# PaddlePaddle/Paddle3D

Measured on NVIDIA H100. Metric: CenterPoint frames/sec @300k pts, 0.075m voxel (0.1m voxel: geometry_01m), 1440x1440x40 grid, higher is better.
Workload: dtype f16x3 (fp16 hi/lo' pairs, f32 accumulation)

## Files before the change

### include/p3d_b200.h

```cpp
#ifndef P3D_B200_H_
#define P3D_B200_H_

#include <stddef.h>
#include <stdint.h>

#ifdef __cplusplus
extern "C" {
#endif

typedef void *p3d_stream_t;

enum p3d_status {
  P3D_OK = 0,
  P3D_ERR_INVALID_ARG = -1,
  P3D_ERR_WORKSPACE = -2,
  P3D_ERR_CUDA = -3,
  P3D_ERR_UNSUPPORTED = -4
};

const char *p3d_status_string(int status);
int p3d_last_cuda_error(void);
int p3d_abi_version(void);

size_t p3d_hard_voxelize_workspace_bytes(int64_t num_points, int max_points, int max_voxels);
int p3d_hard_voxelize(const float *points, int64_t num_points, int num_point_dim, const float *voxel_size_host,
                      const float *point_cloud_range_host, int max_points, int max_voxels, float *voxels,
                      int32_t *coords, int32_t *num_points_per_voxel, int32_t *num_voxels, void *workspace,
                      size_t workspace_bytes, p3d_stream_t stream);

int p3d_voxelize_mean(const float *points, int64_t num_points, int num_point_dim, const float *voxel_size_host,
                      const float *point_cloud_range_host, int max_points, int max_voxels, int batch_id,
                      float *mean, int32_t *coors4, int32_t *num_points_per_voxel, int32_t *num_voxels,
                      void *workspace, size_t workspace_bytes, p3d_stream_t stream);

int p3d_voxel_mean(const float *voxels, const int32_t *num_points_per_voxel, const int32_t *num_voxels_dev,
                   int num_voxels_cap, int max_points, int num_point_dim, float *mean, p3d_stream_t stream);

size_t p3d_scatter_dense_workspace_bytes(int batch, int D, int ny, int nx);
int p3d_scatter_dense(const float *feats, const int32_t *coords, const int32_t *n_dev, int n_cap, int C,
                      int batch, int D, int ny, int nx, int use_z, float *out, void *workspace,
                      size_t workspace_bytes, p3d_stream_t stream);

int p3d_bev_pool_v2(const float *depth, const float *feat, const int32_t *ranks_depth, const int32_t *ranks_feat,
                    const int32_t *ranks_bev, const int32_t *interval_lengths, const int32_t *interval_starts,
                    int n_intervals, int c, float *out, int64_t out_numel, p3d_stream_t stream);
int p3d_bev_pool_v2_bkwd(const float *out_grad, const float *depth, const float *feat, const int32_t *ranks_depth,
                         const int32_t *ranks_feat, const int32_t *ranks_bev, const int32_t *interval_lengths,
                         const int32_t *interval_starts, int n_intervals, int c, float *depth_grad,
                         int64_t depth_numel, float *feat_grad, int64_t feat_numel, p3d_stream_t stream);

int p3d_boxes_overlap_bev(const float *boxes_a, int num_a, const float *boxes_b, int num_b, float *overlap,
                          p3d_stream_t stream);
int p3d_boxes_iou_bev(const float *boxes_a, int num_a, const float *boxes_b, int num_b, float *iou,
                      p3d_stream_t stream);
size_t p3d_nms_workspace_bytes(int n);
int p3d_nms(const float *boxes, int n, float nms_overlap_thresh, int normal, int32_t *keep, int32_t *num_keep,
            void *workspace, size_t workspace_bytes, p3d_stream_t stream);

size_t p3d_centerpoint_postprocess_workspace_bytes(int num_tasks, int feat_h, int feat_w, int nms_pre_max_size,
                                                    int nms_post_max_size);
int p3d_centerpoint_postprocess(int num_tasks, const float *const *hm, const int32_t *hm_channels_host,
                                const float *const *reg, const float *const *height, const float *const *dim,
                                const float *const *vel, const float *const *rot, int feat_h, int feat_w,
                                const float *voxel_size_host, const float *point_cloud_range_host,
                                const float *post_center_range_host, const int32_t *num_classes_host,
                                int down_ratio, float score_threshold, float nms_iou_threshold,
                                int nms_pre_max_size, int nms_post_max_size, int with_velocity, float *bboxes,
                                float *scores, int64_t *labels, int32_t *counts, void *workspace,
                                size_t workspace_bytes, p3d_stream_t stream);

#define P3D_BEVDET_NMS_ROTATE 0
#define P3D_BEVDET_NMS_CIRCLE 1
size_t p3d_bevdet_postprocess_workspace_bytes(int num_tasks, const int32_t *hm_channels_host, int feat_h, int feat_w,
                                              int max_num);
int p3d_bevdet_postprocess(int num_tasks, const float *const *hm, const int32_t *hm_channels_host,
                           const float *const *reg, const float *const *height, const float *const *dim,
                           const float *const *vel, const float *const *rot, int feat_h, int feat_w,
                           const float *voxel_size_host, const float *point_cloud_range_host,
                           const float *post_center_range_host, int out_size_factor, float score_threshold,
                           int max_num, int pre_max_size, int post_max_size, const int32_t *nms_type_host,
                           const float *nms_thr_host, const float *min_radius_host, const float *rescale_host,
                           const int32_t *label_offset_host, float *bboxes, float *scores, int64_t *labels,
                           int32_t *counts, void *workspace, size_t workspace_bytes, p3d_stream_t stream);

size_t p3d_sparse_rulebook_workspace_bytes(int64_t n_in_cap, int64_t n_out_cap);
int p3d_sparse_rulebook_subm(const int32_t *coords, const int32_t *n_in_dev, int64_t n_in_cap, int batch,
                             const int *spatial_host, const int *ksize_host, int32_t *nbr, void *workspace,
                             size_t workspace_bytes, p3d_stream_t stream);
int p3d_sparse_rulebook_conv(const int32_t *coords, const int32_t *n_in_dev, int64_t n_in_cap, int batch,
                             const int *spatial_host, const int *ksize_host, const int *stride_host,
                             const int *pad_host, int32_t *out_coords, int32_t *n_out_dev, int64_t out_cap,
                             int32_t *nbr, void *workspace, size_t workspace_bytes, p3d_stream_t stream);

size_t p3d_sparse_table_bytes(int64_t rows_cap);
int p3d_sparse_table_build(const int32_t *coords, const int32_t *n_dev, int64_t n_cap, int batch,
                           const int *spatial_host, void *table, size_t table_bytes, p3d_stream_t stream);
int p3d_sparse_rulebook_subm_t(const int32_t *coords, const int32_t *n_dev, int64_t n_cap, int batch,
                               const int *spatial_host, const int *ksize_host, const void *table, size_t table_bytes,
                               int32_t *nbr, p3d_stream_t stream);

int p3d_sparse_rulebook_level_t(const int32_t *coords, const int32_t *n_in_dev, int64_t n_in_cap, int batch,
                                const int *spatial_host, const int *ksize_host, const int *stride_host,
                                const int *pad_host, const void *table_in, size_t table_in_bytes, int32_t *out_coords,
                                int32_t *n_out_dev, int64_t out_cap, void *table_out, size_t table_out_bytes,
                                int32_t *nbr, const int *subm_ksize_host, int32_t *nbr_subm, p3d_stream_t stream);

int p3d_sparse_affine_act(const float *x, const int32_t *n_dev, int64_t n_cap, int C, const float *scale,
                          const float *shift, const float *residual, int relu, float *out, p3d_stream_t stream);

enum p3d_conv_precision { P3D_CONV_FP32 = 0, P3D_CONV_TF32X3 = 1 };
size_t p3d_sparse_conv_packed_weight_bytes(int K, int Cin, int Cout);
int p3d_sparse_conv_pack_weights(const float *weight, int K, int Cin, int Cout, float *packed, p3d_stream_t stream);
int p3d_sparse_conv_gather_gemm(const float *in, const int32_t *nbr, const int32_t *n_out_dev, int64_t n_out_cap,
                                int K, int Cin, int Cout, const float *weight, const float *scale,
                                const float *shift, const float *residual, int relu, int precision, float *out,
                                p3d_stream_t stream);

size_t p3d_sparse_conv_splitk_workspace_bytes(int64_t n_out_cap, int Cin, int Cout);
int p3d_sparse_conv_gather_gemm_tf32x3_ws(const float *in, const int32_t *nbr, const int32_t *n_out_dev,
                                          int64_t n_out_cap, int K, int Cin, int Cout, const float *packed_weight,
                                          const float *scale, const float *shift, const float *residual, int relu,
                                          float *out, void *workspace, size_t workspace_bytes, p3d_stream_t stream);

int p3d_rows_convert_layout(const float *src, int src_layout, const int32_t *n_dev, int64_t n_cap, int C, float *dst,
                            p3d_stream_t stream);
int p3d_sparse_conv_gather_gemm_split(const float *in_split, const int32_t *nbr, const int32_t *n_out_dev,
                                      int64_t n_out_cap, int K, int Cin, int Cout, const float *packed_weight,
                                      const float *scale, const float *shift, const float *residual_split, int relu,
                                      float *out_f32, float *out_split, p3d_stream_t stream);
int p3d_sparse_conv_gather_gemm_split_ws(const float *in_split, const int32_t *nbr, const int32_t *n_out_dev,
                                         int64_t n_out_cap, int K, int Cin, int Cout, const float *packed_weight,
                                         const float *scale, const float *shift, const float *residual_split, int relu,
                                         float *out_f32, float *out_split, void *workspace, size_t workspace_bytes,
                                         p3d_stream_t stream);

int p3d_sparse_conv_small_cin_h16(const float *in, const int32_t *nbr, const int32_t *n_out_dev, int64_t n_out_cap, int K,
                                  int Cin, int Cout, const float *weight, const float *scale, const float *shift, int relu,
                                  float *out_f32, void *out_h16, int32_t *status_dev, p3d_stream_t stream);
int p3d_sparse_rows_to_pixel_h16(const void *rows_h16, const int32_t *coords, const int32_t *n_dev, int n_cap, int C,
                                 int batch, int D, int ny, int nx, void *out_pixel_h16, p3d_stream_t stream);
size_t p3d_sparse_conv_f16_packed_weight_bytes(int K, int Cin, int Cout);
int p3d_sparse_conv_f16_pack_weights(const float *weight, int K, int Cin, int Cout, void *packed, int32_t *status_dev,
                                     p3d_stream_t stream);
int p3d_rows_convert_h16(const void *src, int to_h16, const int32_t *n_dev, int64_t n_cap, int C, void *dst,
                         int32_t *status_dev, p3d_stream_t stream);
size_t p3d_sparse_conv_f16_workspace_bytes(int64_t n_out_cap, int Cout, int max_splits);
int p3d_sparse_conv_f16(const void *in_h16, const int32_t *nbr, const int32_t *n_out_dev, int64_t n_out_cap, int K,
                        int Cin, int Cout, const void *packed_weight, const float *scale, const float *shift,
                        const void *residual_h16, int relu, float *out_f32, void *out_h16, void *workspace,
                        size_t workspace_bytes, int max_splits, int32_t *status_dev, p3d_stream_t stream);

size_t p3d_sparse_conv_wm_packed_weight_bytes(int K, int Cin, int Cout);
int p3d_sparse_conv_wm_pack_weights(const float *weight, int K, int Cin, int Cout, void *packed, int32_t *status_dev,
                                    p3d_stream_t stream);
size_t p3d_sparse_conv_wm_workspace_bytes(int64_t n_out_cap, int Cout);
int p3d_sparse_conv_wm(const void *in_h16, const int32_t *nbr, const int32_t *n_out_dev, int64_t n_out_cap, int K, int Cin,
                       int Cout, const void *packed_weight, const float *scale, const float *shift,
                       const void *residual_h16, int relu, float *out_f32, void *out_h16, void *workspace,
                       size_t workspace_bytes, int32_t *status_dev, p3d_stream_t stream);

int p3d_nchw_to_pixel_split(const float *in, int B, int C, int H, int W, float *out_split, p3d_stream_t stream);
size_t p3d_dense_conv2d_packed_weight_bytes(int taps, int Cin, int Cout, int n_tile);
int p3d_dense_conv2d_split(const float *in_split, int B, int H, int W, int Cin, const float *packed_weight, int Cout,
                           int n_tile, int kh, int kw, int stride, int pad, int up, const float *scale,
                           const float *shift, int relu, float *out_split, int out_C, int out_c0, float *out_nchw,
                           p3d_stream_t stream);

int p3d_head_final_conv(const float *in_split, int B, int H, int W, int in_C, int Cin, int groups, const float *weight,
                        const float *bias, const int32_t *plane0_host, const int32_t *cnt_host, int planes,
                        float *out_nchw, p3d_stream_t stream);

int p3d_nchw_to_pixel_h16(const float *in, int B, int C, int H, int W, void *out_h16, int32_t *status_dev,
                          p3d_stream_t stream);
int p3d_pixel_h16_to_nchw(const void *in_h16, int B, int C, int H, int W, float *out, p3d_stream_t stream);
size_t p3d_dense_conv2d_f16_packed_weight_bytes(int taps, int Cin, int Cout, int n_tile);
int p3d_dense_conv2d_f16_pack_weights(const float *weight_tci, int taps, int Cin, int n_tile, void *packed,
                                      int32_t *status_dev, p3d_stream_t stream);
size_t p3d_bev_pool_prepare_workspace_bytes(int64_t num_points);
int p3d_bev_pool_prepare(const float *coor, int B, int N, int D, int H, int W, const float *grid_lower_bound_host,
                         const float *grid_interval_host, const int32_t *grid_size_host, int32_t *ranks_bev,
                         int32_t *ranks_depth, int32_t *ranks_feat, int32_t *interval_starts, int32_t *interval_lengths,
                         int32_t *counts_dev, void *workspace, size_t workspace_bytes, p3d_stream_t stream);

typedef struct p3d_lss_camera {
  float inv_post_rot[9];
  float post_trans[3];
  float combine[9];
  float trans[3];
} p3d_lss_camera;

int p3d_lss_prepare(const p3d_lss_camera *cams, const float *bda, const float *axis_depth, const float *axis_x,
                    const float *axis_y, int B, int N, int D, int H, int W, const float *grid_lower_bound_host,
                    const float *grid_interval_host, const int32_t *grid_size_host, float *coor, int32_t *ranks_bev,
                    int32_t *ranks_depth, int32_t *ranks_feat, int32_t *interval_starts, int32_t *interval_lengths,
                    int32_t *counts_dev, void *workspace, size_t workspace_bytes, p3d_stream_t stream);
int p3d_lss_depth_feat(const float *logits, const float *tran_feat, int BN, int D, int H, int W, int C, float *depth,
                       float *feat, p3d_stream_t stream);
int p3d_lss_depth_feat_h16(const void *rows_h16, int BN, int H, int W, int in_C, int D, int C, float *depth, float *feat,
                           p3d_stream_t stream);
int p3d_bev_pool_v2_dev(const float *depth, const float *feat, const int32_t *ranks_depth, const int32_t *ranks_feat,
                        const int32_t *ranks_bev, const int32_t *interval_lengths, const int32_t *interval_starts,
                        const int32_t *counts_dev, int64_t capacity, int c, int B, int Z, int Y, int X, int planar,
                        float *out, p3d_stream_t stream);

int p3d_head_out_conv_f16(const void *in_h16, int B, int H, int W, int in_C, int Cin, int groups, const void *packed_weight,
                          const float *bias, const int32_t *cin0_dev, const int32_t *plane0_dev, const int32_t *cnt_dev,
                          int planes, float *out_nchw, p3d_stream_t stream);
int p3d_head_conv_p_f16(const void *in_h16, int B, int H, int W, int Cin, const void *packed_weight, int Cout,
                        const float *scale, const float *shift, const void *packed_w2, float *p_out, int32_t *status_dev,
                        p3d_stream_t stream);
int p3d_head_tap_sum(const float *p_in, int B, int H, int W, int groups, const float *bias, const int32_t *plane0_dev,
                     const int32_t *cnt_dev, int planes, float *out_nchw, p3d_stream_t stream);
int p3d_dense_conv2d_f16(const void *in_h16, int B, int H, int W, int Cin, const void *packed_weight, int Cout, int n_tile,
                         int kh, int kw, int stride, int pad, int up, const float *scale, const float *shift, int relu,
                         void *out_h16, int out_C, int out_c0, float *out_nchw, int mode, int m_tiles,
                         int32_t *status_dev, p3d_stream_t stream);
int p3d_dense_conv2d_f16_residual(const void *in_h16, int B, int H, int W, int Cin, const void *packed_weight, int Cout,
                                  int n_tile, int kh, int kw, int stride, int pad, int up, const float *scale,
                                  const float *shift, int relu, void *out_h16, int out_C, int out_c0, float *out_nchw,
                                  const void *res_h16, int res_C, int mode, int m_tiles, int32_t *status_dev,
                                  p3d_stream_t stream);
int p3d_upsample_bilinear_h16(const void *in_h16, int B, int h, int w, int C, int scale, void *out_h16, int out_C, int out_c0,
                              int32_t *status_dev, p3d_stream_t stream);
int p3d_upsample_nearest_h16(const void *in_h16, int B, int h, int w, int C, int scale, void *out_h16, int out_C, int out_c0,
                             p3d_stream_t stream);
size_t p3d_resnet_stem_packed_weight_bytes(void);
int p3d_resnet_stem_pack_weights(const float *weight, void *packed, int32_t *status_dev, p3d_stream_t stream);
int p3d_resnet_stem_h16(const float *in, int B, int H, int W, const void *packed_weight, const float *scale, const float *shift,
                        void *out_h16, int32_t *status_dev, p3d_stream_t stream);
int p3d_image_prep_u8(const uint8_t *frames, int N, int band_rows, int H0, int W0, const int32_t *kh, const int32_t *xbounds,
                      int kh_size, int rW, const int32_t *kv, const int32_t *ybounds, int kv_size, int rH, int crop_x,
                      int crop_y, int fH, int fW, const float *mean_host, const double *std_inv_host, int swap_rb,
                      float *out, p3d_stream_t stream);
int p3d_bev_pool_v2_dev_h16(const float *depth, const float *feat, const int32_t *ranks_depth, const int32_t *ranks_feat,
                            const int32_t *ranks_bev, const int32_t *interval_lengths, const int32_t *interval_starts,
                            const int32_t *counts_dev, int64_t capacity, int c, int B, int Z, int Y, int X, void *out_h16,
                            int out_C, int32_t *status_dev, p3d_stream_t stream);
int p3d_bev_shift_h16(const void *in_h16, int B, int h, int w, int in_C, int C, const float *tf_dev, void *out_h16, int out_C,
                      int out_c0, int32_t *status_dev, p3d_stream_t stream);

int p3d_pillar_feature_net(const float *voxels, const int32_t *num_points_per_voxel, const int32_t *coors,
                           const int32_t *num_voxels_dev, int64_t n_cap, int max_points, int num_point_dim,
                           int out_channels, const float *weight, const float *bn_scale, const float *bn_shift,
                           const float *voxel_size_host, const float *point_cloud_range_host, float *out,
                           p3d_stream_t stream);
int p3d_pillar_feature_net2(const float *voxels, const int32_t *num_points_per_voxel, const int32_t *coors,
                            const int32_t *num_voxels_dev, int64_t n_cap, int max_points, int num_point_dim,
                            int mid_channels, const float *weight1, const float *bn_scale1, const float *bn_shift1,
                            int out_channels, const float *weight2, const float *bn_scale2, const float *bn_shift2,
                            const float *voxel_size_host, const float *point_cloud_range_host, float *out,
                            p3d_stream_t stream);

size_t p3d_anchor_head_postprocess_workspace_bytes(int num_anchors, int grid_nx, int grid_ny, int nms_pre_max_size);
int p3d_anchor_head_postprocess(const float *head, int feat_h, int feat_w, int anchors_per_loc, int num_classes,
                                const float *anchors, const int32_t *anchor_corners, const int32_t *coords,
                                const int32_t *num_coords_dev, int coords_cap, int grid_nx, int grid_ny,
                                int anchor_area_threshold, float score_threshold,
                                float nms_iou_threshold, int nms_pre_max_size, int nms_post_max_size,
                                const float *post_center_range_host, float *boxes, float *scores, int64_t *labels,
                                int32_t *counts, uint8_t *anchor_mask, float *sorted_boxes, float *sorted_scores,
                                void *workspace, size_t workspace_bytes, p3d_stream_t stream);

typedef struct p3d_sweep_desc {
  int32_t slot;
  int32_t rows;
  int32_t has_transform;
  float time_lag;
  double ref_from_curr[12];
} p3d_sweep_desc;

size_t p3d_merge_sweeps_workspace_bytes(int num_entries, int64_t slot_cap);
int p3d_merge_sweeps(const float *raw, int num_slots, int64_t slot_cap, int raw_dim, const p3d_sweep_desc *desc,
                     int num_entries, const int32_t *use_dim_host, int n_use_dim, int use_time_lag,
                     float sweep_remove_radius, float *out, int64_t cap, int32_t *n_out_dev, int32_t *status_dev,
                     void *workspace, size_t workspace_bytes, p3d_stream_t stream);

#ifdef __cplusplus
}
#endif
#endif
```

### paddle3d_b200/_lib.py

```python
import ctypes as C
import os

_HERE = os.path.dirname(os.path.abspath(__file__))
LIB_PATH = os.path.join(_HERE, "libp3d_b200.so")
_lib = None

c_f32p = C.c_void_p
_i64 = C.c_int64
_int = C.c_int
_f = C.c_float
_sz = C.c_size_t
_vp = C.c_void_p

SIGNATURES = {
    "p3d_status_string": (C.c_char_p, [_int]),
    "p3d_last_cuda_error": (_int, []),
    "p3d_abi_version": (_int, []),
    "p3d_hard_voxelize_workspace_bytes": (_sz, [_i64, _int, _int]),
    "p3d_hard_voxelize": (_int, [_vp, _i64, _int, _vp, _vp, _int, _int, _vp, _vp, _vp, _vp, _vp, _sz, _vp]),
    "p3d_voxelize_mean": (_int, [_vp, _i64, _int, _vp, _vp, _int, _int, _int, _vp, _vp, _vp, _vp, _vp, _sz, _vp]),
    "p3d_voxel_mean": (_int, [_vp, _vp, _vp, _int, _int, _int, _vp, _vp]),
    "p3d_scatter_dense_workspace_bytes": (_sz, [_int, _int, _int, _int]),
    "p3d_scatter_dense": (_int, [_vp, _vp, _vp, _int, _int, _int, _int, _int, _int, _int, _vp, _vp, _sz, _vp]),
    "p3d_bev_pool_v2": (_int, [_vp, _vp, _vp, _vp, _vp, _vp, _vp, _int, _int, _vp, _i64, _vp]),
    "p3d_bev_pool_v2_bkwd": (_int, [_vp, _vp, _vp, _vp, _vp, _vp, _vp, _vp, _int, _int, _vp, _i64, _vp, _i64, _vp]),
    "p3d_boxes_overlap_bev": (_int, [_vp, _int, _vp, _int, _vp, _vp]),
    "p3d_boxes_iou_bev": (_int, [_vp, _int, _vp, _int, _vp, _vp]),
    "p3d_nms_workspace_bytes": (_sz, [_int]),
    "p3d_nms": (_int, [_vp, _int, _f, _int, _vp, _vp, _vp, _sz, _vp]),
    "p3d_centerpoint_postprocess_workspace_bytes": (_sz, [_int, _int, _int, _int, _int]),
    "p3d_centerpoint_postprocess": (_int, [_int, _vp, _vp, _vp, _vp, _vp, _vp, _vp, _int, _int, _vp, _vp, _vp, _vp,
                                           _int, _f, _f, _int, _int, _int, _vp, _vp, _vp, _vp, _vp, _sz, _vp]),
    "p3d_bevdet_postprocess_workspace_bytes": (_sz, [_int, _vp, _int, _int, _int]),
    "p3d_bevdet_postprocess": (_int, [_int, _vp, _vp, _vp, _vp, _vp, _vp, _vp, _int, _int, _vp, _vp, _vp, _int, _f, _int,
                                      _int, _int, _vp, _vp, _vp, _vp, _vp, _vp, _vp, _vp, _vp, _vp, _sz, _vp]),
    "p3d_sparse_rulebook_workspace_bytes": (_sz, [_i64, _i64]),
    "p3d_sparse_rulebook_subm": (_int, [_vp, _vp, _i64, _int, _vp, _vp, _vp, _vp, _sz, _vp]),
    "p3d_sparse_rulebook_conv": (_int, [_vp, _vp, _i64, _int, _vp, _vp, _vp, _vp, _vp, _vp, _i64, _vp, _vp, _sz,
                                        _vp]),
    "p3d_sparse_table_bytes": (_sz, [_i64]),
    "p3d_sparse_table_build": (_int, [_vp, _vp, _i64, _int, _vp, _vp, _sz, _vp]),
    "p3d_sparse_rulebook_subm_t": (_int, [_vp, _vp, _i64, _int, _vp, _vp, _vp, _sz, _vp, _vp]),
    "p3d_sparse_rulebook_level_t": (_int, [_vp, _vp, _i64, _int, _vp, _vp, _vp, _vp, _vp, _sz, _vp, _vp, _i64, _vp, _sz,
                                           _vp, _vp, _vp, _vp]),
    "p3d_sparse_affine_act": (_int, [_vp, _vp, _i64, _int, _vp, _vp, _vp, _int, _vp, _vp]),
    "p3d_sparse_conv_packed_weight_bytes": (_sz, [_int, _int, _int]),
    "p3d_sparse_conv_pack_weights": (_int, [_vp, _int, _int, _int, _vp, _vp]),
    "p3d_rows_convert_layout": (_int, [_vp, _int, _vp, _i64, _int, _vp, _vp]),
    "p3d_sparse_conv_gather_gemm_split": (_int, [_vp, _vp, _vp, _i64, _int, _int, _int, _vp, _vp, _vp, _vp, _int, _vp,
                                                 _vp, _vp]),
    "p3d_sparse_conv_gather_gemm_split_ws": (_int, [_vp, _vp, _vp, _i64, _int, _int, _int, _vp, _vp, _vp, _vp, _int, _vp,
                                                    _vp, _vp, _sz, _vp]),
    "p3d_sparse_conv_splitk_workspace_bytes": (_sz, [_i64, _int, _int]),
    "p3d_sparse_conv_small_cin_h16": (_int, [_vp, _vp, _vp, _i64, _int, _int, _int, _vp, _vp, _vp, _int, _vp, _vp, _vp, _vp]),
    "p3d_sparse_rows_to_pixel_h16": (_int, [_vp, _vp, _vp, _int, _int, _int, _int, _int, _int, _vp, _vp]),
    "p3d_sparse_conv_f16_packed_weight_bytes": (_sz, [_int, _int, _int]),
    "p3d_sparse_conv_f16_pack_weights": (_int, [_vp, _int, _int, _int, _vp, _vp, _vp]),
    "p3d_rows_convert_h16": (_int, [_vp, _int, _vp, _i64, _int, _vp, _vp, _vp]),
    "p3d_sparse_conv_f16_workspace_bytes": (_sz, [_i64, _int, _int]),
    "p3d_sparse_conv_f16": (_int, [_vp, _vp, _vp, _i64, _int, _int, _int, _vp, _vp, _vp, _vp, _int, _vp, _vp, _vp, _sz,
                                   _int, _vp, _vp]),
    "p3d_sparse_conv_wm_packed_weight_bytes": (_sz, [_int, _int, _int]),
    "p3d_sparse_conv_wm_pack_weights": (_int, [_vp, _int, _int, _int, _vp, _vp, _vp]),
    "p3d_sparse_conv_wm_workspace_bytes": (_sz, [_i64, _int]),
    "p3d_sparse_conv_wm": (_int, [_vp, _vp, _vp, _i64, _int, _int, _int, _vp, _vp, _vp, _vp, _int, _vp, _vp, _vp, _sz,
                                  _vp, _vp]),
    "p3d_nchw_to_pixel_split": (_int, [_vp, _int, _int, _int, _int, _vp, _vp]),
    "p3d_dense_conv2d_packed_weight_bytes": (_sz, [_int, _int, _int, _int]),
    "p3d_pillar_feature_net": (_int, [_vp, _vp, _vp, _vp, _i64, _int, _int, _int, _vp, _vp, _vp, _vp, _vp, _vp, _vp]),
    "p3d_pillar_feature_net2": (_int, [_vp, _vp, _vp, _vp, _i64, _int, _int, _int, _vp, _vp, _vp, _int, _vp, _vp, _vp, _vp,
                                       _vp, _vp, _vp]),
    "p3d_head_final_conv": (_int, [_vp, _int, _int, _int, _int, _int, _int, _vp, _vp, _vp, _vp, _int, _vp, _vp]),
    "p3d_nchw_to_pixel_h16": (_int, [_vp, _int, _int, _int, _int, _vp, _vp, _vp]),
    "p3d_pixel_h16_to_nchw": (_int, [_vp, _int, _int, _int, _int, _vp, _vp]),
    "p3d_dense_conv2d_f16_packed_weight_bytes": (_sz, [_int, _int, _int, _int]),
    "p3d_dense_conv2d_f16_pack_weights": (_int, [_vp, _int, _int, _int, _vp, _vp, _vp]),
    "p3d_bev_pool_prepare_workspace_bytes": (_sz, [_i64]),
    "p3d_bev_pool_prepare": (_int, [_vp, _int, _int, _int, _int, _int, _vp, _vp, _vp, _vp, _vp, _vp, _vp, _vp, _vp, _vp, _sz,
                                    _vp]),
    "p3d_lss_prepare": (_int, [_vp, _vp, _vp, _vp, _vp, _int, _int, _int, _int, _int, _vp, _vp, _vp, _vp, _vp, _vp, _vp, _vp,
                               _vp, _vp, _vp, _sz, _vp]),
    "p3d_lss_depth_feat": (_int, [_vp, _vp, _int, _int, _int, _int, _int, _vp, _vp, _vp]),
    "p3d_bev_pool_v2_dev": (_int, [_vp, _vp, _vp, _vp, _vp, _vp, _vp, _vp, _i64, _int, _int, _int, _int, _int, _int, _vp, _vp]),
    "p3d_head_out_conv_f16": (_int, [_vp, _int, _int, _int, _int, _int, _int, _vp, _vp, _vp, _vp, _vp, _int, _vp, _vp]),
    "p3d_head_conv_p_f16": (_int, [_vp, _int, _int, _int, _int, _vp, _int, _vp, _vp, _vp, _vp, _vp, _vp]),
    "p3d_head_tap_sum": (_int, [_vp, _int, _int, _int, _int, _vp, _vp, _vp, _int, _vp, _vp]),
    "p3d_dense_conv2d_f16": (_int, [_vp, _int, _int, _int, _int, _vp, _int, _int, _int, _int, _int, _int, _int, _vp, _vp,
                                    _int, _vp, _int, _int, _vp, _int, _int, _vp, _vp]),
    "p3d_dense_conv2d_f16_residual": (_int, [_vp, _int, _int, _int, _int, _vp, _int, _int, _int, _int, _int, _int, _int, _vp,
                                             _vp, _int, _vp, _int, _int, _vp, _vp, _int, _int, _int, _vp, _vp]),
    "p3d_upsample_bilinear_h16": (_int, [_vp, _int, _int, _int, _int, _int, _vp, _int, _int, _vp, _vp]),
    "p3d_upsample_nearest_h16": (_int, [_vp, _int, _int, _int, _int, _int, _vp, _int, _int, _vp]),
    "p3d_resnet_stem_packed_weight_bytes": (_sz, []),
    "p3d_resnet_stem_pack_weights": (_int, [_vp, _vp, _vp, _vp]),
    "p3d_resnet_stem_h16": (_int, [_vp, _int, _int, _int, _vp, _vp, _vp, _vp, _vp, _vp]),
    "p3d_lss_depth_feat_h16": (_int, [_vp, _int, _int, _int, _int, _int, _int, _vp, _vp, _vp]),
    "p3d_image_prep_u8": (_int, [_vp, _int, _int, _int, _int, _vp, _vp, _int, _int, _vp, _vp, _int, _int, _int, _int, _int,
                                 _int, _vp, _vp, _int, _vp, _vp]),
    "p3d_bev_pool_v2_dev_h16": (_int, [_vp, _vp, _vp, _vp, _vp, _vp, _vp, _vp, _i64, _int, _int, _int, _int, _int, _vp, _int,
                                       _vp, _vp]),
    "p3d_bev_shift_h16": (_int, [_vp, _int, _int, _int, _int, _int, _vp, _vp, _int, _int, _vp, _vp]),
    "p3d_dense_conv2d_split": (_int, [_vp, _int, _int, _int, _int, _vp, _int, _int, _int, _int, _int, _int, _int, _vp, _vp,
                                      _int, _vp, _int, _int, _vp, _vp]),
    "p3d_sparse_conv_gather_gemm_tf32x3_ws": (_int, [_vp, _vp, _vp, _i64, _int, _int, _int, _vp, _vp, _vp, _vp, _int, _vp,
                                                     _vp, _sz, _vp]),
    "p3d_sparse_conv_gather_gemm": (_int, [_vp, _vp, _vp, _i64, _int, _int, _int, _vp, _vp, _vp, _vp, _int, _int,
                                           _vp, _vp]),
    "p3d_anchor_head_postprocess_workspace_bytes": (_sz, [_int, _int, _int, _int]),
    "p3d_anchor_head_postprocess": (_int, [_vp, _int, _int, _int, _int, _vp, _vp, _vp, _vp, _int, _int, _int, _int, _f,
                                           _f, _int, _int, _vp, _vp, _vp, _vp, _vp, _vp, _vp, _vp, _vp, _sz, _vp]),
    "p3d_merge_sweeps_workspace_bytes": (_sz, [_int, _i64]),
    "p3d_merge_sweeps": (_int, [_vp, _int, _i64, _int, _vp, _int, _vp, _int, _int, _f, _vp, _i64, _vp, _vp, _vp, _sz,
                                _vp]),
}


class P3DError(RuntimeError):
    pass


def lib():
    global _lib
    if _lib is None:
        if not os.path.exists(LIB_PATH):
            raise P3DError("libp3d_b200.so is not built: run `python -c 'import __graft_entry__ as g; g.build()'` "
                           "(paddle3d_b200 has no CPU or library fallback)")
        _lib = C.CDLL(LIB_PATH)
        for name, (res, args) in SIGNATURES.items():
            fn = getattr(_lib, name)
            fn.restype = res
            fn.argtypes = args
    return _lib


_DEBUG_SYNC = bool(os.environ.get("P3D_DEBUG_SYNC"))


def check(rc, what):
    if _DEBUG_SYNC and rc == 0:
        import torch
        try:
            torch.cuda.synchronize()
        except Exception as e:
            raise P3DError("%s: kernel fault (%s)" % (what, e))
    if rc != 0:
        l = lib()
        msg = l.p3d_status_string(rc).decode()
        extra = " (cudaError %d)" % l.p3d_last_cuda_error() if rc == -3 else ""
        raise P3DError("%s failed: %s%s" % (what, msg, extra))


def fptr(arr):
    return C.cast(arr, C.c_void_p)


def host_floats(vals):
    return (C.c_float * len(vals))(*[float(v) for v in vals])


def host_ints(vals):
    return (C.c_int * len(vals))(*[int(v) for v in vals])
```

### paddle3d_b200/centerpoint_pillars.py

```python
import numpy as np
import torch

from . import synth
from .dense_head import DenseRPNHead, SecondTrunk
from .frame import CapturedFrame, ResultSlot
from .ops import centerpoint_postprocess as cpp
from .ops import pillar_encoder as pe
from .ops import sparse_nn as sp
from .ops import voxelize as vox
from .pointpillars import grid_size

CONFIG = dict(
    pfn=dict(feat_channels=(64, 64), bn_eps=1e-3),
    backbone=dict(out_channels=(64, 128, 256), layer_nums=(3, 5, 5), downsample_strides=(2, 2, 2)),
    fpn=dict(out_channels=(128, 128, 128), upsample_strides=(0.5, 1, 2), use_conv_for_no_stride=True),
    head=dict(tasks=tuple(synth.CENTERPOINT_TASKS), share_conv_channel=64),
    test=synth.CENTERPOINT_PILLARS_TEST_CFG,
)


class CenterPointPillars:

    def __init__(self, cfg=None, model_cfg=None):
        self.cfg = dict(cfg or synth.CP_PILLARS)
        self.mc = model_cfg or CONFIG
        mc = self.mc
        self.grid = grid_size(self.cfg)
        self.F = self.cfg["point_dim"]
        c1, c2 = mc["pfn"]["feat_channels"]
        self.pfn_channels = (c1 // 2, c2)
        self.C = c2
        b, f, h = mc["backbone"], mc["fpn"], mc["head"]
        self.head = DenseRPNHead(in_channels=self.C, out_channels=b["out_channels"], layer_nums=b["layer_nums"],
                                 downsample_strides=b["downsample_strides"], fpn_out_channels=f["out_channels"],
                                 upsample_strides=f["upsample_strides"], tasks=h["tasks"],
                                 share_conv_channel=h["share_conv_channel"], bev_depth=1)
        self.test_cfg = dict(mc["test"])
        self.label_off = synth.label_offsets(list(h["tasks"]))
        self.feat_hw, self.cat_hw = self._feature_sizes()
        self.device = None

    def _feature_sizes(self):
        h, w = self.grid[1], self.grid[0]
        sizes = []
        for blk in self.head.blocks:
            for c in blk:
                h, w = (h + 2 * c.padding - c.k) // c.stride + 1, (w + 2 * c.padding - c.k) // c.stride + 1
            sizes.append((h, w))
        cat = {SecondTrunk.deblock_out_hw(de, hh, ww) for (hh, ww), de in zip(sizes, self.head.deblocks)}
        if len(cat) != 1:
            raise ValueError("model config: the FPN deblocks give different sizes %s" % sorted(cat))
        return sizes, cat.pop()

    def init_weight(self, seed=0, device="cuda", bn_gain=1.0):
        rng = np.random.default_rng(seed)
        eps = self.mc["pfn"]["bn_eps"]
        self.pfn = []
        for fan_in, c in ((self.F + 5, self.pfn_channels[0]), (2 * self.pfn_channels[0], self.pfn_channels[1])):
            self.pfn.append(dict(weight=synth.kaiming_uniform(rng, (fan_in, c), fan_in),
                                 gamma=np.full(c, bn_gain, np.float32), beta=np.zeros(c, np.float32),
                                 mean=np.zeros(c, np.float32), var=np.ones(c, np.float32), eps=eps))
        self.head.init_weight(seed=seed + 1, device=device, bn_gain=bn_gain)
        self.device = None if device is None else torch.device(device)
        if device is not None:
            self.pfn_dev = [dict(l, weight=torch.from_numpy(l["weight"]).to(device)) for l in self.pfn]
            self.pfn_folded = [pe.fold_bn(l["gamma"], l["beta"], l["mean"], l["var"], l["eps"], device) for l in self.pfn]
        return self

    def export_numpy(self):
        return dict(self.head.export_numpy(), pfn=self.pfn)

    def encode(self, points):
        cfg = self.cfg
        voxels, co, npv, nv = vox.hard_voxelize(points, cfg["voxel_size"], cfg["point_cloud_range"], cfg["max_points"],
                                                cfg["max_voxels"])
        coors = torch.nn.functional.pad(co, (1, 0))
        feats = pe.pillar_feature_net2(voxels, npv, coors, self.pfn_dev, cfg["voxel_size"], cfg["point_cloud_range"],
                                       num_voxels=nv, folded=self.pfn_folded)
        nx, ny = self.grid
        image, shape = sp.sparse_coo_tensor(coors, feats, [1, 1, ny, nx, self.C], num=nv).to_pixel_h16()
        return image, shape, coors, nv

    def dense(self, image, shape):
        return self.head.forward_h16(image, shape)

    def postprocess(self, h):
        return cpp.centerpoint_postprocess_heads(h, self.cfg["voxel_size"][:2], self.cfg["point_cloud_range"],
                                                 self.test_cfg, self.label_off)

    def calibrate_heatmap_bias(self, points, target_frac=0.014):
        image, shape, _, _ = self.encode(points)
        self.head.calibrate_heatmap_bias(image, self.test_cfg["score_threshold"], target_frac, shape=shape)
        return self

    def head_planes(self):
        return self.head.head_planes()

    def flops(self):
        out = dict(backbone=0.0, fpn=0.0)
        h, w = self.grid[1], self.grid[0]
        for blk in self.head.blocks:
            for c in blk:
                h, w = (h + 2 * c.padding - c.k) // c.stride + 1, (w + 2 * c.padding - c.k) // c.stride + 1
                out["backbone"] += 2.0 * h * w * c.cin * c.cout * c.k * c.k
        for (h, w), de in zip(self.feat_hw, self.head.deblocks):
            oh, ow = SecondTrunk.deblock_out_hw(de, h, w)
            out["fpn"] += 2.0 * oh * ow * de.cin * de.cout * (1 if de.up > 1 else de.k * de.k)
        out.update(self.head.head_flops(*self.cat_hw))
        return out


class CenterPointPillarsHotPath(CapturedFrame):

    def __init__(self, cfg=None, device="cuda:0", seed=0, num_points=None, bn_gain=1.0, model_cfg=None,
                 sweep_input=None, sweep_ring=None):
        super().__init__(cfg or synth.CP_PILLARS, device, num_points, sweep_input, sweep_ring)
        m = self.model = CenterPointPillars(self.cfg, model_cfg).init_weight(seed=seed, device=self.device,
                                                                             bn_gain=bn_gain)
        self.slot = ResultSlot(len(m.label_off) * m.test_cfg["nms_post_max_size"], 9, len(m.label_off) + 1,
                               1 if self.sweep_input is None else 2)

    def forward_device(self):
        m = self.model
        if self.sweep_input is not None:
            self._merge_sweeps()
        image, shape, coors, nv = m.encode(self.points)
        h = m.dense(image, shape)
        boxes, scores, labels, counts = m.postprocess(h)
        status = torch.stack([sp.status_tensor(self.device)[0]] +
                             ([self._merge_status[0]] if self.sweep_input is not None else []))
        return dict(boxes=boxes, scores=scores, labels=labels, counts=counts, num_voxels=nv, coors=coors, head=h,
                    status=status)

    def _calibrate(self):
        self.model.calibrate_heatmap_bias(self.points)

    def check_status(self, status_host):
        st = [int(v) for v in status_host]
        if len(st) > 1:
            self._check_merge_status(st[1])
        if st[0]:
            raise RuntimeError("CenterPoint-pillars: an activation left fp16's range (|x| >= 65504) on the fp16-pair path")
```

### paddle3d_b200/csrc/dense_conv_f16.cu

```cuda
#include <cuda.h>
#include <cuda_fp16.h>

#include <type_traits>

#include "h16.cuh"
#include "p3d_b200.h"
#include "tc_common.cuh"

namespace p3d {
namespace dcf {

using namespace tc;

constexpr int kTW = 8, kTH = 16;
constexpr int kPitch = kTW + 2;
constexpr int kMaxA = 6, kMaxB = 12;
constexpr int kSmemBudget = (227 - 6) * 1024;
constexpr int kDenseThreads = 384;
constexpr uint32_t kConsumerWarps = 8;
constexpr uint32_t kEpiThreads = 96;

struct Params {
  int B, H, W, Cin;
  int taps, kw, stride, pad;
  int up;
  int oH, oW;
  int tiles_x, tiles_y, n_ntiles;
  int cout;
  int out_H, out_W;
  int out_C, out_c0;
  int relu;
  const uint8_t *packed_w;
  const float *scale, *shift;
  uint8_t *out_h16;
  float *out_nchw;
  int32_t *status;
};
struct ParamsP : Params {
  const uint8_t *packed_w2;
};
struct ParamsR : Params {
  const uint8_t *res_h16;
  int res_C;
};
template <bool FUSE_P, bool RES = false>
using KParams = std::conditional_t<FUSE_P, ParamsP, std::conditional_t<RES, ParamsR, Params>>;

constexpr int kP2Blk = 64 * 32, kP2Bytes = 4 * kP2Blk, kPPitch = 28;

template <int N, int MT, bool HALO>
struct Cfg {
  static constexpr int A_ROWS = HALO ? kPitch * (kTH * MT + 2) : kM * MT;
  static constexpr int A_BYTES = ((A_ROWS * 128 + 1023) / 1024) * 1024;
  static constexpr int B_BYTES = 128 * N;
  static constexpr int B_BLK = 64 * N;
  static constexpr int SP = N + 8;
  static constexpr int STG_WG = MT * 64 * SP;
  static constexpr int STG_BYTES = 2 * STG_WG * 4;
  static constexpr int PAIR_BLK = 64 * 128, PAIR_BYTES = MT * (N / 32) * PAIR_BLK;
  static_assert(PAIR_BYTES + 2 * 2 * N * 4 <= STG_WG * 4 && STG_WG * 4 % 1024 == 0, "pair tile inside the staging tile");
  static constexpr int AVAIL = kSmemBudget - STG_BYTES;
  static constexpr int NA_TAP_RAW = AVAIL / (A_BYTES + B_BYTES);
  static constexpr int NA = HALO ? 2 : (NA_TAP_RAW > kMaxA ? kMaxA : NA_TAP_RAW);
  static constexpr int BUDGET = AVAIL - NA * A_BYTES;
  static constexpr int NB_RAW = BUDGET / B_BYTES;
  static constexpr int NB = NB_RAW > kMaxB ? kMaxB : NB_RAW;
  static constexpr int ACC = MT * N;
  static constexpr int SPU = HALO ? 9 : 1;
  static constexpr int P_REGS = 88, C_REGS = 208;
  static_assert(128 * P_REGS + 256 * C_REGS <= kDenseThreads * 168, "register split");
  static_assert(N == 64 || N == 128, "N tile: 64 or 128");
  static_assert(MT == 1 || MT == 2, "one or two M tiles");
  static_assert(MT * N <= 128, "accumulators: at most 128 registers per thread");
  static_assert(NB >= 3, "weight ring too shallow");
  static_assert(NA >= 2 && NA <= kMaxA, "activation ring depth");
};

__device__ __forceinline__ void tma_tile4d(uint32_t dst, const CUtensorMap *map, int c, int x, int y, int b, uint32_t bar) {
  asm volatile(
      "cp.async.bulk.tensor.4d.shared::cluster.global.tile.mbarrier::complete_tx::bytes [%0], [%1, {%2, %3, %4, %5}], [%6];" ::
          "r"(dst),
      "l"(reinterpret_cast<uint64_t>(map)), "r"(c), "r"(x), "r"(y), "r"(b), "r"(bar)
      : "memory");
}
__device__ __forceinline__ void tma_store4d(const CUtensorMap *map, uint32_t src, int c, int x, int y, int b) {
  asm volatile("cp.async.bulk.tensor.4d.global.shared::cta.bulk_group [%0, {%2, %3, %4, %5}], [%1];" ::"l"(
                   reinterpret_cast<uint64_t>(map)),
               "r"(src), "r"(c), "r"(x), "r"(y), "r"(b)
               : "memory");
}
__device__ __forceinline__ void tma_store5d(const CUtensorMap *map, uint32_t src, int c, int d1, int d2, int d3, int d4) {
  asm volatile("cp.async.bulk.tensor.5d.global.shared::cta.bulk_group [%0, {%2, %3, %4, %5, %6}], [%1];" ::"l"(
                   reinterpret_cast<uint64_t>(map)),
               "r"(src), "r"(c), "r"(d1), "r"(d2), "r"(d3), "r"(d4)
               : "memory");
}
__device__ __forceinline__ void st_shared_u32(uint32_t addr, uint32_t v) {
  asm volatile("st.shared.b32 [%0], %1;" ::"r"(addr), "r"(v));
}
__device__ __forceinline__ float2 ld_shared_f2(uint32_t addr) {
  float2 v;
  asm("ld.shared.v2.f32 {%0, %1}, [%2];" : "=f"(v.x), "=f"(v.y) : "r"(addr));
  return v;
}
__device__ __forceinline__ void bulk_commit() { asm volatile("cp.async.bulk.commit_group;" ::: "memory"); }
__device__ __forceinline__ void bulk_wait_read() { asm volatile("cp.async.bulk.wait_group.read 0;" ::: "memory"); }
__device__ __forceinline__ void bulk_wait_all() { asm volatile("cp.async.bulk.wait_group 0;" ::: "memory"); }
struct Item {
  int nt, tap0, tx0, ty0, b;
};

enum TraceField {
  kTrItems, kTrCycles,
  kTrAFull, kTrBFull = kTrAFull + 2,
  kTrMma = kTrBFull + 2,
  kTrEpi = kTrMma + 2,
  kTrStageFree = kTrEpi + 2,
  kTrAEmpty = kTrStageFree + 2, kTrBEmpty,
  kTrEwWait, kTrEwBusy,
  kTrFields
};
#ifdef P3D_DENSE_TRACE
constexpr int kTrMaxCtas = 1024;
__device__ unsigned long long g_dense_trace[kTrMaxCtas][kTrFields];
struct Trace {
  unsigned long long sum[kTrFields] = {};
  __device__ __forceinline__ long long now() const { return clock64(); }
  __device__ __forceinline__ void add(int f, long long t0) { sum[f] += static_cast<unsigned long long>(clock64() - t0); }
  __device__ __forceinline__ void count(int f, unsigned long long v) { sum[f] += v; }
  __device__ void flush(int cw) const {
#pragma unroll
    for (int f = 0; f < kTrFields; ++f) {
      const int dst = f >= kTrAFull && f < kTrAEmpty ? f + cw : f;
      if (sum[f]) atomicAdd(&g_dense_trace[blockIdx.x % kTrMaxCtas][dst], sum[f]);
    }
  }
};
#else
struct Trace {
  __device__ __forceinline__ long long now() const { return 0; }
  __device__ __forceinline__ void add(int, long long) {}
  __device__ __forceinline__ void count(int, unsigned long long) {}
  __device__ __forceinline__ void flush(int) const {}
};
#endif
__device__ __forceinline__ Item decode(long long idx, const Params &p, int th) {
  Item it;
  long long q = blockIdx.x + idx * gridDim.x;
  it.nt = static_cast<int>(q % p.n_ntiles);
  q /= p.n_ntiles;
  it.tap0 = 0;
  if (p.up > 1) {
    const int up2 = p.up * p.up;
    it.tap0 = static_cast<int>(q % up2);
    q /= up2;
  }
  it.tx0 = static_cast<int>(q % p.tiles_x) * kTW;
  q /= p.tiles_x;
  it.ty0 = static_cast<int>(q % p.tiles_y) * th;
  it.b = static_cast<int>(q / p.tiles_y);
  return it;
}

template <int N, int MT>
__device__ __forceinline__ void epilogue_warps(const Params &p, const float *stg, unsigned long long *staged,
                                               unsigned long long *freed, long long n_items, int th, int et) {
  constexpr int SP = N + 8, ROWS = MT * 64;
  const int ew = et >> 5, lane = et & 31;
  bool ovf = false;
  Trace tr;
  for (long long idx = 0; idx < n_items; ++idx) {
    const Item im = decode(idx, p, th);
    const int dy = p.up > 1 ? im.tap0 / p.up : 0, dx = p.up > 1 ? im.tap0 % p.up : 0;
    for (int c = 0; c < 2; ++c) {
      long long t0 = tr.now();
      mbar_wait(smem_u32(staged + c), static_cast<uint32_t>(idx & 1));
      tr.add(kTrEwWait, t0);
      t0 = tr.now();
      const float *st = stg + c * ROWS * SP;
      auto pixel = [&](int r, int &Y, int &X) {
        const int m = c * 64 + (r & 63), iy = im.ty0 + (r >> 6) * kTH + m / kTW, ix = im.tx0 + m % kTW;
        Y = iy * p.up + dy;
        X = ix * p.up + dx;
        return iy < p.oH && ix < p.oW;
      };
      if (p.out_h16) {
        const int r4 = lane >> 3, c4 = (lane & 7) * 4;
        for (int q = 0; q < N / 32; ++q) {
          const int col = q * 32 + c4, ch = im.nt * N + col, oc = p.out_c0 + ch;
          if (ch >= p.cout) continue;
          float sc[4], sh[4];
#pragma unroll
          for (int e = 0; e < 4; ++e) {
            sc[e] = p.scale ? __ldg(p.scale + ch + e) : 1.0f;
            sh[e] = p.shift ? __ldg(p.shift + ch + e) : 0.0f;
          }
#pragma unroll 2
          for (int rq = ew; rq < ROWS / 4; rq += 3) {
            const int r = rq * 4 + r4;
            int Y, X;
            if (!pixel(r, Y, X)) continue;
            const float4 o4 = *reinterpret_cast<const float4 *>(st + r * SP + col);
            float v[4] = {o4.x, o4.y, o4.z, o4.w};
#pragma unroll
            for (int e = 0; e < 4; ++e) {
              v[e] = fmaf(v[e], sc[e], sh[e]);
              if (p.relu) v[e] = fmaxf(v[e], 0.f);
            }
            __half2 h01, l01, h23, l23;
            split_h16x2(v[0], v[1], h01, l01, ovf);
            split_h16x2(v[2], v[3], h23, l23, ovf);
            uint8_t *op = p.out_h16 + ((static_cast<size_t>(im.b) * p.out_H + Y) * p.out_W + X) * (4 * static_cast<size_t>(p.out_C)) +
                          (oc / 32) * 128 + (oc % 32) * 2;
            *reinterpret_cast<uint2 *>(op) = make_uint2(*reinterpret_cast<const uint32_t *>(&h01), *reinterpret_cast<const uint32_t *>(&h23));
            *reinterpret_cast<uint2 *>(op + 64) = make_uint2(*reinterpret_cast<const uint32_t *>(&l01), *reinterpret_cast<const uint32_t *>(&l23));
          }
        }
      }
      if (p.out_nchw) {
        const int px = lane & 7, cc = lane >> 3;
        for (int u = ew; u < (ROWS / 8) * (N / 4); u += 3) {
          const int r = (u % (ROWS / 8)) * 8 + px, col = (u / (ROWS / 8)) * 4 + cc, ch = im.nt * N + col;
          int Y, X;
          if (ch >= p.cout || !pixel(r, Y, X)) continue;
          const float sc = p.scale ? __ldg(p.scale + ch) : 1.0f, sh = p.shift ? __ldg(p.shift + ch) : 0.0f;
          float v = fmaf(st[r * SP + col], sc, sh);
          if (p.relu) v = fmaxf(v, 0.f);
          p.out_nchw[((static_cast<size_t>(im.b) * p.cout + ch) * p.out_H + Y) * p.out_W + X] = v;
        }
      }
      mbar_arrive(smem_u32(freed + c));
      tr.add(kTrEwBusy, t0);
    }
  }
  if (ovf && p.status) atomicOr(p.status, 1);
  if (et == 0) tr.flush(0);
}

template <int N, int MT, bool FUSE_P>
__device__ __forceinline__ void epilogue_pairs(const Params &p, const CUtensorMap *out_map, const uint8_t *tiles, int tile_bytes,
                                               unsigned long long *staged, unsigned long long *freed, long long n_items,
                                               int th, int et) {
  constexpr int NQ = N / 32, BLK = 64 * 128;
  const bool lead = et == 0;
  const bool whole = p.out_c0 % 32 == 0;
  Trace tr;
  for (long long idx = 0; idx < n_items; ++idx) {
    const Item im = decode(idx, p, th);
    const int dy = p.up > 1 ? im.tap0 / p.up : 0, dx = p.up > 1 ? im.tap0 % p.up : 0;
    for (int c = 0; c < 2; ++c) {
      long long t0 = tr.now();
      mbar_wait(smem_u32(staged + c), static_cast<uint32_t>(idx & 1));
      tr.add(kTrEwWait, t0);
      t0 = tr.now();
      if constexpr (FUSE_P) {
        if (lead) tma_store4d(out_map, smem_u32(tiles + c * tile_bytes), 0, im.tx0, im.ty0 + c * 8, (im.b * p.n_ntiles + im.nt) * 2);
      } else {
        for (int blk = 0; blk < MT * NQ; ++blk) {
          const int ch0 = im.nt * N + (blk % NQ) * 32, iy0 = im.ty0 + (blk / NQ) * kTH + c * 8;
          if (ch0 >= p.cout) continue;
          const uint8_t *src = tiles + c * tile_bytes + blk * BLK;
          if (whole && ch0 + 32 <= p.cout) {
            if (!lead) continue;
            const int hc = 2 * (p.out_c0 + ch0);
            if (p.up == 1) {
              tma_store4d(out_map, smem_u32(src), hc, im.tx0, iy0, im.b);
            } else {
              for (int y = 0; y < 8 && iy0 + y < p.oH; ++y)
                tma_store5d(out_map, smem_u32(src + y * 1024), hc, dx, im.tx0, dy, im.b * p.oH + iy0 + y);
            }
            continue;
          }
          for (int u = et; u < 128; u += kEpiThreads) {
            const int r = u >> 1, h = u & 1, iy = iy0 + (r >> 3), ix = im.tx0 + (r & 7);
            if (ch0 + 16 * h >= p.cout || iy >= p.oH || ix >= p.oW) continue;
            const int oc = p.out_c0 + ch0 + 16 * h, Y = iy * p.up + dy, X = ix * p.up + dx;
            uint8_t *op = p.out_h16 + ((static_cast<size_t>(im.b) * p.out_H + Y) * p.out_W + X) * (4 * static_cast<size_t>(p.out_C)) +
                          (oc / 32) * 128 + (oc % 32) * 2;
            const uint8_t *row = src + r * 128;
  #pragma unroll
            for (int k = 0; k < 2; ++k) {
              *reinterpret_cast<uint4 *>(op + 16 * k) = *reinterpret_cast<const uint4 *>(row + (((2 * h + k) ^ (r & 7)) << 4));
              *reinterpret_cast<uint4 *>(op + 64 + 16 * k) = *reinterpret_cast<const uint4 *>(row + (((4 + 2 * h + k) ^ (r & 7)) << 4));
            }
          }
        }
      }
      if (lead) {
        bulk_commit();
        bulk_wait_read();
      }
      mbar_arrive(smem_u32(freed + c));
      tr.add(kTrEwBusy, t0);
    }
  }
  if (lead) {
    bulk_wait_all();
    tr.flush(0);
  }
}

template <int N, int MT, bool HALO, bool FUSE_P = false, bool RES = false>
__global__ void __launch_bounds__(kDenseThreads, 1)
    dense_conv_f16_kernel(const __grid_constant__ CUtensorMap in_map, const __grid_constant__ CUtensorMap out_map,
                          const KParams<FUSE_P, RES> p) {
  using C = Cfg<N, MT, HALO>;
  static_assert(!(FUSE_P && RES), "a residual launch writes the pixel H16 image");
  static_assert(!FUSE_P || (N == 128 && MT == 1 && HALO && 2 * kP2Bytes == C::B_BYTES &&
                            2 * 64 * kPPitch * 4 <= C::PAIR_BYTES),
                "fused P: two 64-channel heads' W2 images fill one weight slot; P fits over the pair blocks");
  constexpr int TH = kTH * MT;
  constexpr int H = N / 2;
  asm volatile("griddepcontrol.launch_dependents;" ::: "memory");
  asm volatile("griddepcontrol.wait;" ::: "memory");
  const int up2 = p.up * p.up;
  const long long n_total = static_cast<long long>(p.B) * p.tiles_y * p.tiles_x * p.n_ntiles * (p.up > 1 ? up2 : 1);
  if (static_cast<long long>(blockIdx.x) >= n_total) return;
  const long long n_items = (n_total - blockIdx.x + gridDim.x - 1) / gridDim.x;

  extern __shared__ __align__(1024) uint8_t smem_raw[];
  uint8_t *smem = reinterpret_cast<uint8_t *>((reinterpret_cast<uintptr_t>(smem_raw) + 1023) & ~uintptr_t(1023));
  __shared__ __align__(8) unsigned long long s_bar[2 * kMaxA + 2 * kMaxB + 4];
  constexpr int kAF = 0, kAE = kMaxA, kBF = 2 * kMaxA, kBE = 2 * kMaxA + kMaxB, kSS = 2 * kMaxA + 2 * kMaxB, kSF = kSS + 2;

  const int tid = threadIdx.x, wg = tid >> 7, wtid = tid & 127;
  if (tid == 0) {
    for (int s = 0; s < C::NA; ++s) {
      mbar_init(smem_u32(&s_bar[kAF + s]), 1);
      mbar_init(smem_u32(&s_bar[kAE + s]), kConsumerWarps);
    }
    for (int s = 0; s < C::NB; ++s) {
      mbar_init(smem_u32(&s_bar[kBF + s]), 1);
      mbar_init(smem_u32(&s_bar[kBE + s]), kConsumerWarps);
    }
    for (int c = 0; c < 2; ++c) {
      mbar_init(smem_u32(&s_bar[kSS + c]), 128);
      mbar_init(smem_u32(&s_bar[kSF + c]), kEpiThreads);
    }
    fence_mbar_init();
  }
  __syncthreads();
  const uint32_t a_ring = smem_u32(smem);
  const uint32_t b_ring = a_ring + C::NA * C::A_BYTES;
  float *const stg = reinterpret_cast<float *>(smem + C::NA * C::A_BYTES + C::NB * C::B_BYTES);
  const bool pairs = p.out_nchw == nullptr;
  const int G = p.Cin / 32;
  const int taps_item = p.up > 1 ? 1 : p.taps;
  const int units_item = HALO ? G : taps_item * G;

  if (wg == 0) {
    asm volatile("setmaxnreg.dec.sync.aligned.u32 %0;" ::"n"(C::P_REGS));
    if (tid >= 32) {
      if (pairs)
        epilogue_pairs<N, MT, FUSE_P>(p, &out_map, reinterpret_cast<const uint8_t *>(stg), C::STG_WG * 4, s_bar + kSS, s_bar + kSF,
                              n_items, TH, tid - 32);
      else
        epilogue_warps<N, MT>(p, stg, s_bar + kSS, s_bar + kSF, n_items, TH, tid - 32);
      return;
    }
    if (tid != 0) return;
    uint32_t a_slot = 0, a_ph = 0, b_slot = 0, b_ph = 0;
    Trace tr;
    for (long long idx = 0; idx < n_items; ++idx) {
      const Item im = decode(idx, p, TH);
      const uint8_t *w_tile = p.packed_w + static_cast<size_t>(im.nt) * p.taps * (p.Cin / 16) * C::B_BLK;
      int dy = 0, dx = 0;
      for (int tu = 0; tu < (HALO ? 1 : taps_item); ++tu) {
        const int tap = p.up > 1 ? im.tap0 : tu;
        for (int g = 0; g < G; ++g) {
          const uint32_t abar = smem_u32(&s_bar[kAF + a_slot]), a_dst = a_ring + a_slot * C::A_BYTES;
          const long long t0 = tr.now();
          mbar_wait(smem_u32(&s_bar[kAE + a_slot]), a_ph ^ 1u);
          tr.add(kTrAEmpty, t0);
          mbar_arrive_expect_tx(abar, static_cast<uint32_t>(C::A_ROWS * 128));
          if (HALO) {
            tma_tile4d(a_dst, &in_map, g * 64, im.tx0 - 1, im.ty0 - 1, im.b, abar);
          } else {
            const int x = im.tx0 * p.stride - p.pad + dx, y = im.ty0 * p.stride - p.pad + dy;
            tma_tile4d(a_dst, &in_map, g * 64, x, y, im.b, abar);
          }
          if (++a_slot == C::NA) a_slot = 0, a_ph ^= 1u;
          for (int t = 0; t < C::SPU; ++t) {
            const uint32_t bbar = smem_u32(&s_bar[kBF + b_slot]);
            const long long t1 = tr.now();
            mbar_wait(smem_u32(&s_bar[kBE + b_slot]), b_ph ^ 1u);
            tr.add(kTrBEmpty, t1);
            mbar_arrive_expect_tx(bbar, static_cast<uint32_t>(C::B_BYTES));
            bulk_g2s(b_ring + b_slot * C::B_BYTES, w_tile + (static_cast<size_t>(HALO ? t : tap) * (p.Cin / 16) + 2 * g) * C::B_BLK,
                     static_cast<uint32_t>(C::B_BYTES), bbar);
            if (++b_slot == C::NB) b_slot = 0, b_ph ^= 1u;
          }
        }
        if (++dx == p.kw) dx = 0, ++dy;
      }
      if constexpr (FUSE_P) {
        const uint32_t bbar = smem_u32(&s_bar[kBF + b_slot]);
        const long long t1 = tr.now();
        mbar_wait(smem_u32(&s_bar[kBE + b_slot]), b_ph ^ 1u);
        tr.add(kTrBEmpty, t1);
        mbar_arrive_expect_tx(bbar, static_cast<uint32_t>(C::B_BYTES));
        bulk_g2s(b_ring + b_slot * C::B_BYTES, p.packed_w2 + static_cast<size_t>(im.nt) * C::B_BYTES,
                 static_cast<uint32_t>(C::B_BYTES), bbar);
        if (++b_slot == C::NB) b_slot = 0, b_ph ^= 1u;
      }
    }
    tr.flush(0);
    return;
  }

  asm volatile("setmaxnreg.inc.sync.aligned.u32 %0;" ::"n"(C::C_REGS));
  const int cw = wg - 1;
  const bool warp_leader = (tid & 31) == 0;
  auto release = [&](int base, uint32_t slot) {
    if (warp_leader) mbar_arrive(smem_u32(&s_bar[base + slot]));
  };
  uint32_t a_slot = 0, a_ph = 0, b_slot = 0, b_ph = 0;
  float acc[C::ACC];
  bool ovf = false;
  Trace tr;
  const long long t_start = tr.now();
  for (long long idx = 0; idx < n_items; ++idx) {
#pragma unroll
    for (int i = 0; i < C::ACC; ++i) acc[i] = 0.f;
    const Item im = decode(idx, p, TH);
    const uint32_t ss = smem_u32(stg) + cw * C::STG_WG * 4 + C::PAIR_BYTES + static_cast<uint32_t>(idx & 1) * 2 * N * 4;
    if (pairs) {
      for (int c = wtid; c < 2 * N; c += 128) {
        const int ch = im.nt * N + c % N;
        const float *src = c < N ? p.scale : p.shift;
        st_shared_u32(ss + c * 4, __float_as_uint(ch < p.cout && src ? __ldg(src + ch) : (c < N ? 1.0f : 0.0f)));
      }
    }
    uint32_t prev_b = 0;
    int prev_a = -1;
    bool pending = false;
    for (int ua = 0; ua < units_item; ++ua) {
      long long t0 = tr.now();
      mbar_wait(smem_u32(&s_bar[kAF + a_slot]), a_ph);
      tr.add(kTrAFull, t0);
      const uint32_t a_base = a_ring + a_slot * C::A_BYTES;
      for (int t = 0; t < C::SPU; ++t) {
        t0 = tr.now();
        mbar_wait(smem_u32(&s_bar[kBF + b_slot]), b_ph);
        tr.add(kTrBFull, t0);
        const uint32_t b_base = b_ring + b_slot * C::B_BYTES;
        wg_fence();
#pragma unroll
        for (int kb = 0; kb < 2; ++kb) {
          const uint32_t bk = b_base + static_cast<uint32_t>(kb * C::B_BLK);
          const uint64_t dbh = smem_desc(bk, 2 * N * 16, 128), dbl = smem_desc(bk + N * 16, 2 * N * 16, 128);
#pragma unroll
          for (int mt = 0; mt < MT; ++mt) {
            uint32_t a0, sbo;
            if (HALO) {
              a0 = a_base + static_cast<uint32_t>(((mt * kTH + cw * 8 + t / 3) * kPitch + t % 3) * 128);
              sbo = kPitch * 128;
            } else {
              a0 = a_base + static_cast<uint32_t>((mt * kM + cw * 64) * 128);
              sbo = 1024;
            }
            const uint64_t dah = desc_sw128(a0 + kb * 32, sbo), dal = desc_sw128(a0 + (2 + kb) * 32, sbo);
            float *d = acc + mt * N;
            wg::mma_f16<N>(d, dah, dbh, 1u);
            wg::mma_f16<N>(d + H, dah, dbl, 1u);
            wg::mma_f16<N>(d + H, dal, dbh, 1u);
          }
        }
        wg_commit();
        t0 = tr.now();
        wg_wait<1>();
        tr.add(kTrMma, t0);
        if (pending) {
          release(kBE, prev_b);
          if (prev_a >= 0) release(kAE, static_cast<uint32_t>(prev_a));
        }
        pending = true;
        prev_b = b_slot;
        prev_a = t == C::SPU - 1 ? static_cast<int>(a_slot) : -1;
        if (++b_slot == C::NB) b_slot = 0, b_ph ^= 1u;
      }
      if (++a_slot == C::NA) a_slot = 0, a_ph ^= 1u;
    }
    long long t0 = tr.now();
    wg_wait<0>();
    tr.add(kTrMma, t0);
    t0 = tr.now();
    release(kBE, prev_b);
    release(kAE, static_cast<uint32_t>(prev_a));
    wg_fence_acc<C::ACC>(acc);
    tr.add(kTrEpi, t0);
    t0 = tr.now();
    if (idx > 0) mbar_wait(smem_u32(&s_bar[kSF + cw]), static_cast<uint32_t>((idx - 1) & 1));
    tr.add(kTrStageFree, t0);
    t0 = tr.now();
    if (pairs) {
      const int lane = wtid & 31, key = lane >> 2;
      const uint32_t row = smem_u32(stg) + cw * C::STG_WG * 4 + ((wtid >> 5) * 16 + key) * 128 + (lane & 3) * 4;
      uint32_t a_hi[4], a_lo[4];
#pragma unroll
      for (int jj = 0; jj < 4; ++jj) a_hi[jj] = row + ((jj ^ key) << 4), a_lo[jj] = row + (((4 + jj) ^ key) << 4);
      uint32_t after_bar;
      asm volatile("bar.sync %1, 128;\n\tmov.u32 %0, 0;" : "=r"(after_bar) : "r"(1 + cw) : "memory");
      const uint32_t sc_col = ss + after_bar + (lane & 3) * 8;
      int r_off[MT][2], r_rem = 0;
      if constexpr (RES) {
        const int r_iy = im.ty0 + cw * 8 + (wtid >> 5) * 2, r_ix = im.tx0 + key;
#pragma unroll
        for (int mt = 0; mt < MT; ++mt)
#pragma unroll
          for (int h = 0; h < 2; ++h) {
            const int Y = r_iy + mt * kTH + h;
            r_off[mt][h] = r_ix < p.oW && Y < p.oH
                               ? ((im.b * p.out_H + Y) * p.out_W + r_ix) * 4 * p.res_C + (im.nt * N / 32) * 128 + (lane & 3) * 4
                               : -1;
          }
        r_rem = p.cout - im.nt * N;
      }
      bool o[MT][2] = {};
#pragma unroll
      for (int j = 0; j < N / 8; ++j) {
        const float2 sc = ld_shared_f2(sc_col + j * 32), sh = ld_shared_f2(sc_col + (N + j * 8) * 4);
        const float sc0 = sc.x, sc1 = sc.y, sh0 = sh.x, sh1 = sh.y;
#pragma unroll
        for (int mt = 0; mt < MT; ++mt) {
#pragma unroll
          for (int h = 0; h < 2; ++h) {
            const int i = j * 4 + h * 2;
            float v0 = fmaf(acc[mt * N + H + i], kLoInv, acc[mt * N + i]);
            float v1 = fmaf(acc[mt * N + H + i + 1], kLoInv, acc[mt * N + i + 1]);
            v0 = fmaf(v0, sc0, sh0);
            v1 = fmaf(v1, sc1, sh1);
            if constexpr (RES) {
              if (r_off[mt][h] >= 0 && j * 8 < r_rem) {
                const uint8_t *rp = p.res_h16 + r_off[mt][h] + (j / 4) * 128 + (j & 3) * 16;
                const uint32_t rh = __ldg(reinterpret_cast<const unsigned int *>(rp));
                const uint32_t rl = __ldg(reinterpret_cast<const unsigned int *>(rp + 64));
                const float2 fh = __half22float2(*reinterpret_cast<const __half2 *>(&rh));
                const float2 fl = __half22float2(*reinterpret_cast<const __half2 *>(&rl));
                v0 += fmaf(fl.x, kLoInv, fh.x);
                v1 += fmaf(fl.y, kLoInv, fh.y);
              }
            }
            if (p.relu) v0 = fmaxf(v0, 0.f), v1 = fmaxf(v1, 0.f);
            __half2 hi, lo;
            split_h16x2(v0, v1, hi, lo, o[mt][h]);
            const uint32_t off = (mt * (N / 32) + j / 4) * C::PAIR_BLK + h * 8 * 128;
            st_shared_u32(a_hi[j & 3] + off, *reinterpret_cast<const uint32_t *>(&hi));
            st_shared_u32(a_lo[j & 3] + off, *reinterpret_cast<const uint32_t *>(&lo));
          }
        }
      }
      const int iy = im.ty0 + cw * 8 + (wtid >> 5) * 2, ix = im.tx0 + key;
#pragma unroll
      for (int mt = 0; mt < MT; ++mt)
        ovf |= ix < p.oW && ((o[mt][0] && iy + mt * kTH < p.oH) || (o[mt][1] && iy + mt * kTH + 1 < p.oH));
      fence_proxy_async();
      if constexpr (FUSE_P) {
        asm volatile("bar.sync %0, 128;" ::"r"(1 + cw) : "memory");
        const long long t1 = tr.now();
        mbar_wait(smem_u32(&s_bar[kBF + b_slot]), b_ph);
        tr.add(kTrBFull, t1);
        const uint32_t w2 = b_ring + b_slot * C::B_BYTES, tile = smem_u32(stg) + cw * C::STG_WG * 4;
        float pacc[64];
#pragma unroll
        for (int i = 0; i < 64; ++i) pacc[i] = 0.f;
        wg_fence();
#pragma unroll
        for (int j = 0; j < 2; ++j) {
#pragma unroll
          for (int k = 0; k < 2; ++k) {
#pragma unroll
            for (int kb = 0; kb < 2; ++kb) {
              const uint32_t bk = w2 + static_cast<uint32_t>(j * kP2Bytes + (k * 2 + kb) * kP2Blk);
              const uint64_t dbh = smem_desc(bk, 2 * 32 * 16, 128), dbl = smem_desc(bk + 32 * 16, 2 * 32 * 16, 128);
              const uint32_t a0 = tile + static_cast<uint32_t>((2 * j + k) * C::PAIR_BLK);
              const uint64_t dah = desc_sw128(a0 + kb * 32), dal = desc_sw128(a0 + (2 + kb) * 32);
              wg::mma_f16<32>(pacc + 32 * j, dah, dbh, 1u);
              wg::mma_f16<32>(pacc + 32 * j + 16, dah, dbl, 1u);
              wg::mma_f16<32>(pacc + 32 * j + 16, dal, dbh, 1u);
            }
          }
        }
        wg_commit();
        wg_wait<0>();
        release(kBE, b_slot);
        if (++b_slot == C::NB) b_slot = 0, b_ph ^= 1u;
        wg_fence_acc<64>(pacc);
        asm volatile("bar.sync %0, 128;" ::"r"(1 + cw) : "memory");
        float *const pt = stg + cw * C::STG_WG;
#pragma unroll
        for (int j = 0; j < 2; ++j) {
#pragma unroll
          for (int i = 0; i < 16; i += 2) {
            const int r = frag_row(i, wtid), c = frag_col(i, wtid);
            if (c < kPPitch)
              *reinterpret_cast<float2 *>(pt + (j * 64 + r) * kPPitch + c) =
                  make_float2(fmaf(pacc[32 * j + 16 + i], kLoInv, pacc[32 * j + i]),
                              fmaf(pacc[32 * j + 17 + i], kLoInv, pacc[32 * j + 1 + i]));
          }
        }
        fence_proxy_async();
      }
    } else {
      float *const st = stg + cw * C::STG_WG;
#pragma unroll
      for (int mt = 0; mt < MT; ++mt) {
#pragma unroll
        for (int i = 0; i < H; i += 2) {
          const int r = mt * 64 + frag_row(i, wtid), c = frag_col(i, wtid);
          *reinterpret_cast<float2 *>(st + r * C::SP + c) =
              make_float2(fmaf(acc[mt * N + H + i], kLoInv, acc[mt * N + i]), fmaf(acc[mt * N + H + i + 1], kLoInv, acc[mt * N + i + 1]));
        }
      }
    }
    mbar_arrive(smem_u32(&s_bar[kSS + cw]));
    tr.add(kTrEpi, t0);
  }
  if (ovf && p.status) atomicOr(p.status, 1);
  if (cw == 0) {
    tr.count(kTrItems, static_cast<unsigned long long>(n_items));
    tr.add(kTrCycles, t_start);
  }
  if (wtid == 0) tr.flush(cw);
}

__global__ void __launch_bounds__(256) nchw_to_pixel_h16_kernel(const float *__restrict__ in, int C, long long HW,
                                                                __half *__restrict__ out, int32_t *status) {
  __shared__ float s_t[32][33];
  const int b = blockIdx.z;
  const long long p0 = static_cast<long long>(blockIdx.x) * 32;
  const int c0 = blockIdx.y * 32;
  const int tx = threadIdx.x & 31, ty = threadIdx.x >> 5;
  for (int k = ty; k < 32; k += 8) {
    const int c = c0 + k;
    const long long px = p0 + tx;
    s_t[k][tx] = (c < C && px < HW) ? in[(static_cast<size_t>(b) * C + c) * HW + px] : 0.f;
  }
  __syncthreads();
  bool ovf = false;
  for (int k = ty; k < 32; k += 8) {
    const long long px = p0 + k;
    if (px < HW) {
      __half h, l;
      split_h16(s_t[tx][k], h, l, ovf);
      __half *grp = out + (static_cast<size_t>(b) * HW + px) * (2 * static_cast<size_t>(C)) + static_cast<size_t>(c0) * 2;
      grp[tx] = h;
      grp[32 + tx] = l;
    }
  }
  if (ovf && status) atomicOr(status, 1);
}

__global__ void __launch_bounds__(256) pixel_h16_to_nchw_kernel(const __half *__restrict__ in, int C, long long HW,
                                                                float *__restrict__ out, long long total) {
  const long long q = static_cast<long long>(blockIdx.x) * blockDim.x + threadIdx.x;
  if (q >= total) return;
  const long long px = q % HW;
  const int c = static_cast<int>((q / HW) % C);
  const long long b = q / (HW * C);
  const __half *grp = in + (b * HW + px) * (2 * static_cast<long long>(C)) + (c / 32) * 64;
  out[q] = merge_h16(grp[c % 32], grp[32 + c % 32]);
}

using Encode = CUresult (*)(CUtensorMap *, CUtensorMapDataType, cuuint32_t, void *, const cuuint64_t *, const cuuint64_t *,
                            const cuuint32_t *, const cuuint32_t *, CUtensorMapInterleave, CUtensorMapSwizzle,
                            CUtensorMapL2promotion, CUtensorMapFloatOOBfill);
inline Encode tensor_map_encoder() {
  static Encode encode = nullptr;
  if (!encode) {
    void *fn = nullptr;
    cudaDriverEntryPointQueryResult qr;
    if (cudaGetDriverEntryPoint("cuTensorMapEncodeTiled", &fn, cudaEnableDefault, &qr) != cudaSuccess || !fn) return nullptr;
    encode = reinterpret_cast<Encode>(fn);
  }
  return encode;
}

inline int make_image_map(const void *img, int B, int H, int W, int Cin, int stride, int box_x, int box_y, CUtensorMap *map) {
  const Encode encode = tensor_map_encoder();
  if (!encode) return P3D_ERR_UNSUPPORTED;
  const cuuint64_t row = static_cast<cuuint64_t>(4) * Cin;
  const cuuint64_t gdim[4] = {static_cast<cuuint64_t>(2 * Cin), static_cast<cuuint64_t>(W), static_cast<cuuint64_t>(H),
                              static_cast<cuuint64_t>(B)};
  const cuuint64_t gstride[3] = {row, row * W, row * W * H};
  const cuuint32_t box[4] = {64u, static_cast<cuuint32_t>(box_x * stride), static_cast<cuuint32_t>(box_y * stride), 1u};
  const cuuint32_t estride[4] = {1u, static_cast<cuuint32_t>(stride), static_cast<cuuint32_t>(stride), 1u};
  const CUresult r = encode(map, CU_TENSOR_MAP_DATA_TYPE_FLOAT16, 4, const_cast<void *>(img), gdim, gstride, box, estride,
                            CU_TENSOR_MAP_INTERLEAVE_NONE, CU_TENSOR_MAP_SWIZZLE_128B, CU_TENSOR_MAP_L2_PROMOTION_NONE,
                            CU_TENSOR_MAP_FLOAT_OOB_FILL_NONE);
  return r == CUDA_SUCCESS ? P3D_OK : P3D_ERR_INVALID_ARG;
}

inline int make_out_map(void *img, int B, int H, int W, int out_C, int up, CUtensorMap *map) {
  const Encode encode = tensor_map_encoder();
  if (!encode) return P3D_ERR_UNSUPPORTED;
  const cuuint64_t row = static_cast<cuuint64_t>(4) * out_C;
  CUresult r;
  if (up == 1) {
    const cuuint64_t gdim[4] = {static_cast<cuuint64_t>(2 * out_C), static_cast<cuuint64_t>(W), static_cast<cuuint64_t>(H),
                                static_cast<cuuint64_t>(B)};
    const cuuint64_t gstride[3] = {row, row * W, row * W * H};
    const cuuint32_t box[4] = {64u, static_cast<cuuint32_t>(kTW), 8u, 1u}, estride[4] = {1u, 1u, 1u, 1u};
    r = encode(map, CU_TENSOR_MAP_DATA_TYPE_FLOAT16, 4, img, gdim, gstride, box, estride, CU_TENSOR_MAP_INTERLEAVE_NONE,
               CU_TENSOR_MAP_SWIZZLE_128B, CU_TENSOR_MAP_L2_PROMOTION_NONE, CU_TENSOR_MAP_FLOAT_OOB_FILL_NONE);
  } else {
    const cuuint64_t u = static_cast<cuuint64_t>(up), ow = u * W;
    const cuuint64_t gdim[5] = {static_cast<cuuint64_t>(2 * out_C), u, static_cast<cuuint64_t>(W), u,
                                static_cast<cuuint64_t>(B) * H};
    const cuuint64_t gstride[4] = {row, row * u, row * ow, row * ow * u};
    const cuuint32_t box[5] = {64u, 1u, static_cast<cuuint32_t>(kTW), 1u, 1u}, estride[5] = {1u, 1u, 1u, 1u, 1u};
    r = encode(map, CU_TENSOR_MAP_DATA_TYPE_FLOAT16, 5, img, gdim, gstride, box, estride, CU_TENSOR_MAP_INTERLEAVE_NONE,
               CU_TENSOR_MAP_SWIZZLE_128B, CU_TENSOR_MAP_L2_PROMOTION_NONE, CU_TENSOR_MAP_FLOAT_OOB_FILL_NONE);
  }
  return r == CUDA_SUCCESS ? P3D_OK : P3D_ERR_INVALID_ARG;
}

inline int make_p_map(float *pbuf, int B, int H, int W, int p_groups, CUtensorMap *map) {
  const Encode encode = tensor_map_encoder();
  if (!encode) return P3D_ERR_UNSUPPORTED;
  const cuuint64_t px = static_cast<cuuint64_t>(4) * kPPitch;
  const cuuint64_t gdim[4] = {static_cast<cuuint64_t>(kPPitch), static_cast<cuuint64_t>(W), static_cast<cuuint64_t>(H),
                              static_cast<cuuint64_t>(B) * p_groups};
  const cuuint64_t gstride[3] = {px, px * W, px * W * H};
  const cuuint32_t box[4] = {static_cast<cuuint32_t>(kPPitch), static_cast<cuuint32_t>(kTW), 8u, 2u}, estride[4] = {1u, 1u, 1u, 1u};
  const CUresult r = encode(map, CU_TENSOR_MAP_DATA_TYPE_FLOAT32, 4, pbuf, gdim, gstride, box, estride, CU_TENSOR_MAP_INTERLEAVE_NONE,
                            CU_TENSOR_MAP_SWIZZLE_NONE, CU_TENSOR_MAP_L2_PROMOTION_NONE, CU_TENSOR_MAP_FLOAT_OOB_FILL_NONE);
  return r == CUDA_SUCCESS ? P3D_OK : P3D_ERR_INVALID_ARG;
}

template <int N, int MT, bool HALO, bool FUSE_P = false, bool RES = false>
int launch(const CUtensorMap &map, const CUtensorMap &out_map, const KParams<FUSE_P, RES> &p, cudaStream_t st) {
  using C = Cfg<N, MT, HALO>;
  const size_t smem = static_cast<size_t>(C::NA) * C::A_BYTES + static_cast<size_t>(C::NB) * C::B_BYTES + C::STG_BYTES + 1024;
  if (smem > static_cast<size_t>(kSmemBudget)) return P3D_ERR_UNSUPPORTED;
  auto kern = dense_conv_f16_kernel<N, MT, HALO, FUSE_P, RES>;
  P3D_CUDA_CHECK(cudaFuncSetAttribute(kern, cudaFuncAttributeMaxDynamicSharedMemorySize, static_cast<int>(smem)));
  const long long work = static_cast<long long>(p.B) * p.tiles_y * p.tiles_x * p.n_ntiles * (p.up > 1 ? p.up * p.up : 1);
  cudaLaunchConfig_t cfg = {};
  const long long sms = num_sms();
  cfg.gridDim = dim3(static_cast<unsigned int>(work < sms ? work : sms));
  cfg.blockDim = dim3(kDenseThreads);
  cfg.dynamicSmemBytes = smem;
  cfg.stream = st;
  cudaLaunchAttribute attr[1];
  attr[0].id = cudaLaunchAttributeProgrammaticStreamSerialization;
  attr[0].val.programmaticStreamSerializationAllowed = 1;
  cfg.attrs = attr;
  cfg.numAttrs = 1;
  P3D_CUDA_CHECK(cudaLaunchKernelEx(&cfg, kern, map, out_map, p));
  P3D_LAUNCH_CHECK();
  return P3D_OK;
}

namespace out9 {
constexpr int kHT = 16, kOT = 14;
constexpr int kRows = kHT * kHT;
constexpr int kABytes = kRows * 128;
constexpr int kN = 32, kStride = 29;
constexpr int kWBlk = 64 * kN;
constexpr int kPBytes = kRows * kStride * 4;
constexpr int kMaxNA = 5, kNW = 3;
constexpr int kAcc = 2 * kN;

struct Params {
  int B, H, W, G;
  int tiles_x, tiles_y, groups, planes, NA;
  const uint8_t *packed_w;
  const float *bias;
  const int32_t *cin0;
  const int32_t *plane0, *cnt;
  float *out;
};

__global__ void __launch_bounds__(kThreads, 1) head_out9_kernel(const __grid_constant__ CUtensorMap in_map, const Params p) {
  asm volatile("griddepcontrol.launch_dependents;" ::: "memory");
  asm volatile("griddepcontrol.wait;" ::: "memory");
  const long long n_work = static_cast<long long>(p.B) * p.tiles_y * p.tiles_x * p.groups;
  if (static_cast<long long>(blockIdx.x) >= n_work) return;
  extern __shared__ __align__(1024) uint8_t smem_raw[];
  uint8_t *smem = reinterpret_cast<uint8_t *>((reinterpret_cast<uintptr_t>(smem_raw) + 1023) & ~uintptr_t(1023));
  __shared__ __align__(8) unsigned long long s_bar[kMaxNA + kNW];
  constexpr int kAF = 0, kWF = kMaxNA;
  const int tid = threadIdx.x, wg = tid >> 7, wtid = tid & 127;
  const int NA = p.NA, G = p.G;
  const uint32_t w_slot = static_cast<uint32_t>(2 * G * kWBlk);
  if (tid == 0) {
    for (int s = 0; s < NA; ++s) mbar_init(smem_u32(&s_bar[kAF + s]), 1);
    for (int s = 0; s < kNW; ++s) mbar_init(smem_u32(&s_bar[kWF + s]), 1);
    fence_mbar_init();
  }
  const uint32_t a_ring = smem_u32(smem);
  const uint32_t w_ring = a_ring + static_cast<uint32_t>(NA * kABytes);
  float *s_p = reinterpret_cast<float *>(smem + static_cast<size_t>(NA) * kABytes + static_cast<size_t>(kNW) * w_slot);

  auto decode = [&](long long w, int &g, int &tx0, int &ty0, int &b) {
    g = static_cast<int>(w % p.groups);
    long long q = w / p.groups;
    tx0 = static_cast<int>(q % p.tiles_x) * kOT;
    q /= p.tiles_x;
    ty0 = static_cast<int>(q % p.tiles_y) * kOT;
    b = static_cast<int>(q / p.tiles_y);
  };
  const long long n_items = (n_work - blockIdx.x + gridDim.x - 1) / gridDim.x;
  const long long n_steps = n_items * G;
  auto issue_a = [&](long long q) {
    int g, tx0, ty0, b;
    decode(blockIdx.x + (q / G) * gridDim.x, g, tx0, ty0, b);
    const int cg0 = (p.cin0 ? __ldg(p.cin0 + g) : g * G * 32) / 32;
    const uint32_t slot = static_cast<uint32_t>(q % NA), bar = smem_u32(&s_bar[kAF + slot]);
    mbar_arrive_expect_tx(bar, static_cast<uint32_t>(kABytes));
    tma_tile4d(a_ring + slot * kABytes, &in_map, (cg0 + static_cast<int>(q % G)) * 64, tx0 - 1, ty0 - 1, b, bar);
  };
  auto issue_w = [&](long long i) {
    const int g = static_cast<int>((blockIdx.x + i * gridDim.x) % p.groups);
    const uint32_t slot = static_cast<uint32_t>(i % kNW), bar = smem_u32(&s_bar[kWF + slot]);
    mbar_arrive_expect_tx(bar, w_slot);
    bulk_g2s(w_ring + slot * w_slot, p.packed_w + static_cast<size_t>(g) * w_slot, w_slot, bar);
  };

  long long next_a = 0, next_w = 0, q = 0;
  float acc[kAcc];
  for (long long idx = 0; idx < n_items; ++idx) {
    int g, tx0, ty0, b;
    decode(blockIdx.x + idx * gridDim.x, g, tx0, ty0, b);
    const int cnt = __ldg(p.cnt + g), p0 = __ldg(p.plane0 + g);
    const float4 bias = __ldg(reinterpret_cast<const float4 *>(p.bias) + g);
#pragma unroll
    for (int i = 0; i < kAcc; ++i) acc[i] = 0.f;
    const uint32_t ws = static_cast<uint32_t>(idx % kNW);
    for (int k = 0; k < G; ++k, ++q) {
      __syncthreads();
      if (tid == 0) {
        for (; next_a < n_steps && next_a <= q + NA - 1; ++next_a) issue_a(next_a);
        for (; next_w < n_items && (next_w - kNW + 1) * G <= q; ++next_w) issue_w(next_w);
      }
      if (k == 0) mbar_wait(smem_u32(&s_bar[kWF + ws]), static_cast<uint32_t>((idx / kNW) & 1));
      const uint32_t sa = static_cast<uint32_t>(q % NA);
      mbar_wait(smem_u32(&s_bar[kAF + sa]), static_cast<uint32_t>((q / NA) & 1));
      const uint32_t a_base = a_ring + sa * kABytes;
      const uint32_t w_base = w_ring + ws * w_slot;
      wg_fence();
#pragma unroll
      for (int kb = 0; kb < 2; ++kb) {
        const uint32_t bk = w_base + static_cast<uint32_t>((k * 2 + kb) * kWBlk);
        const uint64_t dbh = smem_desc(bk, 2 * kN * 16, 128), dbl = smem_desc(bk + kN * 16, 2 * kN * 16, 128);
#pragma unroll
        for (int mt = 0; mt < 2; ++mt) {
          const uint32_t a0 = a_base + static_cast<uint32_t>((mt * kM + wg * 64) * 128);
          const uint64_t dah = desc_sw128(a0 + kb * 32), dal = desc_sw128(a0 + (2 + kb) * 32);
          float *d = acc + mt * kN;
          wg::mma_f16<kN>(d, dah, dbh, 1u);
          wg::mma_f16<kN>(d + kN / 2, dah, dbl, 1u);
          wg::mma_f16<kN>(d + kN / 2, dal, dbh, 1u);
        }
      }
      wg_commit();
      wg_wait<0>();
    }
    wg_fence_acc<kAcc>(acc);
#pragma unroll
    for (int mt = 0; mt < 2; ++mt) {
#pragma unroll
      for (int i = 0; i < kN / 2; ++i) {
        const int r = mt * kM + wg * 64 + frag_row(i, wtid), c = frag_col(i, wtid);
        if (c < 27) s_p[r * kStride + c] = fmaf(acc[mt * kN + kN / 2 + i], kLoInv, acc[mt * kN + i]);
      }
    }
    __syncthreads();
    for (int o = tid; o < kOT * kOT; o += kThreads) {
      const int oy = o / kOT, ox = o - oy * kOT;
      const int Y = ty0 + oy, X = tx0 + ox;
      if (Y < p.H && X < p.W) {
        float s0 = bias.x, s1 = bias.y, s2 = bias.z;
#pragma unroll
        for (int t = 0; t < 9; ++t) {
          const float *e = s_p + ((oy + t / 3) * kHT + ox + t % 3) * kStride + t * 3;
          s0 += e[0];
          s1 += e[1];
          s2 += e[2];
        }
        float *op = p.out + ((static_cast<size_t>(b) * p.planes + p0) * p.H + Y) * p.W + X;
        const size_t plane = static_cast<size_t>(p.H) * p.W;
        op[0] = s0;
        if (cnt > 1) op[plane] = s1;
        if (cnt > 2) op[2 * plane] = s2;
      }
    }
  }
}
}

namespace tapsum {
constexpr int kTX = 32, kTY = 8, kThreads = kTX * kTY, kSX = kTX + 2, kSY = kTY + 2, kSP = 27;

struct Params {
  int B, H, W, groups, planes, tiles_x, tiles_y;
  const float *p;
  const float *bias;
  const int32_t *plane0, *cnt;
  float *out;
};

__global__ void __launch_bounds__(kThreads) head_tap_sum_kernel(const Params p) {
  asm volatile("griddepcontrol.launch_dependents;" ::: "memory");
  asm volatile("griddepcontrol.wait;" ::: "memory");
  __shared__ float s_p[kSY * kSX * kSP];
  long long q = blockIdx.x;
  const int tx0 = static_cast<int>(q % p.tiles_x) * kTX;
  q /= p.tiles_x;
  const int ty0 = static_cast<int>(q % p.tiles_y) * kTY;
  q /= p.tiles_y;
  const int g = static_cast<int>(q % p.groups), b = static_cast<int>(q / p.groups);
  const float *src = p.p + static_cast<size_t>(b * p.groups + g) * p.H * p.W * kPPitch;
  constexpr int V = kPPitch / 4;
  for (int u = threadIdx.x; u < kSY * kSX * V; u += kThreads) {
    const int pix = u / V, v = u - pix * V, sy = pix / kSX, sx = pix - sy * kSX, Y = ty0 - 1 + sy, X = tx0 - 1 + sx;
    float4 f = make_float4(0.f, 0.f, 0.f, 0.f);
    if (Y >= 0 && Y < p.H && X >= 0 && X < p.W)
      f = __ldg(reinterpret_cast<const float4 *>(src + (static_cast<size_t>(Y) * p.W + X) * kPPitch) + v);
    float *d = s_p + pix * kSP + v * 4;
    d[0] = f.x;
    d[1] = f.y;
    d[2] = f.z;
    if (v < V - 1) d[3] = f.w;
  }
  __syncthreads();
  const int lx = threadIdx.x % kTX, ly = threadIdx.x / kTX, X = tx0 + lx, Y = ty0 + ly;
  if (X >= p.W || Y >= p.H) return;
  const int cnt = __ldg(p.cnt + g), p0 = __ldg(p.plane0 + g);
  const size_t plane = static_cast<size_t>(p.H) * p.W;
  float *op = p.out + (static_cast<size_t>(b) * p.planes + p0) * plane + static_cast<size_t>(Y) * p.W + X;
  for (int co = 0; co < cnt; ++co) {
    float s = __ldg(p.bias + g * 4 + co);
#pragma unroll
    for (int t = 0; t < 9; ++t) s += s_p[((ly + t / 3) * kSX + lx + t % 3) * kSP + t * 3 + co];
    op[co * plane] = s;
  }
}
}

}
}

using namespace p3d;

extern "C" int p3d_nchw_to_pixel_h16(const float *in, int B, int C, int H, int W, void *out_h16, int32_t *status_dev,
                                     p3d_stream_t stream) {
  if (!in || !out_h16 || B < 1 || C < 32 || C % 32 || H < 1 || W < 1) return P3D_ERR_INVALID_ARG;
  const long long hw = static_cast<long long>(H) * W;
  dim3 grid(static_cast<unsigned int>((hw + 31) / 32), static_cast<unsigned int>(C / 32), B);
  dcf::nchw_to_pixel_h16_kernel<<<grid, 256, 0, static_cast<cudaStream_t>(stream)>>>(in, C, hw, static_cast<__half *>(out_h16),
                                                                                      status_dev);
  P3D_LAUNCH_CHECK();
  return P3D_OK;
}

extern "C" int p3d_pixel_h16_to_nchw(const void *in_h16, int B, int C, int H, int W, float *out, p3d_stream_t stream) {
  if (!in_h16 || !out || B < 1 || C < 32 || C % 32 || H < 1 || W < 1) return P3D_ERR_INVALID_ARG;
  const long long hw = static_cast<long long>(H) * W, total = hw * C * B;
  dcf::pixel_h16_to_nchw_kernel<<<div_up(total, 256), 256, 0, static_cast<cudaStream_t>(stream)>>>(
      static_cast<const __half *>(in_h16), C, hw, out, total);
  P3D_LAUNCH_CHECK();
  return P3D_OK;
}

#ifdef P3D_DENSE_TRACE
extern "C" int p3d_dense_trace_read(unsigned long long *host, int max_ctas, int reset) {
  const size_t n = static_cast<size_t>(max_ctas < dcf::kTrMaxCtas ? max_ctas : dcf::kTrMaxCtas) * dcf::kTrFields;
  P3D_CUDA_CHECK(cudaDeviceSynchronize());
  if (host) P3D_CUDA_CHECK(cudaMemcpyFromSymbol(host, dcf::g_dense_trace, n * sizeof(unsigned long long)));
  if (reset) {
    void *dev = nullptr;
    P3D_CUDA_CHECK(cudaGetSymbolAddress(&dev, dcf::g_dense_trace));
    P3D_CUDA_CHECK(cudaMemset(dev, 0, sizeof(dcf::g_dense_trace)));
    P3D_CUDA_CHECK(cudaDeviceSynchronize());
  }
  return dcf::kTrFields;
}
#endif

extern "C" size_t p3d_dense_conv2d_f16_packed_weight_bytes(int taps, int Cin, int Cout, int n_tile) {
  if (taps < 1 || Cin < 32 || Cin % 32 || Cout < 1 || (n_tile != 16 && n_tile != 32 && n_tile != 64 && n_tile != 128)) return 0;
  const size_t tiles = static_cast<size_t>((Cout + n_tile - 1) / n_tile);
  return align_up(tiles * taps * Cin * static_cast<size_t>(n_tile) * 4);
}

namespace {
template <bool RES>
int dense_conv2d_f16(const void *in_h16, int B, int H, int W, int Cin, const void *packed_weight, int Cout, int n_tile, int kh,
                     int kw, int stride, int pad, int up, const float *scale, const float *shift, int relu, void *out_h16,
                     int out_C, int out_c0, float *out_nchw, const void *res_h16, int res_C, int mode, int m_tiles,
                     int32_t *status_dev, p3d_stream_t stream) {
  if (!in_h16 || !packed_weight || (!out_h16 && !out_nchw) || B < 1 || H < 1 || W < 1 || Cout < 1 || (mode != 0 && mode != 1))
    return P3D_ERR_INVALID_ARG;
  if (Cin < 32 || Cin % 32 || (n_tile != 64 && n_tile != 128)) return P3D_ERR_UNSUPPORTED;
  if (up < 1 || (up > 1 && (kh != up || kw != up || stride != up || pad != 0))) return P3D_ERR_UNSUPPORTED;
  if (up == 1 && (kh < 1 || kw < 1 || kh * kw > 32 || stride < 1 || stride > 2 || pad < 0)) return P3D_ERR_UNSUPPORTED;
  if (out_h16 && (Cout % 16 || out_C % 32 || out_c0 % 16 || out_c0 + Cout > out_C)) return P3D_ERR_INVALID_ARG;
  if ((reinterpret_cast<uintptr_t>(in_h16) & 15) || (reinterpret_cast<uintptr_t>(packed_weight) & 15) ||
      (reinterpret_cast<uintptr_t>(out_h16) & 15))
    return P3D_ERR_INVALID_ARG;
  dcf::KParams<false, RES> p;
  if constexpr (RES) {
    p.res_h16 = static_cast<const uint8_t *>(res_h16);
    p.res_C = res_C;
  }
  p.B = B;
  p.H = H;
  p.W = W;
  p.Cin = Cin;
  p.taps = kh * kw;
  p.kw = kw;
  p.up = up;
  p.stride = up > 1 ? 1 : stride;
  p.pad = up > 1 ? 0 : pad;
  p.oH = up > 1 ? H : (H + 2 * pad - kh) / stride + 1;
  p.oW = up > 1 ? W : (W + 2 * pad - kw) / stride + 1;
  if (p.oH < 1 || p.oW < 1) return P3D_ERR_INVALID_ARG;
  p.out_H = up > 1 ? H * up : p.oH;
  p.out_W = up > 1 ? W * up : p.oW;
  p.n_ntiles = (Cout + n_tile - 1) / n_tile;
  p.cout = Cout;
  p.out_C = out_C;
  p.out_c0 = out_c0;
  p.relu = relu;
  p.packed_w = static_cast<const uint8_t *>(packed_weight);
  p.scale = scale;
  p.shift = shift;
  p.out_h16 = static_cast<uint8_t *>(out_h16);
  p.out_nchw = out_nchw;
  p.status = status_dev;
  const bool halo = mode == 0 && up == 1 && kh == 3 && kw == 3 && stride == 1 && pad == 1;
  int mt = m_tiles;
  if (mt != 1 && mt != 2) {
    const long long tx = (p.oW + dcf::kTW - 1) / dcf::kTW, sms = num_sms();
    const long long per_row = static_cast<long long>(B) * tx * p.n_ntiles * (up > 1 ? up * up : 1);
    const long long items1 = per_row * ((p.oH + dcf::kTH - 1) / dcf::kTH), items2 = per_row * ((p.oH + 2 * dcf::kTH - 1) / (2 * dcf::kTH));
    mt = (n_tile <= 64 && 2 * ((items2 + sms - 1) / sms) <= (items1 + sms - 1) / sms) ? 2 : 1;
  }
  if (n_tile > 64) mt = 1;
  p.tiles_x = (p.oW + dcf::kTW - 1) / dcf::kTW;
  p.tiles_y = (p.oH + dcf::kTH * mt - 1) / (dcf::kTH * mt);
  CUtensorMap map;
  const int bx = halo ? dcf::kPitch : dcf::kTW, by = halo ? dcf::kTH * mt + 2 : dcf::kTH * mt;
  int rc = dcf::make_image_map(in_h16, B, H, W, Cin, p.stride, bx, by, &map);
  if (rc != P3D_OK) return rc;
  CUtensorMap omap = {};
  if (!out_nchw && (rc = dcf::make_out_map(out_h16, B, p.oH, p.oW, out_C, up, &omap)) != P3D_OK) return rc;
  cudaStream_t st = static_cast<cudaStream_t>(stream);
  if (n_tile == 128)
    return halo ? dcf::launch<128, 1, true, false, RES>(map, omap, p, st) : dcf::launch<128, 1, false, false, RES>(map, omap, p, st);
  if (mt == 2)
    return halo ? dcf::launch<64, 2, true, false, RES>(map, omap, p, st) : dcf::launch<64, 2, false, false, RES>(map, omap, p, st);
  return halo ? dcf::launch<64, 1, true, false, RES>(map, omap, p, st) : dcf::launch<64, 1, false, false, RES>(map, omap, p, st);
}
}

extern "C" int p3d_dense_conv2d_f16(const void *in_h16, int B, int H, int W, int Cin, const void *packed_weight, int Cout,
                                    int n_tile, int kh, int kw, int stride, int pad, int up, const float *scale,
                                    const float *shift, int relu, void *out_h16, int out_C, int out_c0, float *out_nchw,
                                    int mode, int m_tiles, int32_t *status_dev, p3d_stream_t stream) {
  return dense_conv2d_f16<false>(in_h16, B, H, W, Cin, packed_weight, Cout, n_tile, kh, kw, stride, pad, up, scale, shift, relu,
                                 out_h16, out_C, out_c0, out_nchw, nullptr, 0, mode, m_tiles, status_dev, stream);
}

extern "C" int p3d_dense_conv2d_f16_residual(const void *in_h16, int B, int H, int W, int Cin, const void *packed_weight,
                                             int Cout, int n_tile, int kh, int kw, int stride, int pad, int up,
                                             const float *scale, const float *shift, int relu, void *out_h16, int out_C,
                                             int out_c0, float *out_nchw, const void *res_h16, int res_C, int mode,
                                             int m_tiles, int32_t *status_dev, p3d_stream_t stream) {
  if (!res_h16 || (reinterpret_cast<uintptr_t>(res_h16) & 15)) return P3D_ERR_INVALID_ARG;
  if (up != 1 || out_nchw || !out_h16 || out_c0 % 32 || res_C % 32) return P3D_ERR_UNSUPPORTED;
  if (res_C < Cout) return P3D_ERR_INVALID_ARG;
  const long long oh = (H + 2 * pad - kh) / (stride > 0 ? stride : 1) + 1, ow = (W + 2 * pad - kw) / (stride > 0 ? stride : 1) + 1;
  if (static_cast<long long>(B) * oh * ow * 4 * res_C > 0x7fffffffll) return P3D_ERR_UNSUPPORTED;
  return dense_conv2d_f16<true>(in_h16, B, H, W, Cin, packed_weight, Cout, n_tile, kh, kw, stride, pad, up, scale, shift, relu,
                                out_h16, out_C, out_c0, out_nchw, res_h16, res_C, mode, m_tiles, status_dev, stream);
}

extern "C" int p3d_head_out_conv_f16(const void *in_h16, int B, int H, int W, int in_C, int Cin, int groups,
                                     const void *packed_weight, const float *bias, const int32_t *cin0_dev,
                                     const int32_t *plane0_dev, const int32_t *cnt_dev, int planes, float *out_nchw,
                                     p3d_stream_t stream) {
  if (!in_h16 || !packed_weight || !bias || !plane0_dev || !cnt_dev || !out_nchw || B < 1 || H < 1 || W < 1 || groups < 1 ||
      planes < 1 || in_C % 32 || Cin > in_C)
    return P3D_ERR_INVALID_ARG;
  if (Cin < 32 || Cin % 32) return P3D_ERR_UNSUPPORTED;
  if ((reinterpret_cast<uintptr_t>(in_h16) & 15) || (reinterpret_cast<uintptr_t>(packed_weight) & 15) ||
      (reinterpret_cast<uintptr_t>(bias) & 15))
    return P3D_ERR_INVALID_ARG;
  namespace o9 = dcf::out9;
  const long long w_ring = static_cast<long long>(o9::kNW) * 2 * (Cin / 32) * o9::kWBlk;
  const long long na = (dcf::kSmemBudget - 1024 - o9::kPBytes - w_ring) / o9::kABytes;
  if (na < 2) return P3D_ERR_UNSUPPORTED;
  o9::Params p;
  p.B = B;
  p.H = H;
  p.W = W;
  p.G = Cin / 32;
  p.tiles_x = (W + o9::kOT - 1) / o9::kOT;
  p.tiles_y = (H + o9::kOT - 1) / o9::kOT;
  p.groups = groups;
  p.planes = planes;
  p.NA = static_cast<int>(na < o9::kMaxNA ? na : o9::kMaxNA);
  p.packed_w = static_cast<const uint8_t *>(packed_weight);
  p.bias = bias;
  p.cin0 = cin0_dev;
  p.plane0 = plane0_dev;
  p.cnt = cnt_dev;
  p.out = out_nchw;
  CUtensorMap map;
  const int rc = dcf::make_image_map(in_h16, B, H, W, in_C, 1, o9::kHT, o9::kHT, &map);
  if (rc != P3D_OK) return rc;
  const size_t smem = static_cast<size_t>(p.NA) * o9::kABytes + static_cast<size_t>(w_ring) + o9::kPBytes + 1024;
  auto kern = o9::head_out9_kernel;
  P3D_CUDA_CHECK(cudaFuncSetAttribute(kern, cudaFuncAttributeMaxDynamicSharedMemorySize, static_cast<int>(smem)));
  const long long work = static_cast<long long>(B) * p.tiles_y * p.tiles_x * groups;
  cudaLaunchConfig_t cfg = {};
  const long long sms = num_sms();
  cfg.gridDim = dim3(static_cast<unsigned int>(work < sms ? work : sms));
  cfg.blockDim = dim3(tc::kThreads);
  cfg.dynamicSmemBytes = smem;
  cfg.stream = static_cast<cudaStream_t>(stream);
  cudaLaunchAttribute attr[1];
  attr[0].id = cudaLaunchAttributeProgrammaticStreamSerialization;
  attr[0].val.programmaticStreamSerializationAllowed = 1;
  cfg.attrs = attr;
  cfg.numAttrs = 1;
  P3D_CUDA_CHECK(cudaLaunchKernelEx(&cfg, kern, map, p));
  P3D_LAUNCH_CHECK();
  return P3D_OK;
}

extern "C" int p3d_head_conv_p_f16(const void *in_h16, int B, int H, int W, int Cin, const void *packed_weight, int Cout,
                                   const float *scale, const float *shift, const void *packed_w2, float *p_out,
                                   int32_t *status_dev, p3d_stream_t stream) {
  if (!in_h16 || !packed_weight || !packed_w2 || !p_out || B < 1 || H < 1 || W < 1 || Cout < 1) return P3D_ERR_INVALID_ARG;
  if (Cin < 32 || Cin % 32 || Cout % 128) return P3D_ERR_UNSUPPORTED;
  if ((reinterpret_cast<uintptr_t>(in_h16) & 15) || (reinterpret_cast<uintptr_t>(packed_weight) & 15) ||
      (reinterpret_cast<uintptr_t>(packed_w2) & 15) || (reinterpret_cast<uintptr_t>(p_out) & 15))
    return P3D_ERR_INVALID_ARG;
  dcf::ParamsP p = {};
  p.B = B;
  p.H = p.oH = p.out_H = H;
  p.W = p.oW = p.out_W = W;
  p.Cin = Cin;
  p.taps = 9;
  p.kw = 3;
  p.stride = p.pad = p.up = 1;
  p.n_ntiles = Cout / 128;
  p.cout = Cout;
  p.relu = 1;
  p.packed_w = static_cast<const uint8_t *>(packed_weight);
  p.scale = scale;
  p.shift = shift;
  p.status = status_dev;
  p.packed_w2 = static_cast<const uint8_t *>(packed_w2);
  p.tiles_x = (W + dcf::kTW - 1) / dcf::kTW;
  p.tiles_y = (H + dcf::kTH - 1) / dcf::kTH;
  CUtensorMap map, pmap;
  int rc = dcf::make_image_map(in_h16, B, H, W, Cin, 1, dcf::kPitch, dcf::kTH + 2, &map);
  if (rc != P3D_OK || (rc = dcf::make_p_map(p_out, B, H, W, Cout / 64, &pmap)) != P3D_OK) return rc;
  return dcf::launch<128, 1, true, true>(map, pmap, p, static_cast<cudaStream_t>(stream));
}

extern "C" int p3d_head_tap_sum(const float *p_in, int B, int H, int W, int groups, const float *bias, const int32_t *plane0_dev,
                                const int32_t *cnt_dev, int planes, float *out_nchw, p3d_stream_t stream) {
  if (!p_in || !bias || !plane0_dev || !cnt_dev || !out_nchw || B < 1 || H < 1 || W < 1 || groups < 1 || planes < 1 ||
      (reinterpret_cast<uintptr_t>(p_in) & 15))
    return P3D_ERR_INVALID_ARG;
  namespace ts = dcf::tapsum;
  ts::Params p;
  p.B = B;
  p.H = H;
  p.W = W;
  p.groups = groups;
  p.planes = planes;
  p.tiles_x = (W + ts::kTX - 1) / ts::kTX;
  p.tiles_y = (H + ts::kTY - 1) / ts::kTY;
  p.p = p_in;
  p.bias = bias;
  p.plane0 = plane0_dev;
  p.cnt = cnt_dev;
  p.out = out_nchw;
  cudaLaunchConfig_t cfg = {};
  cfg.gridDim = dim3(static_cast<unsigned int>(static_cast<long long>(B) * groups * p.tiles_y * p.tiles_x));
  cfg.blockDim = dim3(ts::kThreads);
  cfg.stream = static_cast<cudaStream_t>(stream);
  cudaLaunchAttribute attr[1];
  attr[0].id = cudaLaunchAttributeProgrammaticStreamSerialization;
  attr[0].val.programmaticStreamSerializationAllowed = 1;
  cfg.attrs = attr;
  cfg.numAttrs = 1;
  P3D_CUDA_CHECK(cudaLaunchKernelEx(&cfg, ts::head_tap_sum_kernel, p));
  P3D_LAUNCH_CHECK();
  return P3D_OK;
}
```

### paddle3d_b200/dense_head.py

```python
import numpy as np
import torch

from .ops import dense_conv as dc

COMMON_HEADS = (("reg", 2), ("height", 1), ("dim", 3), ("rot", 2), ("vel", 2))


class _Conv:

    def __init__(self, cin, cout, k, stride=1, padding=0, bias=False, bn_eps=None, relu=True, up=1, f16=True, transposed=False,
                 cin_pad=None, cout_pad=None):
        self.cin, self.cout, self.k, self.stride, self.padding, self.up = cin, cout, k, stride, padding, up
        self.cin_pad, self.cout_pad = cin_pad, cout_pad
        self.transposed = transposed or up > 1
        self.has_bias, self.bn_eps, self.relu = bias, bn_eps, relu
        self.f16 = f16 and cout >= 16
        self.n_tile = dc.n_tile_for_f16(cout) if self.f16 else dc.n_tile_for(cout)
        self.np = None
        self.dev = None

    def init(self, rng, device=None, randomize_bn=False, bias_value=None, bn_gain=1.0):
        cin, cout, k = self.cin, self.cout, self.k
        bound = 1.0 / np.sqrt(cin * k * k)
        shape = (cin, cout, k, k) if self.transposed else (cout, cin, k, k)
        w = rng.uniform(-bound, bound, size=shape).astype(np.float32)
        b = None
        if self.has_bias:
            b = (np.full(cout, bias_value, np.float32) if bias_value is not None
                 else rng.uniform(-bound, bound, size=cout).astype(np.float32))
        p = dict(weight=w, bias=b, stride=self.stride, padding=self.padding, up=self.up, relu=self.relu, bn=None,
                 transposed=self.transposed)
        if self.bn_eps is not None:
            if randomize_bn:
                g, bt = rng.uniform(0.5, 1.5, cout), rng.uniform(-0.2, 0.2, cout)
                m, v = rng.uniform(-0.1, 0.1, cout), rng.uniform(0.5, 1.5, cout)
            else:
                g, bt, m, v = np.ones(cout), np.zeros(cout), np.zeros(cout), np.ones(cout)
            g = g * bn_gain
            p["bn"] = dict(gamma=g.astype(np.float32), beta=bt.astype(np.float32), mean=m.astype(np.float32),
                           var=v.astype(np.float32), eps=self.bn_eps)
        self.np = p
        s = np.ones(cout)
        t = np.zeros(cout) if b is None else b.astype(np.float64)
        if p["bn"] is not None:
            bn = p["bn"]
            s = bn["gamma"].astype(np.float64) / np.sqrt(bn["var"].astype(np.float64) + bn["eps"])
            t = (t - bn["mean"]) * s + bn["beta"]
        if device is None:
            return self
        if self.f16:
            pack = dc.pack_deconv_weight_f16 if self.transposed else dc.pack_conv_weight_f16
        else:
            pack = dc.pack_deconv_weight if self.transposed else dc.pack_conv_weight
        wd = w
        if self.cin_pad and self.cin_pad > cin:
            ax = 0 if self.transposed else 1
            wd = np.zeros(shape[:ax] + (self.cin_pad,) + shape[ax + 1:], np.float32)
            wd[(slice(None),) * ax + (slice(0, cin),)] = w
        if self.cout_pad and self.cout_pad > cout:
            if self.transposed:
                raise ValueError("cout_pad: Conv2D weights only")
            wp = np.zeros((self.cout_pad,) + wd.shape[1:], np.float32)
            wp[:cout] = wd
            wd = wp
            s, t = np.concatenate([s, np.ones(self.cout_pad - cout)]), np.concatenate([t, np.zeros(self.cout_pad - cout)])
        self.dev = dict(
            packed=pack(torch.from_numpy(wd).to(device), self.n_tile),
            scale=torch.from_numpy(s.astype(np.float32)).to(device) if p["bn"] is not None else None,
            shift=torch.from_numpy(t.astype(np.float32)).to(device) if (p["bn"] is not None or b is not None) else None)
        return self

    def __call__(self, x_split, shape, **kw):
        d = self.dev
        if self.f16:
            if "out_split" in kw:
                kw["out_h16"] = kw.pop("out_split")
            return dc.dense_conv2d_f16(x_split, shape, d["packed"], self.cout_pad or self.cout, self.n_tile, self.k, self.stride,
                                       self.padding, self.up, d["scale"], d["shift"], self.relu, **kw)
        return dc.dense_conv2d(x_split, shape, d["packed"], self.cout, self.n_tile, self.k, self.stride, self.padding, self.up,
                               d["scale"], d["shift"], self.relu, **kw)


class SecondTrunk:

    def __init__(self, in_channels, out_channels, layer_nums, downsample_strides, fpn_out_channels, upsample_strides,
                 use_conv_for_no_stride=True, f16=True):
        self.f16 = f16

        def conv(*a, **k):
            return _Conv(*a, f16=f16, **k)
        bn3 = 1e-3
        self.blocks = []
        cin = in_channels
        for cout, n, s in zip(out_channels, layer_nums, downsample_strides):
            blk = [conv(cin, cout, 3, s, 1, bn_eps=bn3)] + [conv(cout, cout, 3, 1, 1, bn_eps=bn3) for _ in range(n)]
            self.blocks.append(blk)
            cin = cout
        self.deblocks = []
        for ci, co, u in zip(out_channels, fpn_out_channels, upsample_strides):
            if u > 1:
                self.deblocks.append(conv(ci, co, u, u, 0, bn_eps=bn3, up=u))
            elif u < 1:
                k = int(round(1 / u))
                self.deblocks.append(conv(ci, co, k, k, 0, bn_eps=bn3))
            else:
                self.deblocks.append(conv(ci, co, 1, 1, 0, bn_eps=bn3, transposed=not use_conv_for_no_stride))
        self.fpn_channels = int(sum(fpn_out_channels))

    def convs(self):
        return [c for blk in self.blocks for c in blk] + list(self.deblocks)

    def export_numpy(self):
        return dict(blocks=[[c.np for c in blk] for blk in self.blocks], deblocks=[c.np for c in self.deblocks])

    def __call__(self, x, shape, first=None):
        b = shape[0]
        feats = []
        for bi, blk in enumerate(self.blocks):
            for ci, conv in enumerate(blk):
                if bi == 0 and ci == 0 and first is not None:
                    conv = first
                x, _, (b_, oh, ow) = conv(x, shape)
                shape = (b_, oh, ow, conv.cout)
            feats.append((x, shape))
        out_hws = {self.deblock_out_hw(de, fshape[1], fshape[2]) for (_, fshape), de in zip(feats, self.deblocks)}
        if len(out_hws) != 1:
            raise ValueError("the FPN deblocks give feature maps of different sizes %s; the concat needs one size"
                             % sorted(out_hws))
        out_hw = out_hws.pop()
        cat = torch.empty((b * out_hw[0] * out_hw[1], 2 * self.fpn_channels),
                          dtype=torch.float16 if self.f16 else torch.float32, device=x.device)
        c0 = 0
        for (f, fshape), de in zip(feats, self.deblocks):
            de(f, fshape, out_split=cat, out_channels=self.fpn_channels, out_c0=c0)
            c0 += de.cout
        return cat, (b, out_hw[0], out_hw[1], self.fpn_channels)

    @staticmethod
    def deblock_out_hw(de, h, w):
        if de.up > 1:
            return h * de.up, w * de.up
        return (h + 2 * de.padding - de.k) // de.stride + 1, (w + 2 * de.padding - de.k) // de.stride + 1


class DenseRPNHead:
    def __init__(self, in_channels=256, out_channels=(128, 256), layer_nums=(5, 5), downsample_strides=(1, 2),
                 fpn_out_channels=(256, 256), upsample_strides=(1, 2), tasks=(1, 2, 2, 1, 2, 2), share_conv_channel=64,
                 f16=True, with_velocity=True, bev_depth=2, trunk=None):
        if trunk is not None and (not f16 or bev_depth > 1):
            raise ValueError("a custom trunk runs on the fp16-pair path with bev_depth 1")
        self.tasks = list(tasks)
        self.in_channels, self.bev_depth = in_channels, bev_depth
        self.num_classes = list(tasks)
        self.with_velocity = with_velocity
        self.f16 = f16
        if f16 and (share_conv_channel % 32 or not 32 <= share_conv_channel <= 320):
            raise ValueError("the fp16-pair head output convs need share_conv_channel a multiple of 32 and at most 320 "
                             "(got %d); use f16=False" % share_conv_channel)

        def conv(*a, **k):
            return _Conv(*a, f16=f16, **k)
        bn5 = 1e-5
        if trunk is None:
            trunk = SecondTrunk(in_channels, out_channels, layer_nums, downsample_strides, fpn_out_channels,
                                upsample_strides, use_conv_for_no_stride=True, f16=f16)
            self.blocks, self.deblocks = trunk.blocks, trunk.deblocks
        else:
            self.blocks = self.deblocks = None
        self.trunk, self.fpn_channels = trunk, trunk.fpn_channels
        self.shared = conv(self.fpn_channels, share_conv_channel, 3, 1, 1, bias=True, bn_eps=bn5)
        self.heads = []
        for ncls in self.tasks:
            hs = []
            for name, c in list(COMMON_HEADS) + [("hm", ncls)]:
                hs.append((name, conv(share_conv_channel, share_conv_channel, 3, 1, 1, bias=True, bn_eps=bn5),
                           conv(share_conv_channel, c, 3, 1, 1, bias=True, relu=False)))
            self.heads.append(hs)
        self._batched = None

    def all_convs(self):
        out = self.trunk.convs() + [self.shared]
        for hs in self.heads:
            for _, a, b in hs:
                out += [a, b]
        return out

    def head_planes(self):
        return sum(sum(c for _, c in COMMON_HEADS) + n for n in self.tasks)

    def head_flops(self, h, w):
        px = h * w
        sh = self.shared
        out = dict(head_shared=2.0 * px * sh.cin * sh.cout * sh.k * sh.k, head_convmodules=0.0, head_output=0.0)
        for hs in self.heads:
            for _, a, f in hs:
                out["head_convmodules"] += 2.0 * px * a.cin * a.cout * a.k * a.k
                out["head_output"] += 2.0 * px * f.cin * f.cout * f.k * f.k
        out["head"] = out["head_shared"] + out["head_convmodules"] + out["head_output"]
        return out

    def init_weight(self, seed=0, device="cuda", randomize_bn=False, bn_gain=1.0):
        rng = np.random.default_rng(seed)
        hm_finals = {id(b) for hs in self.heads for name, _, b in hs if name == "hm"}
        finals = {id(b) for hs in self.heads for _, _, b in hs}
        for c in self.all_convs():
            dev = None if (self.f16 and id(c) in finals) else device
            c.init(rng, dev, randomize_bn, bias_value=-2.19 if id(c) in hm_finals else None, bn_gain=bn_gain)
        self._batched = None
        self._first_zc = None
        if self.f16 and device is not None and self.bev_depth > 1 and self.in_channels % self.bev_depth == 0:
            c0 = self.blocks[0][0]
            D, C = self.bev_depth, self.in_channels // self.bev_depth
            perm = np.asarray([c * D + z for z in range(D) for c in range(C)])
            zc = _Conv(c0.cin, c0.cout, c0.k, c0.stride, c0.padding, bias=c0.has_bias, bn_eps=c0.bn_eps, relu=c0.relu, f16=True)
            zc.np = dict(c0.np, weight=np.ascontiguousarray(c0.np["weight"][:, perm]))
            zc.dev = dict(c0.dev, packed=dc.pack_conv_weight_f16(torch.from_numpy(zc.np["weight"]).to(device), zc.n_tile))
            self._first_zc = zc
        return self

    def export_numpy(self):
        return dict(self.trunk.export_numpy(), shared=self.shared.np,
                    heads=[[(n, a.np, b.np) for n, a, b in hs] for hs in self.heads])

    def _trunk(self, bev, shape=None):
        first = None
        if shape is None:
            b, c, h, w = bev.shape
            x = dc.nchw_to_pixel_h16(bev) if self.f16 else dc.nchw_to_pixel_split(bev)
            shape = (b, h, w, c)
        else:
            if not self.f16 or (self.bev_depth > 1 and self._first_zc is None):
                raise ValueError("pixel fp16-pair input needs the f16 head")
            x = bev
            first = self._first_zc
        cat, (b, H, W, _) = self.trunk(x, shape, first=first)
        s, _, _ = self.shared(cat, (b, H, W, self.fpn_channels))
        return s, (b, H, W, self.shared.cout)

    def _final_convs(self, mid, shape, in_C, groups_params, planes_total, device):
        from ._lib import check, lib
        from ._mem import ptr, stream
        b, H, W, cin = shape
        gp = groups_params
        planes = torch.empty((b, planes_total, H, W), dtype=torch.float32, device=device)
        if self.f16:
            check(lib().p3d_head_out_conv_f16(ptr(mid), b, H, W, in_C, cin, int(gp["cnt9"].numel()), ptr(gp["packed9"]),
                                              ptr(gp["bias9"]), ptr(gp["cin0_9"]), ptr(gp["plane0_9"]), ptr(gp["cnt9"]),
                                              planes_total, ptr(planes), stream(device)), "head_out_conv_f16")
        else:
            check(lib().p3d_head_final_conv(ptr(mid), b, H, W, in_C, cin, len(gp["cnt"]), ptr(gp["fw"]), ptr(gp["fb"]),
                                            gp["plane0"].ctypes.data, gp["cnt"].ctypes.data, planes_total, ptr(planes),
                                            stream(device)), "head_final_conv")
        return planes

    def _group_params(self, finals, cin, device):
        groups = len(finals)
        wts, plane0, cnt, p0 = [], [], [], 0
        for _, f in finals:
            wts.append(f.np["weight"].transpose(2, 3, 1, 0).reshape(9, cin, f.cout))
            plane0.append(p0)
            cnt.append(f.cout)
            p0 += f.cout
        out = dict(plane0=np.asarray(plane0, np.int32), cnt=np.asarray(cnt, np.int32), planes=p0)
        if not self.f16:
            fw = np.zeros((groups, 9, cin, 4), np.float32)
            fb = np.zeros((groups, 4), np.float32)
            for g, (_, f) in enumerate(finals):
                fw[g, :, :, :f.cout] = wts[g]
                fb[g, :f.cout] = f.np["bias"]
            out.update(fw=torch.from_numpy(fw).to(device), fb=torch.from_numpy(fb).to(device))
            return out
        from ._lib import check, lib
        from ._mem import ptr, stream
        L = lib()
        w9, b9, cin0, pl0, cn = [], [], [], [], []
        for g, (_, f) in enumerate(finals):
            for j0 in range(0, f.cout, 3):
                k = min(3, f.cout - j0)
                w27 = np.zeros((cin, 9, 3), np.float32)
                w27[:, :, :k] = wts[g][:, :, j0:j0 + k].transpose(1, 0, 2)
                w2 = np.zeros((cin, 32), np.float32)
                w2[:, :27] = w27.reshape(cin, 27)
                bb = np.zeros((4,), np.float32)
                bb[:k] = f.np["bias"][j0:j0 + k]
                w9.append(w2)
                b9.append(bb)
                cin0.append(g * cin)
                pl0.append(int(plane0[g]) + j0)
                cn.append(k)
        blk9 = cin * 32 * 4
        packed9 = torch.zeros((len(w9) * blk9,), dtype=torch.uint8, device=device)
        for v, w2 in enumerate(w9):
            wt = torch.from_numpy(w2).to(device)
            check(L.p3d_dense_conv2d_f16_pack_weights(ptr(wt), 1, cin, 32, ptr(packed9[v * blk9:(v + 1) * blk9]),
                                                      ptr(dc._status(device)), stream(device)), "pack_weights")
        i32 = lambda a: torch.from_numpy(np.asarray(a, np.int32)).to(device)
        out.update(packed9=packed9, bias9=torch.from_numpy(np.stack(b9)).to(device), cin0_9=i32(cin0), plane0_9=i32(pl0),
                   cnt9=i32(cn))
        return out

    def _batched_params(self, device):
        if self._batched is not None:
            return self._batched
        firsts = [a for hs in self.heads for _, a, _ in hs]
        finals = [(n, f) for hs in self.heads for n, _, f in hs]
        cin = firsts[0].cin
        big = _Conv(cin, sum(a.cout for a in firsts), 3, 1, 1, bias=True, bn_eps=firsts[0].bn_eps, f16=self.f16)
        w = np.concatenate([a.np["weight"] for a in firsts], 0)
        scale, shift = [], []
        for a in firsts:
            bn = a.np["bn"]
            s_ = bn["gamma"].astype(np.float64) / np.sqrt(bn["var"].astype(np.float64) + bn["eps"])
            scale.append(s_)
            shift.append((a.np["bias"].astype(np.float64) - bn["mean"]) * s_ + bn["beta"])
        pack = dc.pack_conv_weight_f16 if self.f16 else dc.pack_conv_weight
        big.dev = dict(packed=pack(torch.from_numpy(w).to(device), big.n_tile),
                       scale=torch.from_numpy(np.concatenate(scale).astype(np.float32)).to(device),
                       shift=torch.from_numpy(np.concatenate(shift).astype(np.float32)).to(device))
        self._batched = dict(big=big, names=[n for n, _ in finals])
        self._batched.update(self._group_params(finals, cin, device))
        return self._batched

    def calibrate_heatmap_bias(self, bev, score_threshold=0.1, target_frac=0.014, shape=None):
        out = self.forward(bev, shape)
        logit_thr = float(np.log(score_threshold / (1.0 - score_threshold)))
        for t, hs in enumerate(self.heads):
            hm = out["hm"][t].float().amax(dim=1).flatten()
            k = max(1, int(round(hm.numel() * (1.0 - target_frac))))
            q = float(torch.kthvalue(hm, k).values.item())
            fin = [f for name, _, f in hs if name == "hm"][0]
            fin.np["bias"] = (fin.np["bias"] + np.float32(logit_thr - q)).astype(np.float32)
        self._batched = None
        return self

    def forward_h16(self, rows, shape):
        return self.forward(rows, shape)

    def fused_heads(self, bp):
        big = bp["big"]
        return (self.f16 and self.shared.cout == 64 and big.n_tile == 128 and big.cout % 128 == 0
                and all(int(k) <= 3 for k in bp["cnt"]))

    def _heads_conv_p(self, s, shape, bp, device):
        from ._lib import check, lib
        from ._mem import ptr, stream
        b, H, W, cin = shape
        big = bp["big"]
        d = big.dev
        p = torch.empty((b, big.cout // 64, H, W, 28), dtype=torch.float32, device=device)
        check(lib().p3d_head_conv_p_f16(ptr(s), b, H, W, cin, ptr(d["packed"]), big.cout, ptr(d["scale"]), ptr(d["shift"]),
                                        ptr(bp["packed9"]), ptr(p), ptr(dc._status(device)), stream(device)), "head_conv_p_f16")
        return p

    def _tap_sum(self, p, bp, device):
        from ._lib import check, lib
        from ._mem import ptr, stream
        b, groups, H, W, _ = p.shape
        planes = torch.empty((b, bp["planes"], H, W), dtype=torch.float32, device=device)
        check(lib().p3d_head_tap_sum(ptr(p), b, H, W, groups, ptr(bp["bias9"]), ptr(bp["plane0_9"]), ptr(bp["cnt9"]),
                                     bp["planes"], ptr(planes), stream(device)), "head_tap_sum")
        return planes

    def forward(self, bev, shape=None):
        s, shape = self._trunk(bev, shape)
        bp = self._batched_params(bev.device)
        big = bp["big"]
        if self.fused_heads(bp):
            planes = self._tap_sum(self._heads_conv_p(s, shape, bp, bev.device), bp, bev.device)
        else:
            mid, _, _ = big(s, shape)
            planes = self._final_convs(mid, shape, big.cout, bp, bp["planes"], bev.device)
        out = {}
        for name, p0, k in zip(bp["names"], bp["plane0"], bp["cnt"]):
            out.setdefault(name, []).append(planes[:, int(p0):int(p0) + int(k)])
        return out

    __call__ = forward
    forward_batched = forward

    def forward_per_head(self, bev):
        s, shape = self._trunk(bev)
        out = {}
        for hs in self.heads:
            for name, a, fin in hs:
                t, _, _ = a(s, shape)
                k, cin = fin.cout, fin.cin
                if self.f16:
                    gp = self._group_params([(name, fin)], cin, bev.device)
                    planes = self._final_convs(t, shape, a.cout, gp, k, bev.device)
                else:
                    _, planes, _ = fin(t, shape, want_nchw=True)
                out.setdefault(name, []).append(planes)
        return out

    def predict_by_custom_op(self, example, preds_dicts, test_cfg, **kwargs):
        postprocess_fn = kwargs.get("postprocess_fn")
        if postprocess_fn is None:
            from .ops.centerpoint_postprocess import centerpoint_postprocess as postprocess_fn

        def get(obj, key):
            return obj[key] if isinstance(obj, dict) else getattr(obj, key)

        def has(obj, key):
            return key in obj if isinstance(obj, dict) else hasattr(obj, key)

        nms = get(test_cfg, "nms") if has(test_cfg, "nms") else test_cfg
        if isinstance(preds_dicts, dict):
            preds_dicts = [{k: v[t] for k, v in preds_dicts.items()} for t in range(len(self.tasks))]
        hm, reg, height, dim, vel, rot, num_classes, flag = [], [], [], [], [], [], [], 0
        for task_id, pd in enumerate(preds_dicts):
            for nc in self.num_classes:
                num_classes.append(flag)
                flag += nc
            hm.append(pd["hm"])
            reg.append(pd["reg"])
            height.append(pd["height"])
            dim.append(pd["dim"])
            vel.append(pd["vel"] if self.with_velocity else pd["reg"])
            rot.append(pd["rot"])
        bboxes, scores, labels = postprocess_fn(
            hm, reg, height, dim, vel, rot, get(test_cfg, "voxel_size"), get(test_cfg, "point_cloud_range"),
            get(test_cfg, "post_center_limit_range"), num_classes, get(test_cfg, "down_ratio"),
            get(test_cfg, "score_threshold"), get(nms, "nms_iou_threshold"), get(nms, "nms_pre_max_size"),
            get(nms, "nms_post_max_size"), self.with_velocity)
        meta = None if (not example or "meta" not in example or len(example["meta"]) == 0) else example["meta"][0]
        return [{"meta": meta, "box3d_lidar": bboxes, "label_preds": labels, "scores": scores}]
```

### paddle3d_b200/ops/dense_conv.py

```python
import torch

from .._lib import check, lib
from .._mem import ptr, require_cuda, stream


def n_tile_for(cout):
    return 128 if cout >= 128 else (64 if cout > 16 else 16)


def nchw_to_pixel_split(x):
    x = require_cuda(x, "x", torch.float32)
    b, c, h, w = x.shape
    out = torch.empty((b * h * w, 2 * c), dtype=torch.float32, device=x.device)
    check(lib().p3d_nchw_to_pixel_split(ptr(x), b, c, h, w, ptr(out), stream(x.device)), "nchw_to_pixel_split")
    return out


def _pack(w_tci, n_tile):
    L = lib()
    taps, cin, cout = w_tci.shape
    tiles = (cout + n_tile - 1) // n_tile
    total = L.p3d_dense_conv2d_packed_weight_bytes(taps, cin, cout, n_tile)
    if not total:
        raise ValueError("unsupported dense conv shape: taps %d Cin %d Cout %d" % (taps, cin, cout))
    packed = torch.zeros((total // 4,), dtype=torch.float32, device=w_tci.device)
    padded = torch.zeros((taps, cin, tiles * n_tile), dtype=torch.float32, device=w_tci.device)
    padded[:, :, :cout] = w_tci
    block = taps * cin * 2 * n_tile
    for t in range(tiles):
        wt = padded[:, :, t * n_tile:(t + 1) * n_tile].contiguous()
        dst = packed[t * block:(t + 1) * block]
        check(L.p3d_sparse_conv_pack_weights(ptr(wt), taps, cin, n_tile, ptr(dst), stream(wt.device)),
              "sparse_conv_pack_weights")
    return packed


def pack_conv_weight(weight, n_tile):
    weight = require_cuda(weight, "weight", torch.float32)
    cout, cin, kh, kw = weight.shape
    return _pack(weight.permute(2, 3, 1, 0).reshape(kh * kw, cin, cout).contiguous(), n_tile)


def pack_deconv_weight(weight, n_tile):
    weight = require_cuda(weight, "weight", torch.float32)
    cin, cout, k, k2 = weight.shape
    return _pack(weight.permute(2, 3, 0, 1).reshape(k * k2, cin, cout).contiguous(), n_tile)


def dense_conv2d(x_split, shape, packed, cout, n_tile, kernel, stride=1, padding=0, up=1, scale=None, shift=None,
                 relu=False, out_split=None, out_channels=None, out_c0=0, want_nchw=False):
    x_split = require_cuda(x_split, "x_split", torch.float32)
    b, h, w, cin = [int(v) for v in shape]
    if up > 1:
        oh, ow = h * up, w * up
        kh = kw = st = up
        pd = 0
    else:
        kh = kw = int(kernel)
        st, pd = int(stride), int(padding)
        oh, ow = (h + 2 * pd - kh) // st + 1, (w + 2 * pd - kw) // st + 1
    dev = x_split.device
    oc = int(out_channels or cout)
    if out_split is None and not want_nchw:
        out_split = torch.empty((b * oh * ow, 2 * oc), dtype=torch.float32, device=dev)
    out_nchw = torch.empty((b, cout, oh, ow), dtype=torch.float32, device=dev) if want_nchw else None
    check(lib().p3d_dense_conv2d_split(ptr(x_split), b, h, w, cin, ptr(packed), int(cout), int(n_tile), kh, kw, st, pd,
                                       int(up), ptr(scale), ptr(shift), int(relu), ptr(out_split), oc, int(out_c0),
                                       ptr(out_nchw), stream(dev)), "dense_conv2d_split")
    return out_split, out_nchw, (b, oh, ow)


def n_tile_for_f16(cout):
    import os
    forced = os.environ.get("P3D_DENSE_NTILE")
    if forced and cout >= 128:
        return int(forced)
    return 128 if cout >= 128 else 64


def _status(dev):
    from . import sparse_nn as sp
    return sp.status_tensor(dev)


def nchw_to_pixel_h16(x):
    x = require_cuda(x, "x", torch.float32)
    b, c, h, w = x.shape
    out = torch.empty((b * h * w, 2 * c), dtype=torch.float16, device=x.device)
    check(lib().p3d_nchw_to_pixel_h16(ptr(x), b, c, h, w, ptr(out), ptr(_status(x.device)), stream(x.device)),
          "nchw_to_pixel_h16")
    return out


def pixel_h16_to_nchw(x_h16, shape):
    b, h, w, c = [int(v) for v in shape]
    out = torch.empty((b, c, h, w), dtype=torch.float32, device=x_h16.device)
    check(lib().p3d_pixel_h16_to_nchw(ptr(x_h16), b, c, h, w, ptr(out), stream(x_h16.device)), "pixel_h16_to_nchw")
    return out


def _pack_f16(w_tci, n_tile):
    L = lib()
    taps, cin, cout = w_tci.shape
    tiles = (cout + n_tile - 1) // n_tile
    total = L.p3d_dense_conv2d_f16_packed_weight_bytes(taps, cin, cout, n_tile)
    if not total:
        raise ValueError("unsupported dense conv shape: taps %d Cin %d Cout %d" % (taps, cin, cout))
    packed = torch.zeros((total,), dtype=torch.uint8, device=w_tci.device)
    padded = torch.zeros((taps, cin, tiles * n_tile), dtype=torch.float32, device=w_tci.device)
    padded[:, :, :cout] = w_tci
    block = taps * cin * n_tile * 4
    for t in range(tiles):
        wt = padded[:, :, t * n_tile:(t + 1) * n_tile].contiguous()
        dst = packed[t * block:(t + 1) * block]
        check(L.p3d_dense_conv2d_f16_pack_weights(ptr(wt), taps, cin, n_tile, ptr(dst), ptr(_status(wt.device)),
                                                  stream(wt.device)), "dense_conv2d_f16_pack_weights")
    return packed


def pack_conv_weight_f16(weight, n_tile):
    weight = require_cuda(weight, "weight", torch.float32)
    cout, cin, kh, kw = weight.shape
    return _pack_f16(weight.permute(2, 3, 1, 0).reshape(kh * kw, cin, cout).contiguous(), n_tile)


def pack_deconv_weight_f16(weight, n_tile):
    weight = require_cuda(weight, "weight", torch.float32)
    cin, cout, k, k2 = weight.shape
    return _pack_f16(weight.permute(2, 3, 0, 1).reshape(k * k2, cin, cout).contiguous(), n_tile)


def dense_conv2d_f16(x_h16, shape, packed, cout, n_tile, kernel, stride=1, padding=0, up=1, scale=None, shift=None,
                     relu=False, out_h16=None, out_channels=None, out_c0=0, want_nchw=False, mode=0, m_tiles=0,
                     residual=None, res_channels=None):
    x_h16 = require_cuda(x_h16, "x_h16", torch.float16)
    b, h, w, cin = [int(v) for v in shape]
    if up > 1:
        oh, ow = h * up, w * up
        kh = kw = st = up
        pd = 0
    else:
        kh = kw = int(kernel)
        st, pd = int(stride), int(padding)
        oh, ow = (h + 2 * pd - kh) // st + 1, (w + 2 * pd - kw) // st + 1
    dev = x_h16.device
    oc = int(out_channels or cout)
    if out_h16 is None and not want_nchw:
        out_h16 = torch.empty((b * oh * ow, 2 * oc), dtype=torch.float16, device=dev)
    out_nchw = torch.empty((b, cout, oh, ow), dtype=torch.float32, device=dev) if want_nchw else None
    if residual is not None:
        residual = require_cuda(residual, "residual", torch.float16)
        rc = int(res_channels or cout)
        if tuple(residual.shape) != (b * oh * ow, 2 * rc):
            raise ValueError("residual rows %s, want (%d, %d)" % (tuple(residual.shape), b * oh * ow, 2 * rc))
        check(lib().p3d_dense_conv2d_f16_residual(
            ptr(x_h16), b, h, w, cin, ptr(packed), int(cout), int(n_tile), kh, kw, st, pd, int(up), ptr(scale), ptr(shift),
            int(relu), ptr(out_h16), oc, int(out_c0), ptr(out_nchw), ptr(residual), rc, int(mode), int(m_tiles),
            ptr(_status(dev)), stream(dev)), "dense_conv2d_f16_residual")
        return out_h16, out_nchw, (b, oh, ow)
    check(lib().p3d_dense_conv2d_f16(ptr(x_h16), b, h, w, cin, ptr(packed), int(cout), int(n_tile), kh, kw, st, pd, int(up),
                                     ptr(scale), ptr(shift), int(relu), ptr(out_h16), oc, int(out_c0), ptr(out_nchw),
                                     int(mode), int(m_tiles), ptr(_status(dev)), stream(dev)), "dense_conv2d_f16")
    return out_h16, out_nchw, (b, oh, ow)


def upsample_bilinear_h16(x_h16, shape, scale, out_h16=None, out_channels=None, out_c0=0):
    x_h16 = require_cuda(x_h16, "x_h16", torch.float16)
    b, h, w, c = [int(v) for v in shape]
    s = int(scale)
    oc = int(out_channels or c)
    dev = x_h16.device
    if out_h16 is None:
        out_h16 = torch.empty((b * h * s * w * s, 2 * oc), dtype=torch.float16, device=dev)
    check(lib().p3d_upsample_bilinear_h16(ptr(x_h16), b, h, w, c, s, ptr(out_h16), oc, int(out_c0), ptr(_status(dev)),
                                          stream(dev)), "upsample_bilinear_h16")
    return out_h16, (b, h * s, w * s)


def upsample_nearest_h16(x_h16, shape, scale, out_h16=None, out_channels=None, out_c0=0):
    x_h16 = require_cuda(x_h16, "x_h16", torch.float16)
    b, h, w, c = [int(v) for v in shape]
    s = int(scale)
    oc = int(out_channels or c)
    dev = x_h16.device
    if out_h16 is None:
        out_h16 = torch.empty((b * h * s * w * s, 2 * oc), dtype=torch.float16, device=dev)
    check(lib().p3d_upsample_nearest_h16(ptr(x_h16), b, h, w, c, s, ptr(out_h16), oc, int(out_c0), stream(dev)),
          "upsample_nearest_h16")
    return out_h16, (b, h * s, w * s)


def pack_stem_weight(weight):
    weight = require_cuda(weight, "weight", torch.float32).contiguous()
    if tuple(weight.shape) != (64, 3, 7, 7):
        raise ValueError("resnet stem weight %s, want (64, 3, 7, 7)" % (tuple(weight.shape),))
    L = lib()
    packed = torch.empty((L.p3d_resnet_stem_packed_weight_bytes(),), dtype=torch.uint8, device=weight.device)
    check(L.p3d_resnet_stem_pack_weights(ptr(weight), ptr(packed), ptr(_status(weight.device)), stream(weight.device)),
          "resnet_stem_pack_weights")
    return packed


def stem_shape(h, w):
    ch, cw = (h - 1) // 2 + 1, (w - 1) // 2 + 1
    return (ch - 1) // 2 + 1, (cw - 1) // 2 + 1


def resnet_stem_h16(x, packed, scale, shift, out_h16=None):
    x = require_cuda(x, "x", torch.float32)
    b, c, h, w = x.shape
    if c != 3:
        raise ValueError("resnet_stem_h16 takes 3-channel images, got %d" % c)
    ph, pw = stem_shape(h, w)
    if out_h16 is None:
        out_h16 = torch.empty((b * ph * pw, 128), dtype=torch.float16, device=x.device)
    check(lib().p3d_resnet_stem_h16(ptr(x), b, h, w, ptr(packed), ptr(scale), ptr(shift), ptr(out_h16),
                                    ptr(_status(x.device)), stream(x.device)), "resnet_stem_h16")
    return out_h16, (b, ph, pw, 64)
```

### paddle3d_b200/pipeline.py

```python
import torch

from . import synth
from .frame import SWEEP_INPUT, CapturedFrame, ResultSlot, infer_in_flight, in_flight, stream_frames
from .layers import SparseResNet3D
from .ops import centerpoint_postprocess as cpp
from .ops import sparse_nn as sp
from .ops import voxelize as vox


class CenterPointHotPath(CapturedFrame):
    def __init__(self, cfg=None, device="cuda:0", precision=sp.FP32, seed=0, num_points=None, level_caps=None,
                 head_seed=0, with_head=False, keep_bev=True, bn_gain=1.0, sweep_input=None, sweep_ring=None):
        super().__init__(cfg or synth.C3, device, num_points, sweep_input, sweep_ring)
        self.test_cfg = dict(synth.CENTERPOINT_TEST_CFG)
        self.label_off = synth.label_offsets()
        self.net = SparseResNet3D(self.F, self.cfg["voxel_size"], self.cfg["point_cloud_range"])
        self.net.init_weight(seed=seed, device=self.device, bn_gain=bn_gain).set_precision(precision)
        V = self.cfg["max_voxels"]
        self.net.set_level_caps(level_caps or [3 * V, 3 * V, 2 * V, V])
        h = synth.centerpoint_head_outputs(head_seed)
        self.head_host = h
        self.head = {k: [torch.from_numpy(x).to(self.device) for x in v] for k, v in h.items()}
        self.dense = None
        if with_head:
            from .dense_head import DenseRPNHead
            self.dense = DenseRPNHead(in_channels=128 * 2).init_weight(seed=seed + 1, device=self.device, bn_gain=bn_gain)
        self.keep_bev = keep_bev or self.dense is None or not self.dense.f16
        self.slot = ResultSlot(len(self.label_off) * self.test_cfg["nms_post_max_size"], 9, len(self.label_off) + 1,
                               5 if self.sweep_input is None else 6)

    def forward_device(self):
        cfg = self.cfg
        si = self.sweep_input
        if si is not None:
            self._merge_sweeps()
        mean, coors, npv, nv = vox.voxelize_mean(self.points, cfg["voxel_size"], cfg["point_cloud_range"],
                                                 cfg["max_points"], cfg["max_voxels"], 0)
        bev, bev_h16 = None, None
        if self.keep_bev:
            bev = self.net(mean, coors, 1, num=nv)
            h = self.dense(bev) if self.dense is not None else self.head
        else:
            bev_h16 = self.net(mean, coors, 1, num=nv, pixel_h16=True)
            h = self.dense.forward_h16(*bev_h16)
        status = torch.stack([sp.status_tensor(self.device)[0]] + [c[1] for c in self.net.level_counters] +
                             ([self._merge_status[0]] if si is not None else []))
        boxes, scores, labels, counts = cpp.centerpoint_postprocess_heads(h, cfg["voxel_size"][:2], cfg["point_cloud_range"],
                                                                          self.test_cfg, self.label_off)
        return dict(bev=bev, bev_h16=bev_h16, boxes=boxes, scores=scores, labels=labels, counts=counts, num_voxels=nv,
                    coors=coors, mean=mean, status=status)

    def bev_nchw(self):
        if self.out["bev"] is not None:
            self.stream.synchronize()
            return self.out["bev"]
        from .ops import dense_conv as dc
        rows, shape = self.out["bev_h16"]
        with torch.cuda.stream(self.stream):
            out = dc.pixel_h16_to_nchw(rows, shape)
            b, h, w, cd = shape
            D = self.dense.bev_depth
            out = out.view(b, D, cd // D, h, w).transpose(1, 2).reshape(b, cd, h, w).contiguous()
        self.stream.synchronize()
        return out

    def calibrate_head(self, points_dev):
        if self.dense is None:
            return self
        cfg = self.cfg
        with torch.cuda.stream(self.stream):
            self.points.copy_(points_dev)
            mean, coors, npv, nv = vox.voxelize_mean(self.points, cfg["voxel_size"], cfg["point_cloud_range"],
                                                     cfg["max_points"], cfg["max_voxels"], 0)
            bev = self.net(mean, coors, 1, num=nv)
            self.dense.calibrate_heatmap_bias(bev, self.test_cfg["score_threshold"])
        self.stream.synchronize()
        return self

    def check_status(self, status_host):
        st = [int(v) for v in status_host]
        n_levels = len(self.net.level_counters)
        if len(st) > 1 + n_levels:
            self._check_merge_status(st[1 + n_levels])
        if st[0]:
            raise RuntimeError("sparse backbone: an activation left fp16's range (|x| >= 65504) on the fp16-pair path; "
                               "run this model with precision TF32X3_SPLIT")
        for lvl, v in enumerate(st[1:1 + n_levels]):
            if v:
                raise RuntimeError("sparse backbone: strided level %d overflowed its row capacity (set_level_caps); "
                                   "output sites were dropped" % (lvl + 1))

    def share_model(self, other):
        self.net, self.dense = other.net, other.dense

    def export_weights_numpy(self):
        def conv(l):
            return dict(weight=l.weight.cpu().numpy(), bias=None if l.bias is None else l.bias.cpu().numpy(),
                        stride=l.stride, padding=l.padding)

        def bn(l):
            return dict(gamma=l.weight.cpu().numpy(), beta=l.bias.cpu().numpy(), mean=l._mean.cpu().numpy(),
                        var=l._variance.cpu().numpy(), eps=l.epsilon)

        def block(b):
            return dict(conv1=conv(b.conv1), bn1=bn(b.bn1), conv2=conv(b.conv2), bn2=bn(b.bn2))

        n = self.net
        return dict(conv_input=dict(conv=conv(n.conv_input[0]), bn=bn(n.conv_input[1])),
                    blocks0=[block(b) for b in n.blocks0],
                    stages=[dict(down=dict(conv=conv(d[0]), bn=bn(d[1])), blocks=[block(b) for b in bl]) for d, bl in n.stages],
                    extra=dict(conv=conv(n.extra_conv[0]), bn=bn(n.extra_conv[1])))


class CenterPointSweep:

    def __init__(self, lanes=2, frame_cls=None, **kw):
        if lanes < 1:
            raise ValueError("lanes >= 1")
        frame_cls = frame_cls or CenterPointHotPath
        first = frame_cls(**kw)
        if kw.get("sweep_input") is not None and kw.get("sweep_ring") is None:
            from .sweep_ring import SweepRing
            si = first.sweep_input
            first.ring = SweepRing(si["max_sweeps"], si["raw_dim"], si["slot_cap"], si["max_sweeps"] + lanes, first.device)
            kw = dict(kw, sweep_ring=first.ring)
        self.lanes = [first]
        for _ in range(lanes - 1):
            p = frame_cls(**kw)
            p.share_model(first)
            self.lanes.append(p)
        self.device = first.device

    def __len__(self):
        return len(self.lanes)

    def calibrate_head(self, points_dev):
        self.lanes[0].calibrate_head(points_dev)
        return self

    def capture(self, points_dev, **kw):
        for p in self.lanes:
            p.points.copy_(points_dev)
            p.capture(**kw)
        return self

    def prepare_sweep(self):
        for p in self.lanes:
            p.prepare_sweep()
        return self

    def launch(self, i, points_dev):
        p = self.lanes[i % len(self.lanes)]
        with torch.cuda.stream(p.stream):
            p.points.copy_(points_dev, non_blocking=True)
            p.graph.replay()
        return p

    def synchronize(self):
        for p in self.lanes:
            p.stream.synchronize()

    @staticmethod
    def plan(n_frames, lanes):
        for kind, i, _, lane, slot in in_flight(range(n_frames), lanes):
            yield kind, i, lane, slot

    def infer_stream(self, items):
        return stream_frames(self.lanes, self.lanes[0].ring, items)

    def infer_many(self, frames_host):
        if any(p.graph is None for p in self.lanes):
            raise RuntimeError("infer_many needs captured lanes: call capture() first")
        yield from infer_in_flight(self.lanes, frames_host)
```

### paddle3d_b200/pointpillars.py

```python
import numpy as np
import torch

from . import synth
from .dense_head import SecondTrunk, _Conv
from .ops import anchor_postprocess as ahp
from .ops import pillar_encoder as pe
from .ops import sparse_nn as sp
from .ops import voxelize as vox
from .frame import CapturedFrame, ResultSlot

CONFIG = dict(
    pfn_channels=64, pfn_bn_eps=1e-3,
    backbone=dict(out_channels=(64, 128, 256), layer_nums=(3, 5, 5), downsample_strides=(2, 2, 2)),
    fpn=dict(out_channels=(128, 128, 128), upsample_strides=(1, 2, 4), use_conv_for_no_stride=False),
    anchors_per_loc=2, box_code_size=7, num_dir_bins=2,
    anchor=dict(sizes=(1.6, 3.9, 1.56), strides=(0.32, 0.32, 0.0), offsets=(0.16, -39.52, -1.78), rotations=(0.0, 1.57)),
    test=dict(anchor_area_threshold=1, nms_score_threshold=0.05, nms_iou_threshold=0.5, nms_pre_max_size=1000,
              nms_post_max_size=300, post_center_limit_range=[0.0, -39.68, -5.0, 69.12, 39.68, 5.0]),
)

_PED_CYCLIST_ANCHOR = dict(strides=(0.16, 0.16, 0.0), offsets=(0.08, -19.76, -1.465), rotations=(0.0, 1.57))
CONFIG_PED_CYCLIST = dict(
    pfn_channels=64, pfn_bn_eps=1e-3,
    backbone=dict(out_channels=(64, 128, 256), layer_nums=(3, 5, 5), downsample_strides=(1, 2, 2)),
    fpn=dict(out_channels=(128, 128, 128), upsample_strides=(1, 2, 4), use_conv_for_no_stride=False),
    num_classes=2, anchors_per_loc=4, box_code_size=7, num_dir_bins=2,
    anchors=[dict(_PED_CYCLIST_ANCHOR, sizes=(0.6, 1.76, 1.73)),
             dict(_PED_CYCLIST_ANCHOR, sizes=(0.6, 0.8, 1.73))],
    test=dict(anchor_area_threshold=1, nms_score_threshold=0.05, nms_iou_threshold=0.5, nms_pre_max_size=1000,
              nms_post_max_size=300, post_center_limit_range=[0.0, -19.84, -2.5, 47.36, 19.84, 0.5]),
)


def grid_size(cfg):
    pcr, vs = cfg["point_cloud_range"], cfg["voxel_size"]
    return (int(round((pcr[3] - pcr[0]) / vs[0])), int(round((pcr[4] - pcr[1]) / vs[1])))


def create_anchors_3d_stride(feature_size, sizes, anchor_strides, anchor_offsets, rotations, dtype=np.float32):
    x_stride, y_stride, z_stride = anchor_strides
    x_offset, y_offset, z_offset = anchor_offsets
    z_centers = np.arange(feature_size[0], dtype=dtype) * z_stride + z_offset
    y_centers = np.arange(feature_size[1], dtype=dtype) * y_stride + y_offset
    x_centers = np.arange(feature_size[2], dtype=dtype) * x_stride + x_offset
    sizes = np.reshape(np.array(sizes, dtype=dtype), [-1, 3])
    rotations = np.array(rotations, dtype=dtype)
    rets = list(np.meshgrid(x_centers, y_centers, z_centers, rotations, indexing="ij"))
    tile_shape = [1] * 5
    tile_shape[-2] = int(sizes.shape[0])
    for i in range(len(rets)):
        rets[i] = np.tile(rets[i][..., np.newaxis, :], tile_shape)[..., np.newaxis]
    sizes = np.reshape(sizes, [1, 1, 1, -1, 1, 3])
    tile_size_shape = list(rets[0].shape)
    tile_size_shape[3] = 1
    rets.insert(3, np.tile(sizes, tile_size_shape))
    return np.transpose(np.concatenate(rets, axis=-1), [2, 1, 0, 3, 4, 5])


def anchor_voxel_corners(anchors, voxel_size, point_cloud_range, grid):
    rb = anchors[:, [0, 1, 3, 4, 6]]
    rots = rb[:, -1]
    folded = np.abs(rots - np.floor(rots / np.pi + 0.5) * np.pi)
    cond = (folded > np.pi / 4)[:, np.newaxis]
    centre_dims = np.where(cond, rb[:, [0, 1, 3, 2]], rb[:, :4])
    near = np.concatenate([centre_dims[:, :2] - centre_dims[:, 2:] / 2, centre_dims[:, :2] + centre_dims[:, 2:] / 2], -1)
    out = np.zeros(near.shape, dtype=np.int32)
    out[:, 0] = np.floor((near[:, 0] - point_cloud_range[0]) / voxel_size[0])
    out[:, 1] = np.floor((near[:, 1] - point_cloud_range[1]) / voxel_size[1])
    out[:, 2] = np.floor((near[:, 2] - point_cloud_range[0]) / voxel_size[0])
    out[:, 3] = np.floor((near[:, 3] - point_cloud_range[1]) / voxel_size[1])
    out[:, [0, 2]] = np.clip(out[:, [0, 2]], 0, grid[0] - 1)
    out[:, [1, 3]] = np.clip(out[:, [1, 3]], 0, grid[1] - 1)
    return out


class PointPillars:

    def __init__(self, cfg=None, model_cfg=None):
        self.cfg = dict(cfg or synth.C2)
        self.mc = model_cfg or CONFIG
        mc = self.mc
        self.grid = grid_size(self.cfg)
        self.F = self.cfg["point_dim"]
        self.C = mc["pfn_channels"]
        self.trunk = SecondTrunk(self.C, mc["backbone"]["out_channels"], mc["backbone"]["layer_nums"],
                                 mc["backbone"]["downsample_strides"], mc["fpn"]["out_channels"],
                                 mc["fpn"]["upsample_strides"], mc["fpn"]["use_conv_for_no_stride"])
        R, self.num_classes = mc["anchors_per_loc"], mc.get("num_classes", 1)
        self.head_channels = R * (self.num_classes + mc["box_code_size"] + mc["num_dir_bins"])
        self.head = _Conv(self.trunk.fpn_channels, self.head_channels, 1, bias=True, relu=False)
        s = mc["backbone"]["downsample_strides"][0]
        self.feat_hw = (self.grid[1] // s, self.grid[0] // s)
        per_class = [create_anchors_3d_stride([1, self.feat_hw[0], self.feat_hw[1]], a["sizes"], a["strides"],
                                              a["offsets"], a["rotations"])
                     for a in (mc["anchors"] if "anchors" in mc else [mc["anchor"]])]
        self.anchors_np = np.concatenate(per_class, axis=3).reshape(-1, 7)
        if len(per_class) != self.num_classes or self.anchors_np.shape[0] != self.feat_hw[0] * self.feat_hw[1] * R:
            raise ValueError("model config: one anchor generator per class, anchors_per_loc anchors per location")
        self.corners_np = anchor_voxel_corners(self.anchors_np, self.cfg["voxel_size"], self.cfg["point_cloud_range"],
                                               self.grid)
        self.device = None

    def init_weight(self, seed=0, device="cuda", bn_gain=1.0):
        rng = np.random.default_rng(seed)
        C, F = self.C, self.F
        self.pfn = dict(weight=synth.kaiming_uniform(rng, (F + 5, C), F + 5),
                        gamma=np.full(C, bn_gain, np.float32), beta=np.zeros(C, np.float32),
                        mean=np.zeros(C, np.float32), var=np.ones(C, np.float32), eps=self.mc["pfn_bn_eps"])
        for c in self.trunk.convs():
            c.init(rng, device, bn_gain=bn_gain)
        self.head.init(rng, device)
        self.device = None if device is None else torch.device(device)
        if device is not None:
            p = self.pfn
            self.pfn_weight = torch.from_numpy(p["weight"]).to(device)
            self.pfn_folded = pe.fold_bn(p["gamma"], p["beta"], p["mean"], p["var"], p["eps"], device)
            self.anchors = torch.from_numpy(np.ascontiguousarray(self.anchors_np)).to(device)
            self.corners = torch.from_numpy(np.ascontiguousarray(self.corners_np)).to(device)
        return self

    def export_numpy(self):
        return dict(self.trunk.export_numpy(), pfn=self.pfn, head=self.head.np)

    def encode(self, points):
        cfg = self.cfg
        voxels, co, npv, nv = vox.hard_voxelize(points, cfg["voxel_size"], cfg["point_cloud_range"], cfg["max_points"],
                                                cfg["max_voxels"])
        coors = torch.nn.functional.pad(co, (1, 0))
        p = self.pfn
        feats = pe.pillar_feature_net(voxels, npv, coors, self.pfn_weight, p["gamma"], p["beta"], p["mean"], p["var"],
                                      p["eps"], cfg["voxel_size"], cfg["point_cloud_range"], num_voxels=nv,
                                      folded=self.pfn_folded)
        nx, ny = self.grid
        rows = sp.sparse_coo_tensor(coors, feats, [1, 1, ny, nx, self.C], num=nv)
        image, shape = rows.to_pixel_h16()
        return image, shape, coors, nv

    def dense(self, image, shape):
        cat, cshape = self.trunk(image, shape)
        _, planes, _ = self.head(cat, cshape, want_nchw=True)
        return planes

    def postprocess(self, planes, coors, nv, anchor_mask=None, sorted_out=None):
        t = self.mc["test"]
        return ahp.anchor_head_postprocess_device(
            planes, self.anchors, self.corners, coors, nv, self.grid, t["post_center_limit_range"],
            t["anchor_area_threshold"], t["nms_score_threshold"], t["nms_iou_threshold"], t["nms_pre_max_size"],
            t["nms_post_max_size"], anchor_mask=anchor_mask, sorted_out=sorted_out, num_classes=self.num_classes)

    def calibrate_cls_bias(self, points, target_frac=0.02):
        image, shape, coors, nv = self.encode(points)
        planes = self.dense(image, shape)
        mask = torch.empty((self.anchors.shape[0],), dtype=torch.uint8, device=planes.device)
        self.postprocess(planes, coors, nv, anchor_mask=mask)
        R, C = self.mc["anchors_per_loc"], self.num_classes
        cls = planes[0, :R * C].reshape(R, C, *planes.shape[2:])
        k = int(round(target_frac * self.anchors.shape[0] / C))
        thr = self.mc["test"]["nms_score_threshold"]
        logit_thr = float(np.log(thr / (1.0 - thr)))
        b = self.head.np["bias"].copy()
        for c in range(C):
            logits = cls[:, c].permute(1, 2, 0).reshape(-1)[mask.bool()].float().cpu().numpy()
            if len(logits) > k:
                v = np.sort(logits)[::-1]
                shift = logit_thr - 0.5 * (float(v[k - 1]) + float(v[k]))
            else:
                shift = logit_thr - float(logits.min()) + 1.0 if len(logits) else 0.0
            b[c:R * C:C] = (b[c:R * C:C] + np.float32(shift)).astype(np.float32)
        self.head.np["bias"] = b
        self.head.dev["shift"].copy_(torch.from_numpy(b))
        return self

    def flops(self):
        out = dict(backbone=0.0, fpn=0.0, head=0.0)
        h, w = self.grid[1], self.grid[0]
        sizes = []
        for blk in self.trunk.blocks:
            for c in blk:
                h, w = (h + 2 * c.padding - c.k) // c.stride + 1, (w + 2 * c.padding - c.k) // c.stride + 1
                out["backbone"] += 2.0 * h * w * c.cin * c.cout * c.k * c.k
            sizes.append((h, w))
        for (h, w), de in zip(sizes, self.trunk.deblocks):
            out["fpn"] += 2.0 * (h * de.up) * (w * de.up) * de.cin * de.cout * (1 if de.up > 1 else de.k * de.k)
        out["head"] = 2.0 * self.feat_hw[0] * self.feat_hw[1] * self.head.cin * self.head.cout
        return out


class PointPillarsHotPath(CapturedFrame):

    def __init__(self, cfg=None, device="cuda:0", seed=0, num_points=None, bn_gain=1.0, model_cfg=None):
        super().__init__(cfg or synth.C2, device, num_points)
        self.model = PointPillars(self.cfg, model_cfg).init_weight(seed=seed, device=self.device, bn_gain=bn_gain)
        self.slot = ResultSlot(self.model.mc["test"]["nms_post_max_size"], 7, 2, 1)

    def forward_device(self):
        m = self.model
        image, shape, coors, nv = m.encode(self.points)
        planes = m.dense(image, shape)
        boxes, scores, labels, counts = m.postprocess(planes, coors, nv)
        status = sp.status_tensor(self.device).clone()
        return dict(boxes=boxes, scores=scores, labels=labels, counts=counts, num_voxels=nv, coors=coors, planes=planes,
                    status=status)

    def _calibrate(self):
        self.model.calibrate_cls_bias(self.points)

    @staticmethod
    def check_status(status_host):
        if int(status_host[0]):
            raise RuntimeError("PointPillars: an activation left fp16's range (|x| >= 65504) on the fp16-pair path")
```

Baseline: 434.4.

## Chain consecutive 3x3 trunk convs with per-tile readiness flags across launches

Runs a sequence of stride-1 3x3 dense conv layers as chained PDL launches. Each CTA pulls work items from an atomic ticket counter and, before loading its input, waits on global per-tile ready counters for the 3x3 neighbourhood of tiles from the previous layer. A layer can therefore start on tiles whose inputs are already finished instead of waiting for the whole previous layer to drain, which hides the tail of each launch. The cost is spin-waiting with a timeout, a status flag and error path for timeouts, an extra memset of the workspace, and dependence on co-residency of the CTAs.

```diff
diff --git a/include/p3d_b200.h b/include/p3d_b200.h
--- a/include/p3d_b200.h
+++ b/include/p3d_b200.h
@@ -215,6 +215,16 @@
                          int kh, int kw, int stride, int pad, int up, const float *scale, const float *shift, int relu,
                          void *out_h16, int out_C, int out_c0, float *out_nchw, int mode, int m_tiles,
                          int32_t *status_dev, p3d_stream_t stream);
+typedef struct p3d_dense_chain_layer {
+  const void *packed_weight;
+  const float *scale, *shift;
+  void *out_h16;
+  int Cin, Cout, n_tile, kh, kw, stride, pad, relu;
+} p3d_dense_chain_layer;
+size_t p3d_dense_conv2d_f16_chain_workspace_bytes(int L, int B, int H, int W);
+int p3d_dense_conv2d_f16_chain(const void *in_h16, int B, int H, int W, const p3d_dense_chain_layer *layers, int L,
+                               void *workspace, size_t workspace_bytes, int max_ctas, int32_t *status_dev,
+                               p3d_stream_t stream);
 int p3d_dense_conv2d_f16_residual(const void *in_h16, int B, int H, int W, int Cin, const void *packed_weight, int Cout,
                                   int n_tile, int kh, int kw, int stride, int pad, int up, const float *scale,
                                   const float *shift, int relu, void *out_h16, int out_C, int out_c0, float *out_nchw,
diff --git a/paddle3d_b200/_lib.py b/paddle3d_b200/_lib.py
--- a/paddle3d_b200/_lib.py
+++ b/paddle3d_b200/_lib.py
@@ -87,6 +87,8 @@
     "p3d_head_tap_sum": (_int, [_vp, _int, _int, _int, _int, _vp, _vp, _vp, _int, _vp, _vp]),
     "p3d_dense_conv2d_f16": (_int, [_vp, _int, _int, _int, _int, _vp, _int, _int, _int, _int, _int, _int, _int, _vp, _vp,
                                     _int, _vp, _int, _int, _vp, _int, _int, _vp, _vp]),
+    "p3d_dense_conv2d_f16_chain_workspace_bytes": (_sz, [_int, _int, _int, _int]),
+    "p3d_dense_conv2d_f16_chain": (_int, [_vp, _int, _int, _int, _vp, _int, _vp, _sz, _int, _vp, _vp]),
     "p3d_dense_conv2d_f16_residual": (_int, [_vp, _int, _int, _int, _int, _vp, _int, _int, _int, _int, _int, _int, _int, _vp,
                                              _vp, _int, _vp, _int, _int, _vp, _vp, _int, _int, _int, _vp, _vp]),
     "p3d_upsample_bilinear_h16": (_int, [_vp, _int, _int, _int, _int, _int, _vp, _int, _int, _vp, _vp]),
diff --git a/paddle3d_b200/centerpoint_pillars.py b/paddle3d_b200/centerpoint_pillars.py
--- a/paddle3d_b200/centerpoint_pillars.py
+++ b/paddle3d_b200/centerpoint_pillars.py
@@ -139,5 +139,8 @@
         st = [int(v) for v in status_host]
         if len(st) > 1:
             self._check_merge_status(st[1])
+        if st[0] & 2:
+            raise RuntimeError("CenterPoint-pillars: a chained conv launch of the dense trunk timed out waiting for its "
+                               "input tiles; the frame's outputs are not valid")
         if st[0]:
             raise RuntimeError("CenterPoint-pillars: an activation left fp16's range (|x| >= 65504) on the fp16-pair path")
diff --git a/paddle3d_b200/csrc/dense_conv_f16.cu b/paddle3d_b200/csrc/dense_conv_f16.cu
--- a/paddle3d_b200/csrc/dense_conv_f16.cu
+++ b/paddle3d_b200/csrc/dense_conv_f16.cu
@@ -43,8 +43,29 @@
   const uint8_t *res_h16;
   int res_C;
 };
-template <bool FUSE_P, bool RES = false>
-using KParams = std::conditional_t<FUSE_P, ParamsP, std::conditional_t<RES, ParamsR, Params>>;
+constexpr int kMaxChain = 6;
+constexpr int kItemSlots = 4;
+struct Layer {
+  const uint8_t *packed_w;
+  const float *scale, *shift;
+  int Cin, cout, n_ntiles, relu;
+};
+struct ParamsC : Params {
+  CUtensorMap in_maps[kMaxChain], out_maps[kMaxChain];
+  Layer layer[kMaxChain];
+  int L, lay;
+  int first[kMaxChain + 1];
+  int32_t *ticket;
+  int32_t *ready;
+};
+template <bool FUSE_P, bool RES = false, bool CHAIN = false>
+using KParams = std::conditional_t<CHAIN, ParamsC, std::conditional_t<FUSE_P, ParamsP, std::conditional_t<RES, ParamsR, Params>>>;
+
+template <class P>
+__device__ __forceinline__ Layer layer_of(const P &p, int l) {
+  if constexpr (std::is_same_v<P, ParamsC>) return p.layer[l];
+  else return Layer{p.packed_w, p.scale, p.shift, p.Cin, p.cout, p.n_ntiles, p.relu};
+}
 
 constexpr int kP2Blk = 64 * 32, kP2Bytes = 4 * kP2Blk, kPPitch = 28;
 
@@ -108,6 +129,7 @@
 __device__ __forceinline__ void bulk_wait_all() { asm volatile("cp.async.bulk.wait_group 0;" ::: "memory"); }
 struct Item {
   int nt, tap0, tx0, ty0, b;
+  int l = 0;
 };
 
 enum TraceField {
@@ -118,6 +140,7 @@
   kTrStageFree = kTrEpi + 2,
   kTrAEmpty = kTrStageFree + 2, kTrBEmpty,
   kTrEwWait, kTrEwBusy,
+  kTrDepWait,
   kTrFields
 };
 #ifdef P3D_DENSE_TRACE
@@ -160,6 +183,75 @@
   it.ty0 = static_cast<int>(q % p.tiles_y) * th;
   it.b = static_cast<int>(q / p.tiles_y);
   return it;
+}
+__device__ __forceinline__ Item decode_chain(int t, const ParamsC &p) {
+  Item it;
+  int l = 0;
+  while (l + 1 < p.L && t >= p.first[l + 1]) ++l;
+  int q = t - p.first[l];
+  const int nn = p.layer[l].n_ntiles;
+  it.l = l;
+  it.nt = q % nn;
+  q /= nn;
+  it.tap0 = 0;
+  it.tx0 = (q % p.tiles_x) * kTW;
+  q /= p.tiles_x;
+  it.ty0 = (q % p.tiles_y) * kTH;
+  it.b = q / p.tiles_y;
+  return it;
+}
+
+constexpr uint32_t kItemReaders = kConsumerWarps + kEpiThreads / 32;
+struct ItemRing {
+  volatile int *ticket;
+  unsigned long long *full, *empty;
+  uint32_t slot = 0, ph = 0;
+  __device__ __forceinline__ void put(int t) {
+    mbar_wait(smem_u32(empty + slot), ph ^ 1u);
+    ticket[slot] = t;
+    mbar_arrive(smem_u32(full + slot));
+    if (++slot == kItemSlots) slot = 0, ph ^= 1u;
+  }
+  __device__ __forceinline__ int take() {
+    mbar_wait(smem_u32(full + slot), ph);
+    const int t = ticket[slot];
+    __syncwarp();
+    if ((threadIdx.x & 31) == 0) mbar_arrive(smem_u32(empty + slot));
+    if (++slot == kItemSlots) slot = 0, ph ^= 1u;
+    return t;
+  }
+};
+
+__device__ __forceinline__ int ld_acquire_gpu(const int32_t *p) {
+  int v;
+  asm volatile("ld.acquire.gpu.global.s32 %0, [%1];" : "=r"(v) : "l"(p) : "memory");
+  return v;
+}
+__device__ __forceinline__ void red_release_gpu_add(int32_t *p, int v) {
+  asm volatile("red.release.gpu.global.add.s32 [%0], %1;" ::"l"(p), "r"(v) : "memory");
+}
+__device__ __forceinline__ void fence_proxy_async_global() { asm volatile("fence.proxy.async.global;" ::: "memory"); }
+__device__ __forceinline__ unsigned long long globaltimer() {
+  unsigned long long t;
+  asm volatile("mov.u64 %0, %%globaltimer;" : "=l"(t));
+  return t;
+}
+constexpr unsigned long long kDepTimeoutNs = 200ull * 1000 * 1000;
+
+__device__ __noinline__ bool wait_inputs(const ParamsC &p, const Item &im) {
+  const int tx = im.tx0 / kTW, ty = im.ty0 / kTH, need = p.layer[im.l - 1].n_ntiles;
+  const int32_t *ready = p.ready + (static_cast<size_t>(im.l - 1) * p.B + im.b) * p.tiles_y * p.tiles_x;
+  const unsigned long long t0 = globaltimer();
+  for (int y = max(ty - 1, 0); y <= min(ty + 1, p.tiles_y - 1); ++y)
+    for (int x = max(tx - 1, 0); x <= min(tx + 1, p.tiles_x - 1); ++x) {
+      unsigned int ns = 64;
+      while (ld_acquire_gpu(ready + y * p.tiles_x + x) < need) {
+        if (globaltimer() - t0 > kDepTimeoutNs) return false;
+        __nanosleep(ns);
+        ns = ns < 1024 ? 2 * ns : ns;
+      }
+    }
+  return true;
 }
 
 template <int N, int MT>
@@ -237,16 +329,26 @@
   if (et == 0) tr.flush(0);
 }
 
-template <int N, int MT, bool FUSE_P>
-__device__ __forceinline__ void epilogue_pairs(const Params &p, const CUtensorMap *out_map, const uint8_t *tiles, int tile_bytes,
+template <int N, int MT, bool FUSE_P, bool CHAIN, class P>
+__device__ __forceinline__ void epilogue_pairs(const P &p, const CUtensorMap *out_map, const uint8_t *tiles, int tile_bytes,
                                                unsigned long long *staged, unsigned long long *freed, long long n_items,
-                                               int th, int et) {
+                                               ItemRing ring, int th, int et) {
   constexpr int NQ = N / 32, BLK = 64 * 128;
   const bool lead = et == 0;
   const bool whole = p.out_c0 % 32 == 0;
   Trace tr;
-  for (long long idx = 0; idx < n_items; ++idx) {
-    const Item im = decode(idx, p, th);
+  for (long long idx = 0;; ++idx) {
+    Item im;
+    if constexpr (CHAIN) {
+      const int t = ring.take();
+      if (t < 0) break;
+      im = decode_chain(t, p);
+      out_map = &p.out_maps[im.l];
+    } else {
+      if (idx >= n_items) break;
+      im = decode(idx, p, th);
+    }
+    const int cout = layer_of(p, im.l).cout;
     const int dy = p.up > 1 ? im.tap0 / p.up : 0, dx = p.up > 1 ? im.tap0 % p.up : 0;
     for (int c = 0; c < 2; ++c) {
       long long t0 = tr.now();
@@ -258,9 +360,9 @@
       } else {
         for (int blk = 0; blk < MT * NQ; ++blk) {
           const int ch0 = im.nt * N + (blk % NQ) * 32, iy0 = im.ty0 + (blk / NQ) * kTH + c * 8;
-          if (ch0 >= p.cout) continue;
+          if (ch0 >= cout) continue;
           const uint8_t *src = tiles + c * tile_bytes + blk * BLK;
-          if (whole && ch0 + 32 <= p.cout) {
+          if (whole && ch0 + 32 <= cout) {
             if (!lead) continue;
             const int hc = 2 * (p.out_c0 + ch0);
             if (p.up == 1) {
@@ -273,7 +375,7 @@
           }
           for (int u = et; u < 128; u += kEpiThreads) {
             const int r = u >> 1, h = u & 1, iy = iy0 + (r >> 3), ix = im.tx0 + (r & 7);
-            if (ch0 + 16 * h >= p.cout || iy >= p.oH || ix >= p.oW) continue;
+            if (ch0 + 16 * h >= cout || iy >= p.oH || ix >= p.oW) continue;
             const int oc = p.out_c0 + ch0 + 16 * h, Y = iy * p.up + dy, X = ix * p.up + dx;
             uint8_t *op = p.out_h16 + ((static_cast<size_t>(im.b) * p.out_H + Y) * p.out_W + X) * (4 * static_cast<size_t>(p.out_C)) +
                           (oc / 32) * 128 + (oc % 32) * 2;
@@ -293,6 +395,13 @@
       mbar_arrive(smem_u32(freed + c));
       tr.add(kTrEwBusy, t0);
     }
+    if constexpr (CHAIN) {
+      if (lead && im.l + 1 < p.L) {
+        bulk_wait_all();
+        fence_proxy_async_global();
+        red_release_gpu_add(p.ready + ((static_cast<size_t>(im.l) * p.B + im.b) * p.tiles_y + im.ty0 / kTH) * p.tiles_x + im.tx0 / kTW, 1);
+      }
+    }
   }
   if (lead) {
     bulk_wait_all();
@@ -300,27 +409,34 @@
   }
 }
 
-template <int N, int MT, bool HALO, bool FUSE_P = false, bool RES = false>
+template <int N, int MT, bool HALO, bool FUSE_P = false, bool RES = false, bool CHAIN = false>
 __global__ void __launch_bounds__(kDenseThreads, 1)
     dense_conv_f16_kernel(const __grid_constant__ CUtensorMap in_map, const __grid_constant__ CUtensorMap out_map,
-                          const KParams<FUSE_P, RES> p) {
+                          const __grid_constant__ KParams<FUSE_P, RES, CHAIN> p) {
   using C = Cfg<N, MT, HALO>;
   static_assert(!(FUSE_P && RES), "a residual launch writes the pixel H16 image");
+  static_assert(!CHAIN || (N == 128 && MT == 1 && HALO && !FUSE_P && !RES), "chained launch: the trunk's 3x3 layers");
   static_assert(!FUSE_P || (N == 128 && MT == 1 && HALO && 2 * kP2Bytes == C::B_BYTES &&
                             2 * 64 * kPPitch * 4 <= C::PAIR_BYTES),
                 "fused P: two 64-channel heads' W2 images fill one weight slot; P fits over the pair blocks");
   constexpr int TH = kTH * MT;
   constexpr int H = N / 2;
   asm volatile("griddepcontrol.launch_dependents;" ::: "memory");
-  asm volatile("griddepcontrol.wait;" ::: "memory");
+  bool chained_input = false;
+  if constexpr (CHAIN) chained_input = p.lay > 0;
+  if (!chained_input) asm volatile("griddepcontrol.wait;" ::: "memory");
   const int up2 = p.up * p.up;
-  const long long n_total = static_cast<long long>(p.B) * p.tiles_y * p.tiles_x * p.n_ntiles * (p.up > 1 ? up2 : 1);
+  long long n_total;
+  if constexpr (CHAIN) n_total = p.first[p.lay + 1] - p.first[p.lay];
+  else n_total = static_cast<long long>(p.B) * p.tiles_y * p.tiles_x * p.n_ntiles * (p.up > 1 ? up2 : 1);
   if (static_cast<long long>(blockIdx.x) >= n_total) return;
   const long long n_items = (n_total - blockIdx.x + gridDim.x - 1) / gridDim.x;
 
   extern __shared__ __align__(1024) uint8_t smem_raw[];
   uint8_t *smem = reinterpret_cast<uint8_t *>((reinterpret_cast<uintptr_t>(smem_raw) + 1023) & ~uintptr_t(1023));
-  __shared__ __align__(8) unsigned long long s_bar[2 * kMaxA + 2 * kMaxB + 4];
+  constexpr int kIF = 2 * kMaxA + 2 * kMaxB + 4, kIE = kIF + kItemSlots;
+  __shared__ __align__(8) unsigned long long s_bar[kIF + (CHAIN ? 2 * kItemSlots : 0)];
+  __shared__ int s_ticket[CHAIN ? kItemSlots : 1];
   constexpr int kAF = 0, kAE = kMaxA, kBF = 2 * kMaxA, kBE = 2 * kMaxA + kMaxB, kSS = 2 * kMaxA + 2 * kMaxB, kSF = kSS + 2;
 
   const int tid = threadIdx.x, wg = tid >> 7, wtid = tid & 127;
@@ -337,59 +453,92 @@
       mbar_init(smem_u32(&s_bar[kSS + c]), 128);
       mbar_init(smem_u32(&s_bar[kSF + c]), kEpiThreads);
     }
+    if constexpr (CHAIN) {
+      for (int s = 0; s < kItemSlots; ++s) {
+        mbar_init(smem_u32(&s_bar[kIF + s]), 1);
+        mbar_init(smem_u32(&s_bar[kIE + s]), kItemReaders);
+      }
+    }
     fence_mbar_init();
   }
   __syncthreads();
   const uint32_t a_ring = smem_u32(smem);
   const uint32_t b_ring = a_ring + C::NA * C::A_BYTES;
   float *const stg = reinterpret_cast<float *>(smem + C::NA * C::A_BYTES + C::NB * C::B_BYTES);
-  const bool pairs = p.out_nchw == nullptr;
-  const int G = p.Cin / 32;
+  const bool pairs = CHAIN || p.out_nchw == nullptr;
   const int taps_item = p.up > 1 ? 1 : p.taps;
-  const int units_item = HALO ? G : taps_item * G;
+  ItemRing ring{s_ticket, s_bar + kIF, s_bar + kIE};
 
   if (wg == 0) {
     asm volatile("setmaxnreg.dec.sync.aligned.u32 %0;" ::"n"(C::P_REGS));
     if (tid >= 32) {
       if (pairs)
-        epilogue_pairs<N, MT, FUSE_P>(p, &out_map, reinterpret_cast<const uint8_t *>(stg), C::STG_WG * 4, s_bar + kSS, s_bar + kSF,
-                              n_items, TH, tid - 32);
-      else
+        epilogue_pairs<N, MT, FUSE_P, CHAIN>(p, &out_map, reinterpret_cast<const uint8_t *>(stg), C::STG_WG * 4, s_bar + kSS,
+                                             s_bar + kSF, n_items, ring, TH, tid - 32);
+      else if constexpr (!CHAIN)
         epilogue_warps<N, MT>(p, stg, s_bar + kSS, s_bar + kSF, n_items, TH, tid - 32);
       return;
     }
     if (tid != 0) return;
     uint32_t a_slot = 0, a_ph = 0, b_slot = 0, b_ph = 0;
+    bool waits = true;
     Trace tr;
-    for (long long idx = 0; idx < n_items; ++idx) {
-      const Item im = decode(idx, p, TH);
-      const uint8_t *w_tile = p.packed_w + static_cast<size_t>(im.nt) * p.taps * (p.Cin / 16) * C::B_BLK;
+    for (long long idx = 0;; ++idx) {
+      Item im;
+      const CUtensorMap *imap = &in_map;
+      if constexpr (CHAIN) {
+        const int t = atomicAdd(p.ticket + p.lay, 1);
+        ring.put(t < n_total ? p.first[p.lay] + t : -1);
+        if (t >= n_total) break;
+        im = decode_chain(p.first[p.lay] + t, p);
+        imap = &p.in_maps[im.l];
+      } else {
+        if (idx >= n_items) break;
+        im = decode(idx, p, TH);
+      }
+      const Layer ly = layer_of(p, im.l);
+      const int G = ly.Cin / 32;
+      const uint8_t *w_tile = ly.packed_w + static_cast<size_t>(im.nt) * p.taps * (ly.Cin / 16) * C::B_BLK;
       int dy = 0, dx = 0;
       for (int tu = 0; tu < (HALO ? 1 : taps_item); ++tu) {
         const int tap = p.up > 1 ? im.tap0 : tu;
+        auto fill_b = [&](int t, int g) {
+          const uint32_t bbar = smem_u32(&s_bar[kBF + b_slot]);
+          const long long t1 = tr.now();
+          mbar_wait(smem_u32(&s_bar[kBE + b_slot]), b_ph ^ 1u);
+          tr.add(kTrBEmpty, t1);
+          mbar_arrive_expect_tx(bbar, static_cast<uint32_t>(C::B_BYTES));
+          bulk_g2s(b_ring + b_slot * C::B_BYTES, w_tile + (static_cast<size_t>(HALO ? t : tap) * (ly.Cin / 16) + 2 * g) * C::B_BLK,
+                   static_cast<uint32_t>(C::B_BYTES), bbar);
+          if (++b_slot == C::NB) b_slot = 0, b_ph ^= 1u;
+        };
         for (int g = 0; g < G; ++g) {
+          int t_first = 0;
+          if constexpr (CHAIN) {
+            if (g == 0 && im.l > 0) {
+              for (; t_first < (C::NB < C::SPU ? C::NB : C::SPU); ++t_first) fill_b(t_first, g);
+              const long long t0 = tr.now();
+              if (waits && !wait_inputs(p, im)) {
+                waits = false;
+                if (p.status) atomicOr(p.status, 2);
+              }
+              fence_proxy_async_global();
+              tr.add(kTrDepWait, t0);
+            }
+          }
           const uint32_t abar = smem_u32(&s_bar[kAF + a_slot]), a_dst = a_ring + a_slot * C::A_BYTES;
           const long long t0 = tr.now();
           mbar_wait(smem_u32(&s_bar[kAE + a_slot]), a_ph ^ 1u);
           tr.add(kTrAEmpty, t0);
           mbar_arrive_expect_tx(abar, static_cast<uint32_t>(C::A_ROWS * 128));
           if (HALO) {
-            tma_tile4d(a_dst, &in_map, g * 64, im.tx0 - 1, im.ty0 - 1, im.b, abar);
+            tma_tile4d(a_dst, imap, g * 64, im.tx0 - 1, im.ty0 - 1, im.b, abar);
           } else {
             const int x = im.tx0 * p.stride - p.pad + dx, y = im.ty0 * p.stride - p.pad + dy;
-            tma_tile4d(a_dst, &in_map, g * 64, x, y, im.b, abar);
+            tma_tile4d(a_dst, imap, g * 64, x, y, im.b, abar);
           }
           if (++a_slot == C::NA) a_slot = 0, a_ph ^= 1u;
-          for (int t = 0; t < C::SPU; ++t) {
-            const uint32_t bbar = smem_u32(&s_bar[kBF + b_slot]);
-            const long long t1 = tr.now();
-            mbar_wait(smem_u32(&s_bar[kBE + b_slot]), b_ph ^ 1u);
-            tr.add(kTrBEmpty, t1);
-            mbar_arrive_expect_tx(bbar, static_cast<uint32_t>(C::B_BYTES));
-            bulk_g2s(b_ring + b_slot * C::B_BYTES, w_tile + (static_cast<size_t>(HALO ? t : tap) * (p.Cin / 16) + 2 * g) * C::B_BLK,
-                     static_cast<uint32_t>(C::B_BYTES), bbar);
-            if (++b_slot == C::NB) b_slot = 0, b_ph ^= 1u;
-          }
+          for (int t = t_first; t < C::SPU; ++t) fill_b(t, g);
         }
         if (++dx == p.kw) dx = 0, ++dy;
       }
@@ -404,6 +553,7 @@
         if (++b_slot == C::NB) b_slot = 0, b_ph ^= 1u;
       }
     }
+    if (chained_input) asm volatile("griddepcontrol.wait;" ::: "memory");
     tr.flush(0);
     return;
   }
@@ -419,16 +569,27 @@
   bool ovf = false;
   Trace tr;
   const long long t_start = tr.now();
-  for (long long idx = 0; idx < n_items; ++idx) {
+  long long idx = 0;
+  for (;; ++idx) {
+    Item im;
+    if constexpr (CHAIN) {
+      const int t = ring.take();
+      if (t < 0) break;
+      im = decode_chain(t, p);
+    } else {
+      if (idx >= n_items) break;
+      im = decode(idx, p, TH);
+    }
+    const Layer ly = layer_of(p, im.l);
+    const int units_item = HALO ? ly.Cin / 32 : taps_item * (ly.Cin / 32);
 #pragma unroll
     for (int i = 0; i < C::ACC; ++i) acc[i] = 0.f;
-    const Item im = decode(idx, p, TH);
     const uint32_t ss = smem_u32(stg) + cw * C::STG_WG * 4 + C::PAIR_BYTES + static_cast<uint32_t>(idx & 1) * 2 * N * 4;
     if (pairs) {
       for (int c = wtid; c < 2 * N; c += 128) {
         const int ch = im.nt * N + c % N;
-        const float *src = c < N ? p.scale : p.shift;
-        st_shared_u32(ss + c * 4, __float_as_uint(ch < p.cout && src ? __ldg(src + ch) : (c < N ? 1.0f : 0.0f)));
+        const float *src = c < N ? ly.scale : ly.shift;
+        st_shared_u32(ss + c * 4, __float_as_uint(ch < ly.cout && src ? __ldg(src + ch) : (c < N ? 1.0f : 0.0f)));
       }
     }
     uint32_t prev_b = 0;
@@ -541,7 +702,7 @@
                 v1 += fmaf(fl.y, kLoInv, fh.y);
               }
             }
-            if (p.relu) v0 = fmaxf(v0, 0.f), v1 = fmaxf(v1, 0.f);
+            if (ly.relu) v0 = fmaxf(v0, 0.f), v1 = fmaxf(v1, 0.f);
             __half2 hi, lo;
             split_h16x2(v0, v1, hi, lo, o[mt][h]);
             const uint32_t off = (mt * (N / 32) + j / 4) * C::PAIR_BLK + h * 8 * 128;
@@ -618,7 +779,7 @@
   }
   if (ovf && p.status) atomicOr(p.status, 1);
   if (cw == 0) {
-    tr.count(kTrItems, static_cast<unsigned long long>(n_items));
+    tr.count(kTrItems, static_cast<unsigned long long>(idx));
     tr.add(kTrCycles, t_start);
   }
   if (wtid == 0) tr.flush(cw);
@@ -728,16 +889,19 @@
   return r == CUDA_SUCCESS ? P3D_OK : P3D_ERR_INVALID_ARG;
 }
 
-template <int N, int MT, bool HALO, bool FUSE_P = false, bool RES = false>
-int launch(const CUtensorMap &map, const CUtensorMap &out_map, const KParams<FUSE_P, RES> &p, cudaStream_t st) {
+template <int N, int MT, bool HALO, bool FUSE_P = false, bool RES = false, bool CHAIN = false>
+int launch(const CUtensorMap &map, const CUtensorMap &out_map, const KParams<FUSE_P, RES, CHAIN> &p, cudaStream_t st,
+           int max_ctas = 0) {
   using C = Cfg<N, MT, HALO>;
   const size_t smem = static_cast<size_t>(C::NA) * C::A_BYTES + static_cast<size_t>(C::NB) * C::B_BYTES + C::STG_BYTES + 1024;
   if (smem > static_cast<size_t>(kSmemBudget)) return P3D_ERR_UNSUPPORTED;
-  auto kern = dense_conv_f16_kernel<N, MT, HALO, FUSE_P, RES>;
+  auto kern = dense_conv_f16_kernel<N, MT, HALO, FUSE_P, RES, CHAIN>;
   P3D_CUDA_CHECK(cudaFuncSetAttribute(kern, cudaFuncAttributeMaxDynamicSharedMemorySize, static_cast<int>(smem)));
-  const long long work = static_cast<long long>(p.B) * p.tiles_y * p.tiles_x * p.n_ntiles * (p.up > 1 ? p.up * p.up : 1);
+  long long work;
+  if constexpr (CHAIN) work = p.first[p.lay + 1] - p.first[p.lay];
+  else work = static_cast<long long>(p.B) * p.tiles_y * p.tiles_x * p.n_ntiles * (p.up > 1 ? p.up * p.up : 1);
   cudaLaunchConfig_t cfg = {};
-  const long long sms = num_sms();
+  const long long sms = max_ctas > 0 && max_ctas < num_sms() ? max_ctas : num_sms();
   cfg.gridDim = dim3(static_cast<unsigned int>(work < sms ? work : sms));
   cfg.blockDim = dim3(kDenseThreads);
   cfg.dynamicSmemBytes = smem;
@@ -1076,6 +1240,72 @@
   if (static_cast<long long>(B) * oh * ow * 4 * res_C > 0x7fffffffll) return P3D_ERR_UNSUPPORTED;
   return dense_conv2d_f16<true>(in_h16, B, H, W, Cin, packed_weight, Cout, n_tile, kh, kw, stride, pad, up, scale, shift, relu,
                                 out_h16, out_C, out_c0, out_nchw, res_h16, res_C, mode, m_tiles, status_dev, stream);
+}
+
+extern "C" size_t p3d_dense_conv2d_f16_chain_workspace_bytes(int L, int B, int H, int W) {
+  if (L < 1 || L > dcf::kMaxChain || B < 1 || H < 1 || W < 1) return 0;
+  const size_t tiles = static_cast<size_t>((W + dcf::kTW - 1) / dcf::kTW) * ((H + dcf::kTH - 1) / dcf::kTH);
+  return (L + static_cast<size_t>(L - 1) * B * tiles) * sizeof(int32_t);
+}
+
+extern "C" int p3d_dense_conv2d_f16_chain(const void *in_h16, int B, int H, int W, const p3d_dense_chain_layer *layers, int L,
+                                          void *workspace, size_t workspace_bytes, int max_ctas, int32_t *status_dev,
+                                          p3d_stream_t stream) {
+  if (!in_h16 || !layers || !workspace || L < 1 || L > dcf::kMaxChain || B < 1 || H < 1 || W < 1 || max_ctas < 0)
+    return P3D_ERR_INVALID_ARG;
+  if ((reinterpret_cast<uintptr_t>(in_h16) & 15) || (reinterpret_cast<uintptr_t>(workspace) & 3)) return P3D_ERR_INVALID_ARG;
+  if (workspace_bytes < p3d_dense_conv2d_f16_chain_workspace_bytes(L, B, H, W)) return P3D_ERR_WORKSPACE;
+  dcf::ParamsC p = {};
+  p.B = B;
+  p.H = p.oH = p.out_H = H;
+  p.W = p.oW = p.out_W = W;
+  p.taps = 9;
+  p.kw = 3;
+  p.stride = p.pad = p.up = 1;
+  p.tiles_x = (W + dcf::kTW - 1) / dcf::kTW;
+  p.tiles_y = (H + dcf::kTH - 1) / dcf::kTH;
+  p.status = status_dev;
+  p.L = L;
+  p.ticket = static_cast<int32_t *>(workspace);
+  p.ready = p.ticket + L;
+  const long long tiles = static_cast<long long>(B) * p.tiles_y * p.tiles_x;
+  const uint8_t *in = static_cast<const uint8_t *>(in_h16);
+  size_t in_bytes = 0;
+  long long items = 0;
+  for (int l = 0; l < L; ++l) {
+    const p3d_dense_chain_layer &d = layers[l];
+    if (!d.packed_weight || !d.out_h16 || d.Cin < 32 || d.Cin % 32 || d.Cout < 32) return P3D_ERR_INVALID_ARG;
+    if (d.kh != 3 || d.kw != 3 || d.stride != 1 || d.pad != 1 || d.n_tile != 128) return P3D_ERR_UNSUPPORTED;
+    if (d.Cout % 32) return P3D_ERR_UNSUPPORTED;
+    if (l > 0 && d.Cin != layers[l - 1].Cout) return P3D_ERR_INVALID_ARG;
+    if ((reinterpret_cast<uintptr_t>(d.packed_weight) & 15) || (reinterpret_cast<uintptr_t>(d.out_h16) & 15) ||
+        (reinterpret_cast<uintptr_t>(d.scale) & 15) || (reinterpret_cast<uintptr_t>(d.shift) & 15))
+      return P3D_ERR_INVALID_ARG;
+    const uint8_t *out = static_cast<const uint8_t *>(d.out_h16);
+    const size_t out_bytes = static_cast<size_t>(B) * H * W * 4 * static_cast<size_t>(d.Cout);
+    if (l == 0) in_bytes = static_cast<size_t>(B) * H * W * 4 * static_cast<size_t>(d.Cin);
+    if (out < in + in_bytes && in < out + out_bytes) return P3D_ERR_INVALID_ARG;
+    int rc = dcf::make_image_map(in, B, H, W, d.Cin, 1, dcf::kPitch, dcf::kTH + 2, &p.in_maps[l]);
+    if (rc != P3D_OK || (rc = dcf::make_out_map(d.out_h16, B, H, W, d.Cout, 1, &p.out_maps[l])) != P3D_OK) return rc;
+    p.layer[l] = dcf::Layer{static_cast<const uint8_t *>(d.packed_weight), d.scale, d.shift, d.Cin, d.Cout, (d.Cout + 127) / 128,
+                            d.relu};
+    p.first[l] = static_cast<int>(items);
+    items += tiles * p.layer[l].n_ntiles;
+    if (items > 0x7fffffffll) return P3D_ERR_UNSUPPORTED;
+    in = out;
+    in_bytes = out_bytes;
+  }
+  p.first[L] = static_cast<int>(items);
+  p.Cin = layers[0].Cin;
+  p.cout = p.out_C = layers[L - 1].Cout;
+  p.out_c0 = 0;
+  const cudaStream_t st = static_cast<cudaStream_t>(stream);
+  P3D_CUDA_CHECK(cudaMemsetAsync(workspace, 0, p3d_dense_conv2d_f16_chain_workspace_bytes(L, B, H, W), st));
+  for (p.lay = 0; p.lay < L; ++p.lay) {
+    const int rc = dcf::launch<128, 1, true, false, false, true>(p.in_maps[p.lay], p.out_maps[p.lay], p, st, max_ctas);
+    if (rc != P3D_OK) return rc;
+  }
+  return P3D_OK;
 }
 
 extern "C" int p3d_head_out_conv_f16(const void *in_h16, int B, int H, int W, int in_C, int Cin, int groups,
diff --git a/paddle3d_b200/dense_head.py b/paddle3d_b200/dense_head.py
--- a/paddle3d_b200/dense_head.py
+++ b/paddle3d_b200/dense_head.py
@@ -70,6 +70,15 @@
             shift=torch.from_numpy(t.astype(np.float32)).to(device) if (p["bn"] is not None or b is not None) else None)
         return self
 
+    def chains(self):
+        return (self.f16 and not self.transposed and self.k == 3 and self.stride == 1 and self.padding == 1 and
+                self.n_tile == 128 and (self.cout_pad or self.cout) % 32 == 0)
+
+    def chain_layer(self):
+        d = self.dev
+        return dict(packed=d["packed"], cout=self.cout_pad or self.cout, n_tile=self.n_tile, kernel=self.k,
+                    stride=self.stride, padding=self.padding, scale=d["scale"], shift=d["shift"], relu=self.relu)
+
     def __call__(self, x_split, shape, **kw):
         d = self.dev
         if self.f16:
@@ -117,11 +126,21 @@
         b = shape[0]
         feats = []
         for bi, blk in enumerate(self.blocks):
-            for ci, conv in enumerate(blk):
-                if bi == 0 and ci == 0 and first is not None:
-                    conv = first
+            convs = [first if bi == 0 and ci == 0 and first is not None else c for ci, c in enumerate(blk)]
+            ci = 0
+            while ci < len(convs):
+                cj = ci
+                while (cj < len(convs) and cj - ci < dc.CHAIN_MAX_LAYERS and convs[cj].chains() and
+                       dc.chain_items(shape[:3], convs[cj].cout_pad or convs[cj].cout) > dc.sm_count(x.device)):
+                    cj += 1
+                if cj - ci >= 2:
+                    outs, shape = dc.dense_conv2d_f16_chain(x, shape, [c.chain_layer() for c in convs[ci:cj]])
+                    x, ci = outs[-1], cj
+                    continue
+                conv = convs[ci]
                 x, _, (b_, oh, ow) = conv(x, shape)
                 shape = (b_, oh, ow, conv.cout)
+                ci += 1
             feats.append((x, shape))
         out_hws = {self.deblock_out_hw(de, fshape[1], fshape[2]) for (_, fshape), de in zip(feats, self.deblocks)}
         if len(out_hws) != 1:
diff --git a/paddle3d_b200/ops/dense_conv.py b/paddle3d_b200/ops/dense_conv.py
--- a/paddle3d_b200/ops/dense_conv.py
+++ b/paddle3d_b200/ops/dense_conv.py
@@ -1,3 +1,5 @@
+import ctypes as C
+
 import torch
 
 from .._lib import check, lib
@@ -164,6 +166,50 @@
     return out_h16, out_nchw, (b, oh, ow)
 
 
+CHAIN_MAX_LAYERS = 6
+
+
+def chain_items(bhw, cout):
+    b, h, w = [int(v) for v in bhw]
+    return b * -(-h // 16) * -(-w // 8) * -(-int(cout) // 128)
+
+
+def sm_count(device):
+    return torch.cuda.get_device_properties(device).multi_processor_count
+
+
+class _ChainLayer(C.Structure):
+    _fields_ = [("packed_weight", C.c_void_p), ("scale", C.c_void_p), ("shift", C.c_void_p), ("out_h16", C.c_void_p)] + \
+               [(n, C.c_int) for n in ("Cin", "Cout", "n_tile", "kh", "kw", "stride", "pad", "relu")]
+
+
+def dense_conv2d_f16_chain(x_h16, shape, layers, max_ctas=0):
+    x_h16 = require_cuda(x_h16, "x_h16", torch.float16)
+    b, h, w, cin = [int(v) for v in shape]
+    dev = x_h16.device
+    L = lib()
+    n = len(layers)
+    desc = (_ChainLayer * n)()
+    outs = []
+    for d, ly in zip(desc, layers):
+        cout = int(ly["cout"])
+        out = torch.empty((b * h * w, 2 * cout), dtype=torch.float16, device=dev)
+        outs.append(out)
+        k = int(ly["kernel"])
+        d.packed_weight, d.scale, d.shift, d.out_h16 = (ptr(ly["packed"]).value, ptr(ly["scale"]).value,
+                                                        ptr(ly["shift"]).value, out.data_ptr())
+        d.Cin, d.Cout, d.n_tile, d.kh, d.kw = cin, cout, int(ly["n_tile"]), k, k
+        d.stride, d.pad, d.relu = int(ly["stride"]), int(ly["padding"]), int(bool(ly["relu"]))
+        cin = cout
+    nbytes = L.p3d_dense_conv2d_f16_chain_workspace_bytes(n, b, h, w)
+    if not nbytes:
+        raise ValueError("unsupported dense conv chain: %d layers on %s" % (n, (b, h, w)))
+    ws = torch.empty((nbytes // 4,), dtype=torch.int32, device=dev)
+    check(L.p3d_dense_conv2d_f16_chain(ptr(x_h16), b, h, w, C.addressof(desc), n, ptr(ws), nbytes, int(max_ctas),
+                                       ptr(_status(dev)), stream(dev)), "dense_conv2d_f16_chain")
+    return outs, (b, h, w, cin)
+
+
 def upsample_bilinear_h16(x_h16, shape, scale, out_h16=None, out_channels=None, out_c0=0):
     x_h16 = require_cuda(x_h16, "x_h16", torch.float16)
     b, h, w, c = [int(v) for v in shape]
diff --git a/paddle3d_b200/pipeline.py b/paddle3d_b200/pipeline.py
--- a/paddle3d_b200/pipeline.py
+++ b/paddle3d_b200/pipeline.py
@@ -82,6 +82,9 @@
         n_levels = len(self.net.level_counters)
         if len(st) > 1 + n_levels:
             self._check_merge_status(st[1 + n_levels])
+        if st[0] & 2:
+            raise RuntimeError("dense trunk: a chained conv launch timed out waiting for its input tiles; the frame's "
+                               "outputs are not valid")
         if st[0]:
             raise RuntimeError("sparse backbone: an activation left fp16's range (|x| >= 65504) on the fp16-pair path; "
                                "run this model with precision TF32X3_SPLIT")
diff --git a/paddle3d_b200/pointpillars.py b/paddle3d_b200/pointpillars.py
--- a/paddle3d_b200/pointpillars.py
+++ b/paddle3d_b200/pointpillars.py
@@ -207,5 +207,8 @@
 
     @staticmethod
     def check_status(status_host):
+        if int(status_host[0]) & 2:
+            raise RuntimeError("PointPillars: a chained conv launch of the dense trunk timed out waiting for its input "
+                               "tiles; the frame's outputs are not valid")
         if int(status_host[0]):
             raise RuntimeError("PointPillars: an activation left fp16's range (|x| >= 65504) on the fp16-pair path")
```

New measurement: 429.0, median of 6. About the same (-1.2%).
